# wmeddie/CycloneML

Hardware: AMD Instinct MI355X
Metric: rows/s per training iteration (higher is better)
Workload: dtype f64

## Files before the change

### cycloneml_amd/csrc/kmeans.hip

```cpp
#pragma clang fp contract(off)

#include <hip/hip_runtime.h>

#include <algorithm>
#include <cmath>
#include <cstdlib>
#include <mutex>
#include <utility>
#include <vector>

#include "common.hpp"
#include "kmeans_i8.hpp"
#include "kmeans_cos.hpp"
#include "kmeans_sparse.hpp"
#include "silhouette.hpp"

namespace {

constexpr int kWaves = 8;
constexpr int kAssignThreads = kWaves * 64;
constexpr int kSortTile = 4096;
constexpr int kChunkRows = 256;
constexpr int kMaxK = 8192;

constexpr int kNormRows = 256, kNormCols = 16, kNormStride = kNormCols + 1;
__global__ __launch_bounds__(kNormRows) void k_row_norms(const double* __restrict__ X, int64_t n,
                                                         int d, double* __restrict__ norms) {
  __shared__ double tile[2][kNormRows * kNormStride];
  const int t = threadIdx.x;
  const int64_t row0 = (int64_t)blockIdx.x * kNormRows;
  constexpr int PER = kNormRows * kNormCols / kNormRows;
  double v[PER];
  auto load = [&](int c0) {
#pragma unroll
    for (int i = 0; i < PER; ++i) {
      const int e = t + kNormRows * i, r = e / kNormCols, c = c0 + e % kNormCols;
      const int64_t gr = row0 + r;
      v[i] = (gr < n && c < d) ? __builtin_nontemporal_load(&X[gr * d + c]) : 0.0;
    }
  };
  auto store = [&](double* b) {
#pragma unroll
    for (int i = 0; i < PER; ++i) {
      const int e = t + kNormRows * i;
      b[(e / kNormCols) * kNormStride + e % kNormCols] = v[i];
    }
  };
  double s = 0.0;
  load(0);
  store(tile[0]);
  int buf = 0;
  for (int c0 = 0; c0 < d; c0 += kNormCols) {
    if (c0 + kNormCols < d) load(c0 + kNormCols);
    __syncthreads();
    const double* row = tile[buf] + t * kNormStride;
    const int lim = min(kNormCols, d - c0);
    for (int c = 0; c < lim; ++c) s = dadd(s, dmul(row[c], row[c]));
    if (c0 + kNormCols < d) store(tile[buf ^ 1]);
    buf ^= 1;
  }
  const int64_t gr = row0 + t;
  if (gr < n) norms[gr] = __builtin_sqrt(s);
}

__global__ void k_center_transpose(const double* __restrict__ C, int k, int d, int d4, int kpad,
                                   double* __restrict__ Ct) {
  int64_t idx = (int64_t)blockIdx.x * blockDim.x + threadIdx.x;
  int64_t total = (int64_t)d4 * kpad;
  if (idx >= total) return;
  int j = (int)(idx / kpad), i = (int)(idx % kpad);
  Ct[idx] = (i < k && j < d) ? C[(int64_t)i * d + j] : 0.0;
}

constexpr unsigned long long kInfBits = 0x7FF0000000000000ull;
constexpr int kStT = 32;
constexpr int kStC = 32;

__global__ void k_fill_u64(unsigned long long* __restrict__ p, int n, unsigned long long v) {
  const int i = blockIdx.x * blockDim.x + threadIdx.x;
  if (i < n) p[i] = v;
}
__global__ void k_center_transpose_fill(const double* __restrict__ C, int k, int d, int d4,
                                        int kpad, double* __restrict__ Ct,
                                        unsigned long long* __restrict__ p, unsigned long long v) {
  const int64_t idx = (int64_t)blockIdx.x * blockDim.x + threadIdx.x;
  if (idx < k) p[idx] = v;
  const int64_t total = (int64_t)d4 * kpad;
  if (idx >= total) return;
  const int j = (int)(idx / kpad), i = (int)(idx % kpad);
  Ct[idx] = (i < k && j < d) ? C[(int64_t)i * d + j] : 0.0;
}
__global__ void k_zero2(unsigned int* __restrict__ a, unsigned int* __restrict__ b) {
  if (threadIdx.x == 0) *a = 0u;
  if (threadIdx.x == 1 && b) *b = 0u;
}

__global__ __launch_bounds__(256) void k_stats_pairs(const double* __restrict__ C, int k, int d,
                                                     int tps, double* __restrict__ packed,
                                                     unsigned long long* __restrict__ dmin) {
  __shared__ double Ci[kStT][kStC + 1], Cj[kStT][kStC + 1];
  __shared__ unsigned long long rmin[kStT], cmin[kStT];
  int t = blockIdx.x, bi = 0;
  while (t >= tps - bi) {
    t -= tps - bi;
    ++bi;
  }
  const int bj = bi + t;
  const int tx = threadIdx.x & 15, ty = threadIdx.x >> 4;
  if (threadIdx.x < kStT) rmin[threadIdx.x] = cmin[threadIdx.x] = kInfBits;
  double s00 = 0.0, s01 = 0.0, s10 = 0.0, s11 = 0.0;
  for (int c0 = 0; c0 < d; c0 += kStC) {
    __syncthreads();
    for (int e = threadIdx.x; e < kStT * kStC; e += 256) {
      const int r = e >> 5, cc = e & 31, col = c0 + cc;
      const int gi = bi * kStT + r, gj = bj * kStT + r;
      Ci[r][cc] = (gi < k && col < d) ? C[(int64_t)gi * d + col] : 0.0;
      Cj[r][cc] = (gj < k && col < d) ? C[(int64_t)gj * d + col] : 0.0;
    }
    __syncthreads();
    const int lim = min(kStC, d - c0);
    for (int cc = 0; cc < lim; ++cc) {
      const double a0 = Ci[ty][cc], a1 = Ci[ty + 16][cc];
      const double b0 = Cj[tx][cc], b1 = Cj[tx + 16][cc];
      double q = dsub(a0, b0);
      s00 = dadd(s00, dmul(q, q));
      q = dsub(a0, b1);
      s01 = dadd(s01, dmul(q, q));
      q = dsub(a1, b0);
      s10 = dadd(s10, dmul(q, q));
      q = dsub(a1, b1);
      s11 = dadd(s11, dmul(q, q));
    }
  }
  const double sv[2][2] = {{s00, s01}, {s10, s11}};
#pragma unroll
  for (int a = 0; a < 2; ++a) {
#pragma unroll
    for (int b = 0; b < 2; ++b) {
      const int i = bi * kStT + ty + 16 * a, j = bj * kStT + tx + 16 * b;
      if (i < k && j < k && j > i) {
        const double dist = __builtin_sqrt(sv[a][b]);
        const double v = dmul(dmul(0.25, dist), dist);
        packed[iut(i, j)] = v;
        const unsigned long long bits = (unsigned long long)__double_as_longlong(v);
        atomicMin(&rmin[ty + 16 * a], bits);
        atomicMin(&cmin[tx + 16 * b], bits);
      }
    }
  }
  __syncthreads();
  if (threadIdx.x < kStT) {
    const int i = bi * kStT + threadIdx.x, j = bj * kStT + threadIdx.x;
    if (i < k && rmin[threadIdx.x] != kInfBits) atomicMin(&dmin[i], rmin[threadIdx.x]);
    if (j < k && cmin[threadIdx.x] != kInfBits) atomicMin(&dmin[j], cmin[threadIdx.x]);
  }
}

__global__ void k_stats_diag(int k, double* __restrict__ packed,
                             const unsigned long long* __restrict__ dmin) {
  const int i = blockIdx.x * blockDim.x + threadIdx.x;
  if (i >= k) return;
  if (k == 1) {
    packed[0] = __builtin_nan("");
    return;
  }
  packed[iut(i, i)] = __longlong_as_double((long long)dmin[i]);
}

struct Slot {
  float L1, U1, L2;
  int I1;
};

__device__ __forceinline__ float ulp_down(float f) {
  int b = __float_as_int(f);
  if (f == 0.0f) return -__int_as_float(1);
  return __int_as_float(f > 0.0f ? b - 1 : b + 1);
}
__device__ __forceinline__ float f_down(double x) {
  float f = (float)x;
  return ((double)f > x) ? ulp_down(f) : f;
}
__device__ __forceinline__ float f_up(double x) {
  float f = (float)x;
  return ((double)f < x) ? -ulp_down(-f) : f;
}

__device__ __forceinline__ void slot_merge(Slot& a, float oL1, float oU1, float oL2, int oI1) {
  float hi = fmaxf(a.L1, oL1);
  float l2 = fminf(hi, fminf(a.L2, oL2));
  if (oL1 < a.L1 || (oL1 == a.L1 && oI1 >= 0 && (a.I1 < 0 || oI1 < a.I1))) {
    a.L1 = oL1;
    a.U1 = oU1;
    a.I1 = oI1;
  }
  a.L2 = l2;
}

template <int BM>
__global__ __launch_bounds__(kAssignThreads, 1) void k_kmeans_assign(
    const double* __restrict__ X, const double* __restrict__ xnorm, int64_t n, int d, int d4,
    int ldsStride, const double* __restrict__ Ct, const double* __restrict__ C,
    const double* __restrict__ cnorm, int k, int kpad, double marginFac,
    int32_t* __restrict__ assign, double* __restrict__ cost, int32_t* __restrict__ slowList,
    unsigned int* __restrict__ slowCount, const int32_t* __restrict__ rowList,
    const unsigned int* __restrict__ rowCount) {
  constexpr int T = BM / 16;
  extern __shared__ __attribute__((aligned(16))) double smem[];
  double* Xs = smem;
  double* xnS = Xs + BM * ldsStride;
  double* mrg = xnS + BM;

  const int tid = threadIdx.x, lane = tid & 63, wave = tid >> 6;
  const int64_t nsrc = rowList ? (int64_t)*rowCount : n;
  for (int64_t blk = blockIdx.x; blk * BM < nsrc; blk += gridDim.x) {
#define CYC_GROW1(i) (rowList ? (int64_t)rowList[row0 + (i)] : row0 + (i))
  const int64_t row0 = blk * BM;
  const int rows = (int)min<int64_t>(BM, nsrc - row0);

  {
    const int total = rows * d;
    for (int e = tid; e < total; e += kAssignThreads) {
      int r = e / d, c = e - r * d;
      Xs[r * ldsStride + c] = X[CYC_GROW1(r) * d + c];
    }
    for (int e = tid; e < BM * d4; e += kAssignThreads) {
      int r = e / d4, c = e - r * d4;
      if (r >= rows || c >= d) Xs[r * ldsStride + c] = 0.0;
    }
    if (tid < BM) xnS[tid] = (tid < rows) ? xnorm[CYC_GROW1(tid)] : 0.0;
  }
  __syncthreads();

  float sL1[T * 4], sU1[T * 4], sL2[T * 4];
  int sI1[T * 4];
#pragma unroll
  for (int q = 0; q < T * 4; ++q) {
    sL1[q] = sU1[q] = sL2[q] = __builtin_inff();
    sI1[q] = -1;
  }
  unsigned poison = 0;
  const double* arow = Xs + (lane & 15) * ldsStride + (lane >> 4);
  cyc_double4 acc[T];

#define CYC_EPILOGUE(NB, CN)                                                   \
  do {                                                                         \
    const int c_ = (NB) + (lane & 15);                                         \
    if (c_ < k) {                                                              \
      const double cn_ = (CN);                                                 \
      const double cn2_ = cn_ * cn_;                                           \
      _Pragma("unroll") for (int t = 0; t < T; ++t) {                          \
        _Pragma("unroll") for (int r = 0; r < 4; ++r) {                        \
          const int q = 4 * t + r;                                             \
          const double xn = xnS[t * 16 + (lane >> 4) + 4 * r];                 \
          const double approx = (xn * xn + cn2_) - 2.0 * acc[t][r];            \
          const double sm = xn + cn_;                                          \
          const double M = (sm * sm) * marginFac;                              \
          const double L = approx - M, U = approx + M;                         \
          if (!(L == L) || !(U == U)) poison |= 1u << q;                       \
          if (L < sL1[q]) {                                                    \
            sL2[q] = sL1[q];                                                   \
            sL1[q] = f_down(L);                                                \
            sU1[q] = f_up(U);                                                  \
            sI1[q] = c_;                                                       \
          } else if (L < sL2[q]) {                                             \
            sL2[q] = f_down(L);                                                \
          }                                                                    \
        }                                                                      \
      }                                                                        \
    }                                                                          \
  } while (0)

  const int nslabs = (kpad - wave * 16 + kWaves * 16 - 1) / (kWaves * 16);
  if ((d4 & 15) == 0) {
    const int G = d4 / 16;
    const int total = nslabs * G;
    double cn = 0.0;
    double b0[4], b1[4];
#define CYC_LOADB(B, I)                                                             \
  do {                                                                              \
    const int nb_ = wave * 16 + ((I) / G) * (kWaves * 16);                          \
    const double* bc_ = Ct + (int64_t)(((I) % G) * 16 + (lane >> 4)) * kpad + nb_ + \
                        (lane & 15);                                                \
    _Pragma("unroll") for (int s = 0; s < 4; ++s) B[s] = bc_[(int64_t)(s * 4) * kpad]; \
  } while (0)
#define CYC_COMPUTE(B, I)                                                           \
  do {                                                                              \
    const int g_ = (I) % G;                                                         \
    const int nb_ = wave * 16 + ((I) / G) * (kWaves * 16);                          \
    if (g_ == 0) {                                                                  \
      _Pragma("unroll") for (int t = 0; t < T; ++t) acc[t] = cyc_double4{0.0, 0.0, 0.0, 0.0}; \
      const int c0_ = nb_ + (lane & 15);                                            \
      cn = c0_ < k ? cnorm[c0_] : 0.0;                                              \
    }                                                                               \
    _Pragma("unroll") for (int s = 0; s < 4; ++s) {                                 \
      _Pragma("unroll") for (int t = 0; t < T; ++t) {                               \
        const double a_ = arow[t * 16 * ldsStride + g_ * 16 + s * 4];               \
        acc[t] = __builtin_amdgcn_mfma_f64_16x16x4f64(a_, B[s], acc[t], 0, 0, 0);   \
      }                                                                             \
    }                                                                               \
    if (g_ == G - 1) CYC_EPILOGUE(nb_, cn);                                         \
  } while (0)
    if (total > 0) CYC_LOADB(b0, 0);
    for (int i = 0; i < total; i += 2) {
      if (i + 1 < total) CYC_LOADB(b1, i + 1);
      CYC_COMPUTE(b0, i);
      if (i + 2 < total) CYC_LOADB(b0, i + 2);
      if (i + 1 < total) CYC_COMPUTE(b1, i + 1);
    }
#undef CYC_LOADB
#undef CYC_COMPUTE
  } else {
    for (int nb = wave * 16; nb < kpad; nb += kWaves * 16) {
#pragma unroll
      for (int t = 0; t < T; ++t) acc[t] = cyc_double4{0.0, 0.0, 0.0, 0.0};
      const double* bcol = Ct + (int64_t)(lane >> 4) * kpad + nb + (lane & 15);
      for (int kb = 0; kb < d4; kb += 4) {
        const double b = bcol[(int64_t)kb * kpad];
#pragma unroll
// ... 604 lines not shown
  for (int i0 = first; !done && i0 < k; i0 += 64) {
    const int i = i0 + lane;
    const bool valid = i < k;
    double lb = __builtin_inf(), sii = 0.0, dd = 0.0;
    if (valid) {
      const double nd = dsub(cnorm[i], xn);
      lb = dmul(nd, nd);
      sii = ns ? 0.0 : stats[iut(i, i)];
      dd = dds[i];
    }
    int pos = 0;
    for (;;) {
      const bool visit = valid && lane >= pos && lb < best && (ns || stats[iut(i, bi)] < best);
      const bool brk = !ns && visit && dd < sii;
      const bool ev = visit && (brk || dd < best);
      const unsigned long long m = __ballot(ev);
      if (!m) break;
      const int f = __ffsll((long long)m) - 1;
      best = __shfl(dd, f);
      bi = i0 + f;
      if (__shfl((int)brk, f)) {
        done = true;
        break;
      }
      pos = f + 1;
    }
  }
  if (lane == 0) {
    assign[r] = bi;
    if (cost) cost[r] = best;
  }
}

constexpr int kExactChunk = 1024;
constexpr int kExactX = 1280;

__global__ __launch_bounds__(256) void k_assign_exact(
    const double* __restrict__ X, const double* __restrict__ xnorm, int d,
    const double* __restrict__ C, const double* __restrict__ Ct, int kpad,
    const double* __restrict__ cnorm, int k,
    const double* __restrict__ stats, const int32_t* __restrict__ slowList,
    const unsigned int* __restrict__ slowCount, int32_t* __restrict__ assign,
    double* __restrict__ cost, int exactNorm, unsigned int skipUpTo) {
  __shared__ double xs[kExactX];
  __shared__ double dds[kExactChunk];
  __shared__ int doneS;
  __shared__ double xnS;
  const unsigned cnt = *slowCount;
  if (cnt <= skipUpTo) return;
  const int tid = threadIdx.x, lane = tid & 63;
  const bool ns = stats == nullptr;
  for (unsigned idx = blockIdx.x; idx < cnt; idx += gridDim.x) {
    const int64_t r = slowList[idx];
    const double* x = X + r * d;
    __syncthreads();
    const bool xl = d <= kExactX;
    if (xl)
      for (int j = tid; j < d; j += 256) xs[j] = x[j];
    const double* xv = xl ? xs : x;
    if (exactNorm) {
      __syncthreads();
      if (tid == 0) xnS = seq_norm2(xv, d);
      __syncthreads();
    }
    const double xn = exactNorm ? xnS : xnorm[r];
    double best = __builtin_inf();
    int bi = 0;
    bool done = false;
    for (int c0 = 0; c0 < k; c0 += kExactChunk) {
      __syncthreads();
      double acc[kExactChunk / 256];
#pragma unroll
      for (int u = 0; u < kExactChunk / 256; ++u) acc[u] = 0.0;
      for (int j0 = 0; j0 < d; j0 += 16) {
        double cv[16][kExactChunk / 256];
#pragma unroll
        for (int jj = 0; jj < 16; ++jj) {
          const double* row = Ct + (int64_t)(j0 + jj) * kpad + c0 + tid;
#pragma unroll
          for (int u = 0; u < kExactChunk / 256; ++u)
            cv[jj][u] = (j0 + jj < d && c0 + tid + 256 * u < k) ? row[256 * u] : 0.0;
        }
#pragma unroll
        for (int jj = 0; jj < 16; ++jj) {
          if (j0 + jj < d) {
            const double xj = xv[j0 + jj];
#pragma unroll
            for (int u = 0; u < kExactChunk / 256; ++u) {
              const double sc = dsub(cv[jj][u], xj);
              acc[u] = dadd(acc[u], dmul(sc, sc));
            }
          }
        }
      }
#pragma unroll
      for (int u = 0; u < kExactChunk / 256; ++u)
        if (c0 + tid + 256 * u < k) dds[tid + 256 * u] = acc[u];
      __syncthreads();
      if (tid < 64) {
        int first = c0;
        if (c0 == 0 && !ns) {
          best = dds[0];
          done = best < stats[0];
          first = 1;
        }
        const int end = min(k, c0 + kExactChunk);
        for (int i0 = first; !done && i0 < end; i0 += 64) {
          const int i = i0 + lane;
          const bool valid = i < end;
          double lb = __builtin_inf(), sii = 0.0, dd = 0.0;
          if (valid) {
            const double nd = dsub(cnorm[i], xn);
            lb = dmul(nd, nd);
            sii = ns ? 0.0 : stats[iut(i, i)];
            dd = dds[i - c0];
          }
          int pos = 0;
          for (;;) {
            const bool visit = valid && lane >= pos && lb < best && (ns || stats[iut(i, bi)] < best);
            const bool brk = !ns && visit && dd < sii;
            const bool ev = visit && (brk || dd < best);
            const unsigned long long m = __ballot(ev);
            if (!m) break;
            const int f = __ffsll((long long)m) - 1;
            best = __shfl(dd, f);
            bi = i0 + f;
            if (__shfl((int)brk, f)) {
              done = true;
              break;
            }
            pos = f + 1;
          }
        }
        if (tid == 0) doneS = done;
      }
      __syncthreads();
      if (doneS) break;
    }
    if (tid == 0) {
      assign[r] = bi;
      if (cost) cost[r] = best;
    }
  }
}

__global__ void k_nostats_cost_fix(int64_t n, double* __restrict__ cost) {
  const int64_t r = (int64_t)blockIdx.x * blockDim.x + threadIdx.x;
  if (r < n && __builtin_isnan(cost[r])) cost[r] = __builtin_inf();
}

__global__ void k_require_norms(const double* __restrict__ C, int k, int d,
                                const double* __restrict__ xnorm, int64_t n,
                                unsigned long long* __restrict__ req) {
  const int64_t stride = (int64_t)gridDim.x * blockDim.x;
  const int64_t t0 = (int64_t)blockIdx.x * blockDim.x + threadIdx.x;
  const int64_t kd = (int64_t)k * d;
  for (int64_t i = t0; i < kd; i += stride)
    if (__builtin_isnan(C[i])) atomicMin(&req[0], (unsigned long long)(i / d));
  for (int64_t r = t0; r < n; r += stride)
    if (__builtin_isnan(xnorm[r])) atomicMin(&req[1], (unsigned long long)r);
  double* out = reinterpret_cast<double*>(req + 2);
  if (t0 < 2 && t0 < k) out[t0] = seq_norm2(C + t0 * d, d);
  if (t0 == 2) out[2] = n > 0 ? xnorm[0] : 0.0;
}

__global__ void k_hist(const int32_t* __restrict__ assign, int64_t n, int k,
                       int32_t* __restrict__ hist, const int* __restrict__ gate) {
  if (gate && !*gate) return;
  extern __shared__ int32_t cnt[];
  for (int c = threadIdx.x; c < k; c += blockDim.x) cnt[c] = 0;
  __syncthreads();
  const int64_t r0 = (int64_t)blockIdx.x * kSortTile;
  const int64_t r1 = min<int64_t>(n, r0 + kSortTile);
  for (int64_t r = r0 + threadIdx.x; r < r1; r += blockDim.x) atomicAdd(&cnt[assign[r]], 1);
  __syncthreads();
  for (int c = threadIdx.x; c < k; c += blockDim.x) hist[(int64_t)blockIdx.x * k + c] = cnt[c];
}

constexpr int kScanSegs = 64;

__global__ void k_scan_seg(const int32_t* __restrict__ hist, int tiles, int k, int segT,
                           int32_t* __restrict__ segsum, const int* __restrict__ gate) {
  if (gate && !*gate) return;
  const int c = blockIdx.x * 64 + threadIdx.x, s = blockIdx.y;
  if (c >= k) return;
  const int t0 = s * segT, t1 = min(tiles, t0 + segT);
  int sum = 0;
#pragma unroll 8
  for (int t = t0; t < t1; ++t) sum += hist[(int64_t)t * k + c];
  segsum[(int64_t)s * k + c] = sum;
}

__global__ void k_scan_segoff(int32_t* __restrict__ segsum, int segs, int k,
                              int64_t* __restrict__ total, const int* __restrict__ gate) {
  if (gate && !*gate) return;
  const int c = blockIdx.x * blockDim.x + threadIdx.x;
  if (c >= k) return;
  int64_t run = 0;
  for (int s = 0; s < segs; ++s) {
    const int32_t h = segsum[(int64_t)s * k + c];
    segsum[(int64_t)s * k + c] = (int32_t)run;
    run += h;
  }
  total[c] = run;
}

__global__ void k_scan_apply(int32_t* __restrict__ hist, int tiles, int k, int segT,
                             const int32_t* __restrict__ segoff, const int* __restrict__ gate) {
  if (gate && !*gate) return;
  const int c = blockIdx.x * 64 + threadIdx.x, s = blockIdx.y;
  if (c >= k) return;
  const int t0 = s * segT, t1 = min(tiles, t0 + segT);
  int32_t run = segoff[(int64_t)s * k + c];
  for (int t = t0; t < t1; ++t) {
    const int32_t h = hist[(int64_t)t * k + c];
    hist[(int64_t)t * k + c] = run;
    run += h;
  }
}

__global__ void k_scan_clusters(const int64_t* __restrict__ total, int k,
                                int64_t* __restrict__ cstart, int64_t* __restrict__ chunkStart,
                                const int* __restrict__ gate) {
  if (gate && !*gate) return;
  __shared__ int64_t s_rows[1024], s_chunks[1024];
  const int tid = threadIdx.x;
  const int per = (k + 1023) / 1024;
  int64_t rows = 0, chunks = 0;
  for (int q = 0; q < per; ++q) {
    int c = tid * per + q;
    if (c < k) {
      rows += total[c];
      chunks += (total[c] + kChunkRows - 1) / kChunkRows;
    }
  }
  s_rows[tid] = rows;
  s_chunks[tid] = chunks;
  __syncthreads();
  for (int off = 1; off < 1024; off <<= 1) {
    int64_t a = tid >= off ? s_rows[tid - off] : 0, b = tid >= off ? s_chunks[tid - off] : 0;
    __syncthreads();
    s_rows[tid] += a;
    s_chunks[tid] += b;
    __syncthreads();
  }
  int64_t rbase = tid ? s_rows[tid - 1] : 0, cbase = tid ? s_chunks[tid - 1] : 0;
  for (int q = 0; q < per; ++q) {
    int c = tid * per + q;
    if (c < k) {
      cstart[c] = rbase;
      chunkStart[c] = cbase;
      rbase += total[c];
      cbase += (total[c] + kChunkRows - 1) / kChunkRows;
    }
  }
  if (tid == 1023) {
    cstart[k] = s_rows[1023];
    chunkStart[k] = s_chunks[1023];
  }
}

__global__ void k_scatter(const int32_t* __restrict__ assign, int64_t n, int k,
                          const int32_t* __restrict__ tileOff, const int64_t* __restrict__ cstart,
                          int32_t* __restrict__ perm, int64_t tiles, const int* __restrict__ gate) {
  if (gate && !*gate) return;
  extern __shared__ int64_t pos[];
  const int64_t per = ((int64_t)gridDim.x + 7) / 8;
  const int64_t tile = (int64_t)(blockIdx.x & 7) * per + (blockIdx.x >> 3);
  if (tile >= tiles) return;
  const int lane = threadIdx.x;
  const int kb = 32 - __builtin_clz((unsigned)max(k - 1, 1));
  for (int c = lane; c < k; c += 64) pos[c] = cstart[c] + tileOff[tile * k + c];
  __syncthreads();
  const int64_t r0 = tile * kSortTile;
  const int64_t r1 = min<int64_t>(n, r0 + kSortTile);
  constexpr int PER = kSortTile / 64;
  int cv[PER];
#pragma unroll
  for (int i = 0; i < PER; ++i) {
    const int64_t r = r0 + i * 64 + lane;
    cv[i] = (r < r1) ? assign[r] : -1;
  }
#pragma unroll
  for (int i = 0; i < PER; ++i) {
    const int64_t r = r0 + i * 64 + lane;
    const int c = cv[i];
    unsigned long long m = __ballot(c >= 0);
    for (int b = 0; b < kb; ++b) {
      const bool bit = (c >> b) & 1;
      const unsigned long long bal = __ballot(bit);
      m &= bit ? bal : ~bal;
    }
    const int prior = __popcll(m & ((1ull << lane) - 1));
    const int last = 63 - __clzll(m);
    int64_t p = (c >= 0) ? pos[c] + prior : 0;
    __builtin_amdgcn_wave_barrier();
    if (c >= 0) {
      perm[p] = (int32_t)r;
      if (last == lane) pos[c] = p + 1;
    }
    __builtin_amdgcn_wave_barrier();
  }
}

template <int NJ>
__global__ __launch_bounds__(256) void k_chunk_sums(
    const double* __restrict__ X, int d, const double* __restrict__ w,
    const double* __restrict__ C, const int32_t* __restrict__ perm,
    const int64_t* __restrict__ cstart, const int64_t* __restrict__ chunkStart, int k,
    double* __restrict__ part, double* __restrict__ pw, double* __restrict__ pc,
    double* __restrict__ costOut) {
  constexpr int G = 16;
  __shared__ double sq[G * (NJ * 256 + 1)];
  __shared__ double rcost[G];
  const int64_t ch = blockIdx.x;
  if (ch >= chunkStart[k]) return;
// ... 914 lines not shown
  const int cands[3] = {64, 32, 16};
  const int maxbm = 64;
  for (int bm : cands) {
    if (bm > maxbm) continue;
    int s = d4 + ((2 - d4 % 32) + 32) % 32;
    size_t bytes = ((size_t)bm * s + bm + (size_t)kWaves * bm * 4) * sizeof(double);
    if (bytes <= 160 * 1024) {
      stride = s;
      lds = bytes;
      return bm;
    }
  }
  return 0;
}

template <int BM>
int launch_assign(cyc_kmeans_plan p, const double* X, const double* xnorm, int64_t n,
                  const double* C, const double* cnorm, int32_t* assign, double* cost,
                  hipStream_t st, const int32_t* rowList = nullptr,
                  const unsigned int* rowCount = nullptr) {
  static bool attr_set = false;
  if (!attr_set) {
    CYC_HIP(hipFuncSetAttribute((const void*)k_kmeans_assign<BM>,
                                hipFuncAttributeMaxDynamicSharedMemorySize, 160 * 1024));
    CYC_HIP(hipFuncSetAttribute(reinterpret_cast<const void*>(&k_kmeans_assign2<BM>),
                                hipFuncAttributeMaxDynamicSharedMemorySize, 160 * 1024));
    attr_set = true;
  }
  const double marginFac = (double)(p->d + 16) * 0x1p-46;
  const int64_t blocks = rowList ? std::min<int64_t>((n + BM - 1) / BM, 1024) : (n + BM - 1) / BM;
  cyc::KernelTimer timer(rowList ? "k_kmeans_assign_fp64" : "k_kmeans_assign", st);
#define CYC_A2()                                                                              \
  hipLaunchKernelGGL(HIP_KERNEL_NAME(k_kmeans_assign2<BM>), dim3((unsigned)blocks), dim3(kAssignThreads), \
                     p->assignLds2, st, X, xnorm, n, p->d, p->d4, p->ldsStride2,               \
                     (const double*)p->ct.ptr, C, cnorm, p->k, p->kpad, marginFac, assign, cost, \
                     (int32_t*)p->slowList.ptr, (unsigned int*)p->slowCount.ptr, rowList, rowCount)
  if (p->variant == 2 || p->variant == 3) CYC_A2();
  else
  hipLaunchKernelGGL(k_kmeans_assign<BM>, dim3((unsigned)blocks), dim3(kAssignThreads),
                     p->assignLds, st, X, xnorm, n, p->d, p->d4, p->ldsStride,
                     (const double*)p->ct.ptr, C, cnorm, p->k, p->kpad, marginFac, assign, cost,
                     (int32_t*)p->slowList.ptr, (unsigned int*)p->slowCount.ptr, rowList,
                     rowCount);
  CYC_LAUNCH_CHECK("k_kmeans_assign");
  return CYC_OK;
}

int do_stats(cyc_kmeans_plan p, const double* C, hipStream_t st) {
  const int k = p->k, d = p->d;
  const int tps = (k + kStT - 1) / kStT;
  unsigned long long* dmin = (unsigned long long*)p->dmin.ptr;
  if (p->dense_ok) {
    const int64_t total = std::max<int64_t>((int64_t)p->d4 * p->kpad, k);
    hipLaunchKernelGGL(k_center_transpose_fill, dim3((unsigned)((total + 255) / 256)), dim3(256),
                       0, st, C, k, d, p->d4, p->kpad, (double*)p->ct.ptr, dmin, kInfBits);
    CYC_LAUNCH_CHECK("k_center_transpose_fill");
  } else {
    hipLaunchKernelGGL(k_fill_u64, dim3((k + 255) / 256), dim3(256), 0, st, dmin, k, kInfBits);
    CYC_LAUNCH_CHECK("k_fill_u64");
  }
  hipLaunchKernelGGL(k_stats_pairs, dim3((unsigned)(tps * (tps + 1) / 2)), dim3(256), 0, st, C, k,
                     d, tps, (double*)p->stats.ptr, dmin);
  CYC_LAUNCH_CHECK("k_stats_pairs");
  hipLaunchKernelGGL(k_stats_diag, dim3((k + 255) / 256), dim3(256), 0, st, k,
                     (double*)p->stats.ptr, (const unsigned long long*)dmin);
  CYC_LAUNCH_CHECK("k_stats_diag");
  return CYC_OK;
}

template <int TB>
int launch_assign3(cyc_kmeans_plan p, const double* X, const double* xnorm, int64_t n,
                   const double* C, const double* cnorm, int32_t* assign, double* cost,
                   hipStream_t st) {
  static bool attr_set = false;
  if (!attr_set) {
    CYC_HIP(hipFuncSetAttribute(reinterpret_cast<const void*>(&k_kmeans_assign3<TB>),
                                hipFuncAttributeMaxDynamicSharedMemorySize, 160 * 1024));
    attr_set = true;
  }
  cyc::KernelTimer timer("k_kmeans_assign", st);
  hipLaunchKernelGGL(HIP_KERNEL_NAME(k_kmeans_assign3<TB>), dim3((unsigned)((n + kS3BM - 1) / kS3BM)),
                     dim3(kS3Threads), p->lds3, st, X, xnorm, n, p->d, p->ks3,
                     (const uint4*)p->cb3.ptr, (const float*)p->cq3.ptr, p->ktp3,
                     (const int*)p->ok3.ptr, C, cnorm, p->omE3, p->tauL3, p->facU3, p->tauU3,
                     assign, cost, (int32_t*)p->list3.ptr, (unsigned int*)p->list3Count.ptr);
  CYC_LAUNCH_CHECK("k_kmeans_assign3");
  return CYC_OK;
}

int cand_args(cyc_kmeans_plan p, int64_t n, const double* X, const double* xnorm,
              const double* C, const double* cnorm, bool unit, cyc::km8::CandArgs& ca,
              bool& use) {
  use = cyc::km8::uses32(p->d);
  if (!use) return CYC_OK;
  int rc;
  if ((rc = p->candRows.reserve(sizeof(int32_t) * (size_t)n)) ||
      (rc = p->cands.reserve(sizeof(int32_t) * (size_t)n * cyc::km8::kCandMax)) ||
      (rc = p->candCount.reserve(64)))
    return rc;
  ca = cyc::km8::CandArgs{X, xnorm, C, cnorm, p->k, unit, unit ? 0x1p-19 : 0x1p-30,
                          (int32_t*)p->candRows.ptr, (int32_t*)p->cands.ptr,
                          (unsigned int*)p->candCount.ptr};
  const char* e3 = std::getenv("CYC_KMEANS_CANDS3");
  p->cands3 = !(e3 && e3[0] == '0');
  if (p->cands3) {
    if ((rc = p->candRows2.reserve(sizeof(int32_t) * (size_t)n)) ||
        (rc = p->cands2.reserve(sizeof(int32_t) * (size_t)n * cyc::km8::kCandMax)) ||
        (rc = p->candCount2.reserve(64)))
      return rc;
    ca.candRows2 = (int32_t*)p->candRows2.ptr;
    ca.cands2 = (int32_t*)p->cands2.ptr;
    ca.candCount2 = (unsigned int*)p->candCount2.ptr;
  }
  return CYC_OK;
}

int refine_args(cyc_kmeans_plan p, int64_t n, bool useCa, cyc::km8::RefineArgs& ra, bool& use) {
  const int kstride = cyc::km8::tiles32(p->k) * 32;
  use = useCa && p->k > 96 && kstride <= 4096 && std::getenv("CYC_KMEANS_NO_REFINE") == nullptr;
  p->lastRefined = use;
  if (!use) return CYC_OK;
  int rc;
  if ((rc = p->cand1Rows.reserve(sizeof(int32_t) * (size_t)n)) ||
      (rc = p->cand1.reserve(sizeof(int32_t) * (size_t)n * cyc::km8::kCand1)) ||
      (rc = p->cand1Count.reserve(64)) ||
      (rc = p->fullList.reserve(sizeof(int32_t) * (size_t)n)) ||
      (rc = p->fullCount.reserve(64)))
    return rc;
  ra = cyc::km8::RefineArgs{kstride, (int32_t*)p->cand1Rows.ptr, (int32_t*)p->cand1.ptr,
                            (unsigned int*)p->cand1Count.ptr, (int32_t*)p->fullList.ptr,
                            (unsigned int*)p->fullCount.ptr};
  return CYC_OK;
}

bool bounds_on(cyc_kmeans_plan p, cyc_kmeans_rows rows) {
  static const bool envOff = [] {
    const char* e = std::getenv("CYC_KMEANS_BOUNDS");
    return e && e[0] == '0';
  }();
  return rows && rows->usable && !rows->cosine && rows->bEnabled && !envOff &&
         !cyc::strict_parity() &&
         p->measure == CYC_DISTANCE_EUCLIDEAN && cyc::km8::uses32(p->d) && p->k > 96 &&
         cyc::km8::tiles32(p->k) * 32 <= 4096 && std::getenv("CYC_KMEANS_NO_REFINE") == nullptr;
}

bool nbrOff() {
  static const bool off = [] {
    const char* e = std::getenv("CYC_KMEANS_NBR");
    return e && e[0] == '0';
  }();
  return off || cyc::strict_parity();
}

int bounds_prepare(cyc_kmeans_plan p, cyc_kmeans_rows rows, const double* C,
                   const double* xnorm, int64_t n, hipStream_t st, cyc::km8::Bounds& bd) {
  namespace k8 = cyc::km8;
  const int k = p->k, d = p->d;
  int rc;
  if ((rc = rows->bnd.reserve(sizeof(float2) * (size_t)n)) ||
      (rc = rows->bAssign.reserve(sizeof(int32_t) * (size_t)n)) ||
      (rc = rows->bCp.reserve(sizeof(double) * (size_t)k * d)) ||
      (rc = rows->bDelta.reserve(sizeof(double) * (size_t)k)) ||
      (rc = rows->bCcs.reserve(sizeof(double) * (size_t)k)) ||
      (rc = rows->bPrm.reserve(sizeof(k8::DriftParams))) ||
      (rc = rows->bTmp.reserve(sizeof(int32_t) * (size_t)n)) ||
      (rc = rows->bCount.reserve(sizeof(unsigned int) * (size_t)(k8::bounds_blocks(n) + 1))) ||
      (rc = rows->bTmp2.reserve(sizeof(int32_t) * (size_t)n)) ||
      (rc = rows->bCount2.reserve(sizeof(unsigned int) * (size_t)(k8::bounds_blocks(n) + 1))) ||
      (rc = rows->bList.reserve(sizeof(int32_t) * (size_t)n)) ||
      (rc = rows->bListCount.reserve(64)) ||
      (rc = rows->bLnc.reserve(sizeof(float) * (size_t)n)) ||
      (rc = rows->bSets.reserve(sizeof(int32_t) * (size_t)n * k8::kCandMax)) ||
      (rc = rows->bState.reserve((size_t)n)) ||
      (rc = rows->bRc.reserve(sizeof(int32_t) * (size_t)n)) ||
      (rc = rows->bRcCount.reserve(64)) ||
      (rc = rows->bNbr.reserve(sizeof(int32_t) * (size_t)k * k8::kCandMax)) ||
      (rc = rows->bNbrR.reserve(sizeof(float) * (size_t)k)))
    return rc;
  if (!rows->bCum.ptr) {
    if ((rc = rows->bCum.reserve(64)) || (rc = rows->bRcCum.reserve(64))) return rc;
    CYC_HIP(hipMemsetAsync(rows->bCum.ptr, 0, 8, st));
    CYC_HIP(hipMemsetAsync(rows->bRcCum.ptr, 0, 8, st));
  }
  const bool carry = rows->bValid && rows->bk == k;
  rows->bValid = false;
  if ((rc = k8::centers_drift(C, (double*)rows->bCp.ptr, k, d, (double*)rows->bDelta.ptr,
                              (double*)rows->bCcs.ptr, (k8::DriftParams*)rows->bPrm.ptr, st)))
    return rc;
  bd = k8::Bounds{(float2*)rows->bnd.ptr, nullptr, nullptr};
  bd.lnc = (float*)rows->bLnc.ptr;
  bd.sets = (int32_t*)rows->bSets.ptr;
  bd.state = (unsigned char*)rows->bState.ptr;
  bd.dp = (const k8::DriftParams*)rows->bPrm.ptr;
  bd.tmp = (int32_t*)rows->bTmp.ptr;
  bd.bcount = (unsigned int*)rows->bCount.ptr;
  bd.list = (int32_t*)rows->bList.ptr;
  bd.listCount = (unsigned int*)rows->bListCount.ptr;
  bd.cum = (unsigned long long*)rows->bCum.ptr;
  bd.n = n;
  if (carry) {
    const bool two = k8::recheck_two_phase();
    if ((rc = k8::bounds_filter((const int32_t*)rows->bAssign.ptr, (float2*)rows->bnd.ptr,
                                bd.lnc, bd.state, xnorm, n, k, (const double*)rows->bDelta.ptr,
                                bd.dp, bd.tmp, bd.bcount, (int32_t*)rows->bRc.ptr,
                                (unsigned int*)rows->bRcCount.ptr,
                                (unsigned long long*)rows->bRcCum.ptr,
                                nbrOff() ? nullptr : (const double*)p->stats.ptr,
                                (int32_t*)rows->bNbr.ptr, (float*)rows->bNbrR.ptr, st,
                                two ? (int32_t*)rows->bTmp2.ptr : nullptr,
                                two ? (unsigned int*)rows->bCount2.ptr : nullptr,
                                two ? bd.list : nullptr, two ? bd.listCount : nullptr,
                                two ? bd.cum : nullptr)))
      return rc;
    bd.collected = two;
    if (!nbrOff()) {
      bd.nbr = (const int32_t*)rows->bNbr.ptr;
      bd.nbrR = (const float*)rows->bNbrR.ptr;
    }
    static const int dumpCall = [] {
      const char* e = std::getenv("CYC_KMEANS_DUMP_CALL");
      return e ? std::atoi(e) : 10;
    }();
    if (cyc::dump_dir() && rows->bCalls == dumpCall) {
      bd.dump = 1;
      cyc::dump_dev("state_filter", rows->bState.ptr, (size_t)n, st);
      cyc::dump_dev("bnd", rows->bnd.ptr, sizeof(float2) * (size_t)n, st);
      cyc::dump_dev("lnc", rows->bLnc.ptr, sizeof(float) * (size_t)n, st);
      cyc::dump_dev("assign", rows->bAssign.ptr, sizeof(int32_t) * (size_t)n, st);
      cyc::dump_dev("nbrR", rows->bNbrR.ptr, sizeof(float) * (size_t)k, st);
      cyc::dump_dev("nbr", rows->bNbr.ptr, sizeof(int32_t) * (size_t)k * k8::kCandMax, st);
      cyc::dump_dev("delta", rows->bDelta.ptr, sizeof(double) * (size_t)k, st);
      cyc::dump_dev("prm", rows->bPrm.ptr, sizeof(k8::DriftParams), st);
    }
    bd.rcRows = (const int32_t*)rows->bRc.ptr;
    bd.rcCount = (const unsigned int*)rows->bRcCount.ptr;
    bd.rowsIn = bd.list;
    bd.rowsInCount = bd.listCount;
  } else {
    CYC_HIP(hipMemsetAsync(bd.lnc, 0xff, sizeof(float) * (size_t)n, st));
    rows->bFullRows += n;
  }
  return CYC_OK;
}

int stage_args(cyc_kmeans_plan p, int64_t n, bool useCa, cyc::km8::AppendStage& sg, bool& use) {
  use = useCa && std::getenv("CYC_KMEANS_NO_STAGE") == nullptr;
  if (!use) return CYC_OK;
  namespace k8 = cyc::km8;
  const unsigned cap = k8::shard_cap(n);
  const size_t ent = (size_t)cap * k8::kShards;
  const size_t cbytes = sizeof(unsigned int) * k8::kSets * k8::kShards * k8::kShardStride;
  int rc;
  if ((rc = p->stgRowsA.reserve(sizeof(int32_t) * ent)) ||
      (rc = p->stgRowsB.reserve(sizeof(int32_t) * ent)) ||
      (rc = p->stgCandRows.reserve(sizeof(int32_t) * ent)) ||
      (rc = p->stgCands.reserve(sizeof(int32_t) * ent * k8::kCand1)) ||
      (rc = p->stgCounts.reserve(cbytes)))
    return rc;
  sg = k8::AppendStage{(int32_t*)p->stgRowsA.ptr, (int32_t*)p->stgRowsB.ptr,
                       (int32_t*)p->stgCandRows.ptr, (int32_t*)p->stgCands.ptr,
                       (unsigned int*)p->stgCounts.ptr, cap};
  return CYC_OK;
}

int launch_exact(cyc_kmeans_plan p, const double* X, const double* xnorm, int64_t n,
                 const double* C, const double* cnorm, const double* statsArg, int32_t* assign,
                 double* cost, bool approxNorm, int64_t known, hipStream_t st) {
  cyc::KernelTimer timer("k_kmeans_exact", st);
  const int k = p->k, kpad = p->kpad;
  const unsigned* cnt = (const unsigned*)p->slowCount.ptr;
  static const bool splitOff = [] {
    const char* e = std::getenv("CYC_KMEANS_EXACT_SPLIT");
    return e && e[0] == '0';
  }();
  const bool split = !splitOff && p->d <= 1280 && (known < 0 || known <= kExactCap);
  if (split) {
    int rc;
    if ((rc = p->exactDist.reserve(sizeof(double) * (size_t)kExactCap * kpad))) return rc;
    const unsigned rowsMax = (unsigned)std::min<int64_t>(known < 0 ? n : known, kExactCap);
    hipLaunchKernelGGL(k_exact_dist, dim3((unsigned)((k + 255) / 256), rowsMax), dim3(256), 0, st,
                       X, p->d, (const double*)p->ct.ptr, kpad, k, (const int32_t*)p->slowList.ptr,
                       cnt, (double*)p->exactDist.ptr);
    CYC_LAUNCH_CHECK("k_exact_dist");
    hipLaunchKernelGGL(k_exact_replay, dim3(rowsMax), dim3(64), 0, st, X, xnorm, p->d, kpad, cnorm,
                       k, statsArg, (const int32_t*)p->slowList.ptr, cnt,
                       (const double*)p->exactDist.ptr, assign, cost, approxNorm ? 1 : 0);
    CYC_LAUNCH_CHECK("k_exact_replay");
    if (known >= 0) return CYC_OK;
  }
  const unsigned grid = known >= 0 ? (unsigned)std::min<int64_t>(known, 4096)
                                   : (unsigned)std::min<int64_t>((n + 3) / 4, 2048);
  hipLaunchKernelGGL(k_assign_exact, dim3(grid), dim3(256), 0, st, X, xnorm, p->d, C,
                     (const double*)p->ct.ptr, kpad, cnorm, k, statsArg,
                     (const int32_t*)p->slowList.ptr, cnt, assign, cost, approxNorm ? 1 : 0,
                     split ? (unsigned)kExactCap : 0u);
  CYC_LAUNCH_CHECK("k_assign_exact");
  return CYC_OK;
}

int do_assign(cyc_kmeans_plan p, const double* X, const double* xnorm, cyc_kmeans_rows rows,
              int64_t n, const double* C, const double* cnorm, int32_t* assign, double* cost,
              int64_t* n_exact_out, hipStream_t st, bool nostats = false,
              const cyc::km8::Bounds* bd = nullptr, bool approxNorm = false) {
  const double* statsArg = nostats ? nullptr : (const double*)p->stats.ptr;
  const bool i8 = rows && rows->usable;
  hipLaunchKernelGGL(k_zero2, dim3(1), dim3(64), 0, st, (unsigned int*)p->slowCount.ptr,
                     i8 ? (unsigned int*)p->list3Count.ptr : nullptr);
  CYC_LAUNCH_CHECK("k_zero2");
  int rc = CYC_OK;
  const int32_t* rowList = nullptr;
  const unsigned int* rowCount = nullptr;
  if (i8) {
    if ((rc = cyc::km8::centers_prepare(C, cnorm, p->k, p->d, p->ktp8, p->cb8.ptr,
                                        (float*)p->cq8.ptr, (double*)p->g8.ptr,
                                        (cyc::km8::CenterParams*)p->prm8.ptr,
                                        (double*)p->scr8.ptr, st)))
      return rc;
    cyc::km8::CandArgs ca;
    bool useCa = false;
    if ((rc = cand_args(p, n, X, nullptr, C, cnorm, false, ca, useCa))) return rc;
    cyc::km8::RefineArgs ra;
    bool useRa = false;
    if ((rc = refine_args(p, n, useCa, ra, useRa))) return rc;
    cyc::km8::AppendStage sg;
    bool useSg = false;
    if ((rc = stage_args(p, n, useCa, sg, useSg))) return rc;
    if ((rc = cyc::km8::screen(rows->img.ptr, (const int2*)rows->meta.ptr, xnorm, n, p->d,
                               p->cb8.ptr, (const float*)p->cq8.ptr, (const double*)p->g8.ptr,
                               cnorm, (const cyc::km8::CenterParams*)p->prm8.ptr, p->ktp8,
                               assign, (int32_t*)p->list3.ptr, (unsigned int*)p->list3Count.ptr,
                               (int32_t*)p->slowList.ptr, (unsigned int*)p->list8Count.ptr, st,
                               useCa ? &ca : nullptr, useRa ? &ra : nullptr,
                               useSg ? &sg : nullptr, bd)))
      return rc;
    rowList = (const int32_t*)p->list3.ptr;
    rowCount = (const unsigned int*)p->list3Count.ptr;
  } else if (p->variant == 3) {
    CYC_HIP(hipMemsetAsync(p->list3Count.ptr, 0, sizeof(unsigned int), st));
    CYC_HIP(hipMemsetAsync(p->ok3.ptr, 1, sizeof(int), st));
    const int64_t tot = (int64_t)p->ktp3 * p->ks3 * 64;
    hipLaunchKernelGGL(k_center_split, dim3((unsigned)((tot + 255) / 256)), dim3(256), 0, st, C,
                       cnorm, p->k, p->d, p->ks3, p->ktp3, p->omE3, (uint4*)p->cb3.ptr,
                       (float*)p->cq3.ptr, (int*)p->ok3.ptr);
    CYC_LAUNCH_CHECK("k_center_split");
    rc = launch_assign3<2>(p, X, xnorm, n, C, cnorm, assign, cost, st);
    if (rc) return rc;
    rowList = (const int32_t*)p->list3.ptr;
    rowCount = (const unsigned int*)p->list3Count.ptr;
  }
  static const bool list16 = [] {
    const char* e = std::getenv("CYC_KMEANS_LIST_BM");
    return !(e && e[0] == '0');
  }();
  if (rowList && list16 && p->bm >= 16) {
    rc = launch_assign<16>(p, X, xnorm, n, C, cnorm, assign, cost, st, rowList, rowCount);
  } else switch (p->bm) {
    case 64: rc = launch_assign<64>(p, X, xnorm, n, C, cnorm, assign, cost, st, rowList, rowCount); break;
    case 32: rc = launch_assign<32>(p, X, xnorm, n, C, cnorm, assign, cost, st, rowList, rowCount); break;
    default: rc = launch_assign<16>(p, X, xnorm, n, C, cnorm, assign, cost, st, rowList, rowCount); break;
  }
  if (rc) return rc;
  unsigned int h_slow = 0, h_tier2 = 0, h_limb3 = 0, h_cand = 0, h_cand2 = 0;
  if (n_exact_out) {
    const bool twoPass = rows && rows->usable && cyc::km8::uses32(p->d);
    CYC_HIP(hipMemcpyAsync(&h_slow, p->slowCount.ptr, sizeof(unsigned), hipMemcpyDeviceToHost, st));
    if (rowCount)
      CYC_HIP(hipMemcpyAsync(&h_tier2, rowCount, sizeof(unsigned), hipMemcpyDeviceToHost, st));
    if (twoPass) {
      CYC_HIP(hipMemcpyAsync(&h_limb3, p->list8Count.ptr, sizeof(unsigned), hipMemcpyDeviceToHost, st));
      CYC_HIP(hipMemcpyAsync(&h_cand, p->candCount.ptr, sizeof(unsigned), hipMemcpyDeviceToHost, st));
      if (p->cands3)
        CYC_HIP(hipMemcpyAsync(&h_cand2, p->candCount2.ptr, sizeof(unsigned), hipMemcpyDeviceToHost, st));
    }
    CYC_HIP(hipStreamSynchronize(st));
    *n_exact_out = h_slow;
    p->lastTier2 = rowCount ? (int64_t)h_tier2 : n;
    p->lastExact = h_slow;
    p->lastLimb3 = twoPass ? (int64_t)h_limb3 : -1;
    p->lastCands = twoPass ? (int64_t)h_cand : -1;
    p->lastCands2 = twoPass && p->cands3 ? (int64_t)h_cand2 : -1;
    if (h_slow)
      return launch_exact(p, X, xnorm, n, C, cnorm, statsArg, assign, cost, approxNorm,
                          (int64_t)h_slow, st);
    return CYC_OK;
  }
  return launch_exact(p, X, xnorm, n, C, cnorm, statsArg, assign, cost, approxNorm, -1, st);
}

int require_enqueue(cyc_kmeans_plan p, const double* C, const double* xnorm, int64_t n,
                    hipStream_t st) {
  int rc;
  if ((rc = p->req.reserve(5 * sizeof(unsigned long long)))) return rc;
  if (!p->reqHost) CYC_HIP(hipHostMalloc((void**)&p->reqHost, 5 * sizeof(unsigned long long)));
  if (!p->reqEv) CYC_HIP(hipEventCreateWithFlags(&p->reqEv, hipEventDisableTiming));
  CYC_HIP(hipMemsetAsync(p->req.ptr, 0xff, 2 * sizeof(unsigned long long), st));
  const int64_t work = std::max<int64_t>(n, (int64_t)p->k * p->d);
  const unsigned grid = (unsigned)std::max<int64_t>(1, std::min<int64_t>((work + 255) / 256, 2048));
  hipLaunchKernelGGL(k_require_norms, dim3(grid), dim3(256), 0, st, C, p->k, p->d, xnorm, n,
                     (unsigned long long*)p->req.ptr);
  CYC_LAUNCH_CHECK("k_require_norms");
  CYC_HIP(hipMemcpyAsync(p->reqHost, p->req.ptr, 5 * sizeof(unsigned long long),
                         hipMemcpyDeviceToHost, st));
  CYC_HIP(hipEventRecord(p->reqEv, st));
  return CYC_OK;
}

int require_check(cyc_kmeans_plan p, int64_t n, const double* Xrow0 = nullptr) {
  CYC_HIP(hipEventSynchronize(p->reqEv));
  const unsigned long long cbad = p->reqHost[0], rbad = p->reqHost[1];
  double* v = reinterpret_cast<double*>(p->reqHost + 2);
  if (Xrow0 && n > 0 && cbad == 0 && !(p->k >= 2)) {
    std::vector<double> x0((size_t)p->d);
    CYC_HIP(hipMemcpy(x0.data(), Xrow0, sizeof(double) * (size_t)p->d, hipMemcpyDeviceToHost));
    double sq = 0.0;
    for (int j = 0; j < p->d; ++j) sq = sq + x0[j] * x0[j];
    v[2] = std::sqrt(sq);
  }
  const double nan = __builtin_nan("");
  auto fail = [](double n1, double n2) {
    cyc::set_error("requirement failed: Both norms should be greater or equal to 0.0, found "
                   "norm1=" + cyc::java_double(n1) + ", norm2=" + cyc::java_double(n2));
    return CYC_ERR_INVALID_ARG;
  };
  if (p->k >= 2 && cbad < (unsigned long long)p->k) return cbad == 0 ? fail(nan, v[1]) : fail(v[0], nan);
  if (n > 0 && cbad == 0) return fail(nan, v[2]);
  if (rbad < (unsigned long long)n) return fail(v[0], nan);
  return CYC_OK;
}

int ensure_rows(cyc_kmeans_plan p, int64_t n) {
  if (n <= p->max_rows && p->slowList.ptr) return CYC_OK;
  int rc;
  if ((rc = p->slowList.reserve(sizeof(int32_t) * (size_t)std::max<int64_t>(n, 1)))) return rc;
  if ((rc = p->list3.reserve(sizeof(int32_t) * (size_t)std::max<int64_t>(n, 1)))) return rc;
  p->max_rows = std::max(p->max_rows, n);
  return CYC_OK;
}

bool is_cos(cyc_kmeans_plan p) { return p->measure == CYC_DISTANCE_COSINE; }

int cos_enqueue(cyc_kmeans_plan p, const double* cnorm, bool checkCenters, const double* xnorm,
                int64_t n, hipStream_t st) {
  int rc;
  if ((rc = p->req.reserve(5 * sizeof(unsigned long long)))) return rc;
  if (!p->reqHost) CYC_HIP(hipHostMalloc((void**)&p->reqHost, 5 * sizeof(unsigned long long)));
  if (!p->reqEv) CYC_HIP(hipEventCreateWithFlags(&p->reqEv, hipEventDisableTiming));
  if ((rc = cyc::kmcos::assert_norms(cnorm, p->k, checkCenters, xnorm, n,
                                     (unsigned long long*)p->req.ptr, st)))
    return rc;
  CYC_HIP(hipMemcpyAsync(p->reqHost, p->req.ptr, sizeof(unsigned long long),
                         hipMemcpyDeviceToHost, st));
  CYC_HIP(hipEventRecord(p->reqEv, st));
  return CYC_OK;
}

int cos_check(cyc_kmeans_plan p) {
  CYC_HIP(hipEventSynchronize(p->reqEv));
  if (p->reqHost[0]) {
    cyc::set_error("assertion failed: Cosine distance is not defined for zero-length vectors.");
    return CYC_ERR_ASSERTION;
  }
  return CYC_OK;
}

int cos_transpose(cyc_kmeans_plan p, const double* C, hipStream_t st) {
  const int64_t total = (int64_t)p->d4 * p->kpad;
  hipLaunchKernelGGL(k_center_transpose, dim3((unsigned)((total + 255) / 256)), dim3(256), 0, st,
                     C, p->k, p->d, p->d4, p->kpad, (double*)p->ct.ptr);
  CYC_LAUNCH_CHECK("k_center_transpose");
  return CYC_OK;
}

int cos_stats(cyc_kmeans_plan p, const double* C, const double* cnorm, hipStream_t st) {
  return cyc::kmcos::stats(C, cnorm, p->k, p->d, (double*)p->stats.ptr,
                           (unsigned long long*)p->dmin.ptr, st);
}

int cos_assign(cyc_kmeans_plan p, const double* X, const double* xnorm, cyc_kmeans_rows rows,
               int64_t n, const double* C, const double* cnorm, int32_t* assign, double* cost,
               int64_t* n_exact_out, hipStream_t st, bool nostats) {
  int rc;
  if ((rc = cos_transpose(p, C, st))) return rc;
  int32_t* list = (int32_t*)p->list3.ptr;
  unsigned int* count = (unsigned int*)p->list3Count.ptr;
  const bool screen = rows && rows->usable && p->ktp8 > 0;
  if (screen) {
    if ((rc = p->cosV.reserve(sizeof(double) * (size_t)p->k * p->d)) ||
        (rc = p->cosVn.reserve(sizeof(double) * (size_t)p->k)))
      return rc;
    double* V = (double*)p->cosV.ptr;
    double* Vn = (double*)p->cosVn.ptr;
    if ((rc = cyc::kmcos::centers_unit(C, cnorm, p->k, p->d, V, Vn, st))) return rc;
    CYC_HIP(hipMemsetAsync(count, 0, sizeof(unsigned int), st));
    cyc::km8::CandArgs ca;
    bool useCa = false;
    if ((rc = cand_args(p, n, X, xnorm, V, Vn, true, ca, useCa))) return rc;
    cyc::km8::AppendStage sg;
    bool useSg = false;
    if ((rc = stage_args(p, n, useCa, sg, useSg))) return rc;
    if ((rc = cyc::km8::centers_prepare(V, Vn, p->k, p->d, p->ktp8, p->cb8.ptr,
                                        (float*)p->cq8.ptr, (double*)p->g8.ptr,
                                        (cyc::km8::CenterParams*)p->prm8.ptr,
                                        (double*)p->scr8.ptr, st)) ||
        (rc = cyc::km8::screen(rows->img.ptr, (const int2*)rows->meta.ptr,
                               (const double*)rows->unorm.ptr, n, p->d, p->cb8.ptr,
                               (const float*)p->cq8.ptr, (const double*)p->g8.ptr, Vn,
                               (const cyc::km8::CenterParams*)p->prm8.ptr, p->ktp8, assign, list,
                               count, (int32_t*)p->slowList.ptr,
                               (unsigned int*)p->list8Count.ptr, st, useCa ? &ca : nullptr,
                               nullptr, useSg ? &sg : nullptr)))
      return rc;
  } else if ((rc = cyc::kmcos::list_all(list, count, n, st))) {
    return rc;
  }
  int64_t maxRows = n;
  if (n_exact_out) {
    unsigned int h = 0, h3 = 0, hc = 0, hc2 = 0;
    const bool twoPass = screen && cyc::km8::uses32(p->d);
    CYC_HIP(hipMemcpyAsync(&h, count, sizeof(unsigned), hipMemcpyDeviceToHost, st));
    if (twoPass) {
      CYC_HIP(hipMemcpyAsync(&h3, p->list8Count.ptr, sizeof(unsigned), hipMemcpyDeviceToHost, st));
      CYC_HIP(hipMemcpyAsync(&hc, p->candCount.ptr, sizeof(unsigned), hipMemcpyDeviceToHost, st));
      if (p->cands3)
        CYC_HIP(hipMemcpyAsync(&hc2, p->candCount2.ptr, sizeof(unsigned), hipMemcpyDeviceToHost, st));
    }
    CYC_HIP(hipStreamSynchronize(st));
    *n_exact_out = h;
    p->lastTier2 = h;
    p->lastExact = h;
    p->lastLimb3 = twoPass ? (int64_t)h3 : -1;
    p->lastCands = twoPass ? (int64_t)hc : -1;
    p->lastCands2 = twoPass && p->cands3 ? (int64_t)hc2 : -1;
    maxRows = h;
  }
  if (maxRows == 0) return CYC_OK;
  return cyc::kmcos::assign_exact(X, xnorm, p->d, C, (const double*)p->ct.ptr, p->kpad, cnorm,
                                  p->k, nostats ? nullptr : (const double*)p->stats.ptr, list,
                                  count, maxRows, assign, cost, st);
}

}

namespace {

int sort_clusters(cyc_kmeans_plan p, const int32_t* assign, int64_t n, int d, hipStream_t st,
                  int64_t& maxChunks, const int* gate = nullptr) {
  const int k = p->k;
  int rc;
  const int tiles = (int)((n + kSortTile - 1) / kSortTile);
  maxChunks = (n + kChunkRows - 1) / kChunkRows + k;
  if ((rc = p->hist.reserve(sizeof(int32_t) * (size_t)tiles * k)) ||
      (rc = p->total.reserve(sizeof(int64_t) * (size_t)k)) ||
      (rc = p->cstart.reserve(sizeof(int64_t) * (size_t)(k + 1))) ||
      (rc = p->chunkStart.reserve(sizeof(int64_t) * (size_t)(k + 1))) ||
      (rc = p->perm.reserve(sizeof(int32_t) * (size_t)n)) ||
      (rc = p->part.reserve(sizeof(double) * (size_t)maxChunks * d)) ||
      (rc = p->pw.reserve(sizeof(double) * (size_t)maxChunks)) ||
// ... 171 lines not shown
  CYC_REQUIRE(d > 0, "Number of features must be positive");
  CYC_REQUIRE(k >= 1, "Number of clusters must be positive but got " + std::to_string(k));
  int ndev = 0;
  if (hipGetDeviceCount(&ndev) != hipSuccess || ndev == 0) {
    cyc::set_error("no HIP device visible");
    return CYC_ERR_NO_DEVICE;
  }
  if (k > kMaxK) {
    cyc::set_error("k > 8192 is not supported by the device counting sort");
    return CYC_ERR_UNSUPPORTED;
  }
  auto* p = new cyc_kmeans_plan_s();
  p->d = d;
  p->k = k;
  p->d4 = (int)cyc::round_up(d, 4);
  p->kpad = (int)cyc::round_up(k, 16);
  p->bm = pick_bm(p->d4, p->ldsStride, p->assignLds);
  p->ldsStride2 = p->d4 + 1;
  p->assignLds2 = p->assignLds + sizeof(double) * ((size_t)p->kpad + p->bm) -
                  sizeof(double) * (size_t)p->bm * (p->ldsStride - p->ldsStride2);
  p->variant = ((p->d4 % 32) == 0 && p->assignLds2 <= 160 * 1024) ? 2 : 1;
  p->ks3 = (int)((d + 31) / 32);
  p->lds3 = (size_t)2 * kS3BM * (p->ks3 * 4 + 1) * 16 + (size_t)kS3Waves * kS3BM * 12 +
            (size_t)kS3BM * 8;
  const bool fits3 = p->variant == 2 && p->lds3 <= 160 * 1024;
  if (fits3) p->variant = 3;
  if (const char* v = std::getenv("CYC_KMEANS_ASSIGN")) {
    const int want = std::atoi(v);
    if (want == 1 || (p->d4 % 32 == 0 && p->assignLds2 <= 160 * 1024 && want >= 2 && want <= 3 &&
                      (want != 3 || fits3)))
      p->variant = want;
  }
  {
    p->ktp3 = (int)cyc::round_up((k + 15) / 16, kS3Waves * p->tb3);
    const double d32 = 32.0 * p->ks3;
    const double eps = 3.1 * 0x1p-16 + 2.0 * 1.03 * (3.0 * d32 + 64.0) * 0x1p-23 + 0x1p-20;
    const double tau = 0x1p-58;
    p->omE3 = 1.0 - eps;
    p->tauL3 = 2.0 * tau;
    p->facU3 = (2.0 * eps + 0x1p-20) * (1.0 + 0x1p-20);
    p->tauU3 = 4.0 * tau;
  }
  p->dense_ok = p->bm != 0;
  int rc;
  if (p->variant == 3 &&
      ((rc = p->cb3.reserve((size_t)p->ktp3 * p->ks3 * 2 * 64 * 16)) ||
       (rc = p->cq3.reserve(sizeof(float) * (size_t)p->ktp3 * 16)) ||
       (rc = p->ok3.reserve(64)))) {
    delete p;
    return rc;
  }
  if ((rc = p->list3Count.reserve(64))) {
    delete p;
    return rc;
  }
  if (d <= cyc::km8::kMaxD) {
    const int ks8 = cyc::km8::ksteps(d);
    p->ktp8 = (int)cyc::round_up((k + 15) / 16, cyc::km8::kWaves);
    if ((rc = p->cb8.reserve((size_t)p->ktp8 * ks8 * 3 * 64 * 16 * 2)) ||
        (rc = p->cq8.reserve(sizeof(float) * (size_t)p->ktp8 * 48)) ||
        (rc = p->g8.reserve(sizeof(double) * (size_t)p->ktp8 * 48)) ||
        (rc = p->list8Count.reserve(64)) ||
        (rc = p->prm8.reserve(sizeof(cyc::km8::CenterParams))) ||
        (rc = p->scr8.reserve(sizeof(double) * 2 * (size_t)k))) {
      delete p;
      return rc;
    }
  }
  if ((p->dense_ok && (rc = p->ct.reserve(sizeof(double) * (size_t)p->d4 * p->kpad))) ||
      (rc = p->stats.reserve(sizeof(double) * ((size_t)k * (k + 1) / 2))) ||
      (rc = p->dmin.reserve(sizeof(unsigned long long) * (size_t)k)) ||
      (rc = p->slowCount.reserve(64)) || (rc = ensure_rows(p, std::max<int64_t>(max_rows, 1)))) {
    delete p;
    return rc;
  }
  *plan = p;
  return CYC_OK;
}

int cyc_kmeans_last_tiers(cyc_kmeans_plan p, int64_t* fp64_screen_rows, int64_t* exact_rows) {
  CYC_REQUIRE(p != nullptr && fp64_screen_rows && exact_rows, "arguments must not be null");
  std::lock_guard<std::mutex> g(p->mu);
  *fp64_screen_rows = p->lastTier2;
  *exact_rows = p->lastExact;
  return CYC_OK;
}

int cyc_kmeans_last_screen(cyc_kmeans_plan p, int64_t* three_limb_rows) {
  CYC_REQUIRE(p != nullptr && three_limb_rows, "arguments must not be null");
  std::lock_guard<std::mutex> g(p->mu);
  *three_limb_rows = p->lastLimb3;
  return CYC_OK;
}

int cyc_kmeans_last_candidates(cyc_kmeans_plan p, int64_t* candidate_rows) {
  CYC_REQUIRE(p != nullptr && candidate_rows, "arguments must not be null");
  std::lock_guard<std::mutex> g(p->mu);
  *candidate_rows = p->lastCands;
  return CYC_OK;
}

int cyc_kmeans_last_candidates3(cyc_kmeans_plan p, int64_t* fp64_rows) {
  CYC_REQUIRE(p != nullptr && fp64_rows, "arguments must not be null");
  std::lock_guard<std::mutex> g(p->mu);
  *fp64_rows = p->lastCands2;
  return CYC_OK;
}

int cyc_kmeans_last_refine(cyc_kmeans_plan p, int64_t* listed_rows, int64_t* full_rows,
                           int64_t* union_centers) {
  CYC_REQUIRE(p != nullptr && listed_rows && full_rows && union_centers,
              "arguments must not be null");
  std::lock_guard<std::mutex> g(p->mu);
  *listed_rows = *full_rows = *union_centers = -1;
  if (!p->lastRefined) return CYC_OK;
  unsigned int h[3] = {0, 0, 0};
  CYC_HIP(hipMemcpy(h, p->cand1Count.ptr, sizeof(unsigned int), hipMemcpyDeviceToHost));
  CYC_HIP(hipMemcpy(h + 1, p->fullCount.ptr, 2 * sizeof(unsigned int), hipMemcpyDeviceToHost));
  *listed_rows = h[0];
  *full_rows = h[1];
  *union_centers = h[2];
  return CYC_OK;
}

int cyc_kmeans_plan_destroy(cyc_kmeans_plan plan) {
  delete plan;
  return CYC_OK;
}

int cyc_kmeans_plan_set_distance_measure(cyc_kmeans_plan p, int32_t measure) {
  CYC_REQUIRE(p != nullptr, "plan must not be null");
  CYC_REQUIRE(measure == CYC_DISTANCE_EUCLIDEAN || measure == CYC_DISTANCE_COSINE,
              "distanceMeasure must be one of: euclidean, cosine. " + std::to_string(measure) +
                  " provided.");
  std::lock_guard<std::mutex> g(p->mu);
  p->measure = measure;
  return CYC_OK;
}

int cyc_kmeans_stats_dev(cyc_kmeans_plan p, const double* C, double* stats_out, void* stream) {
  CYC_REQUIRE(p != nullptr && C != nullptr, "plan and centers must not be null");
  std::lock_guard<std::mutex> g(p->mu);
  hipStream_t st = cyc::as_stream(stream);
  int rc;
  if (is_cos(p)) {
    if ((rc = p->cosCn.reserve(sizeof(double) * (size_t)p->k))) return rc;
    const double* cn = (const double*)p->cosCn.ptr;
    hipLaunchKernelGGL(k_row_norms, dim3((unsigned)((p->k + kNormRows - 1) / kNormRows)),
                       dim3(kNormRows), 0, st, C, (int64_t)p->k, p->d, (double*)p->cosCn.ptr);
    CYC_LAUNCH_CHECK("k_row_norms");
    if ((rc = cos_enqueue(p, cn, p->k >= 2, nullptr, 0, st))) return rc;
    if (p->dense_ok && (rc = cos_transpose(p, C, st))) return rc;
    if ((rc = cos_stats(p, C, cn, st))) return rc;
  } else {
    if ((rc = require_enqueue(p, C, nullptr, 0, st))) return rc;
    if ((rc = do_stats(p, C, st))) return rc;
  }
  if (stats_out)
    CYC_HIP(hipMemcpyAsync(stats_out, p->stats.ptr, sizeof(double) * ((size_t)p->k * (p->k + 1) / 2),
                           hipMemcpyDeviceToDevice, st));
  return is_cos(p) ? cos_check(p) : require_check(p, 0);
}

int cyc_kmeans_rows_create(cyc_kmeans_plan p, const double* X, int64_t n, void* stream,
                           cyc_kmeans_rows* out) {
  CYC_REQUIRE(p != nullptr && out != nullptr, "plan and out must not be null");
  CYC_REQUIRE(n >= 0, "n >= 0");
  CYC_REQUIRE(X != nullptr || n == 0, "X must not be null");
  auto* r = new cyc_kmeans_rows_s();
  r->X = X;
  r->n = n;
  r->d = p->d;
  r->usable = p->d <= cyc::km8::kMaxD && p->ktp8 > 0;
  r->cosine = is_cos(p);
  if (r->usable && n > 0) {
    int rc;
    hipStream_t st = cyc::as_stream(stream);
    if ((rc = r->img.reserve((size_t)n * cyc::km8::image_row_bytes(p->d))) ||
        (rc = r->meta.reserve(sizeof(int2) * (size_t)n))) {
      delete r;
      return rc;
    }
    if (r->cosine) {
      cyc::DeviceBuffer xn;
      if ((rc = r->unorm.reserve(sizeof(double) * (size_t)n)) ||
          (rc = xn.reserve(sizeof(double) * (size_t)n))) {
        delete r;
        return rc;
      }
      hipLaunchKernelGGL(k_row_norms, dim3((unsigned)((n + kNormRows - 1) / kNormRows)),
                         dim3(kNormRows), 0, st, X, n, p->d, (double*)xn.ptr);
      CYC_LAUNCH_CHECK("k_row_norms");
      rc = cyc::km8::rows_quantize(X, n, p->d, r->img.ptr, (int2*)r->meta.ptr, st,
                                   (const double*)xn.ptr, (double*)r->unorm.ptr);
      if (!rc && hipStreamSynchronize(st) != hipSuccess) rc = CYC_ERR_HIP;
    } else {
      if ((rc = r->unorm.reserve(sizeof(double) * (size_t)n))) {
        delete r;
        return rc;
      }
      rc = cyc::km8::rows_quantize(X, n, p->d, r->img.ptr, (int2*)r->meta.ptr, st, nullptr,
                                   (double*)r->unorm.ptr);
    }
    if (rc) {
      delete r;
      return rc;
    }
  }
  *out = r;
  return CYC_OK;
}

int cyc_kmeans_rows_destroy(cyc_kmeans_rows rows) {
  delete rows;
  return CYC_OK;
}

int64_t cyc_kmeans_rows_bytes(cyc_kmeans_rows rows) {
  return rows ? (int64_t)(rows->img.bytes + rows->meta.bytes) : 0;
}

int cyc_kmeans_rows_set_bounds(cyc_kmeans_rows rows, int32_t enable) {
  CYC_REQUIRE(rows != nullptr, "rows must not be null");
  rows->bEnabled = enable != 0;
  rows->bValid = false;
  return CYC_OK;
}

int cyc_kmeans_rows_set_incremental(cyc_kmeans_rows rows, int32_t enable) {
  CYC_REQUIRE(rows != nullptr, "rows must not be null");
  rows->iEnabled = enable != 0;
  rows->iValid = false;
  return CYC_OK;
}

int cyc_kmeans_rows_incremental_info(cyc_kmeans_rows rows, int64_t* incremental_calls,
                                     int64_t* moved_rows) {
  CYC_REQUIRE(rows != nullptr && incremental_calls != nullptr && moved_rows != nullptr,
              "arguments must not be null");
  unsigned long long cum[2] = {0, 0};
  if (rows->iCum.ptr) {
    CYC_HIP(hipDeviceSynchronize());
    CYC_HIP(hipMemcpy(cum, rows->iCum.ptr, sizeof(cum), hipMemcpyDeviceToHost));
  }
  *incremental_calls = (int64_t)cum[1];
  *moved_rows = (int64_t)cum[0];
  return CYC_OK;
}

int cyc_kmeans_rows_bounds_rechecked(cyc_kmeans_rows rows, int64_t* rechecked_rows) {
  CYC_REQUIRE(rows != nullptr && rechecked_rows != nullptr, "arguments must not be null");
  unsigned long long cum = 0;
  if (rows->bRcCum.ptr) {
    CYC_HIP(hipDeviceSynchronize());
    CYC_HIP(hipMemcpy(&cum, rows->bRcCum.ptr, sizeof(cum), hipMemcpyDeviceToHost));
  }
  *rechecked_rows = (int64_t)cum;
  return CYC_OK;
}

int cyc_kmeans_rows_bounds_info(cyc_kmeans_rows rows, int64_t* calls, int64_t* screened_rows) {
  CYC_REQUIRE(rows != nullptr && calls != nullptr && screened_rows != nullptr,
              "arguments must not be null");
  unsigned long long cum = 0;
  if (rows->bCum.ptr) {
    CYC_HIP(hipDeviceSynchronize());
    CYC_HIP(hipMemcpy(&cum, rows->bCum.ptr, sizeof(cum), hipMemcpyDeviceToHost));
  }
  *calls = rows->bCalls;
  *screened_rows = rows->bFullRows + (int64_t)cum;
  return CYC_OK;
}

namespace {
int check_rows(cyc_kmeans_plan p, cyc_kmeans_rows rows, const double* X, int64_t n) {
  CYC_REQUIRE(rows == nullptr || (rows->X == X && rows->n == n && rows->d == p->d),
              "the row image was built for other rows (cyc_kmeans_rows_create)");
  CYC_REQUIRE(rows == nullptr || rows->cosine == is_cos(p),
              "the row image was built for another distance measure");
  return CYC_OK;
}
}

int cyc_kmeans_assign_dev(cyc_kmeans_plan p, const double* X, const double* xnorm,
                          cyc_kmeans_rows rows, int64_t n, const double* C, const double* cnorm,
                          int32_t* assign, double* cost, int64_t* n_exact_out, void* stream) {
  CYC_REQUIRE(p != nullptr, "plan must not be null");
  CYC_REQUIRE(n >= 0, "n >= 0");
  CYC_REQUIRE(assign != nullptr && cost != nullptr, "assign and cost must not be null");
  if (n_exact_out) *n_exact_out = 0;
  if (n == 0) return CYC_OK;
  if (int rc = check_rows(p, rows, X, n)) return rc;
  if (!p->dense_ok) {
    cyc::set_error("d > 1240 is not supported by the LDS-resident assign kernel (dense rows)");
    return CYC_ERR_UNSUPPORTED;
  }
  std::lock_guard<std::mutex> g(p->mu);
  hipStream_t st = cyc::as_stream(stream);
  int rc = ensure_rows(p, n);
  if (rc) return rc;
  if (is_cos(p)) {
    if ((rc = cos_enqueue(p, cnorm, true, xnorm, n, st)) ||
        (rc = cos_assign(p, X, xnorm, rows, n, C, cnorm, assign, nullptr, n_exact_out, st, false)) ||
        (rc = cyc::kmcos::row_cost(X, n, p->d, C, cnorm, xnorm, assign, cost, st)))
      return rc;
    return cos_check(p);
  }
  if ((rc = require_enqueue(p, C, xnorm, n, st))) return rc;
  if ((rc = do_assign(p, X, xnorm, rows, n, C, cnorm, assign, nullptr, n_exact_out, st))) return rc;
  hipLaunchKernelGGL(k_row_cost, dim3((unsigned)((n + kNormRows - 1) / kNormRows)),
                     dim3(kNormRows), 0, st, X, n, p->d, C,
                     (const int32_t*)assign, cost);
  CYC_LAUNCH_CHECK("k_row_cost");
  return require_check(p, n);
}

int cyc_kmeans_point_cost_dev(cyc_kmeans_plan p, const double* X, const double* xnorm,
                              cyc_kmeans_rows rows, int64_t n, const double* C,
                              const double* cnorm, int32_t* assign, double* cost, void* stream) {
  CYC_REQUIRE(p != nullptr, "plan must not be null");
  CYC_REQUIRE(n >= 0, "n >= 0");
  CYC_REQUIRE(assign != nullptr && cost != nullptr, "assign and cost must not be null");
  if (n == 0) return CYC_OK;
  if (int rc = check_rows(p, rows, X, n)) return rc;
  if (!p->dense_ok) {
    cyc::set_error("d > 1240 is not supported by the LDS-resident assign kernel (dense rows)");
    return CYC_ERR_UNSUPPORTED;
  }
  std::lock_guard<std::mutex> g(p->mu);
  hipStream_t st = cyc::as_stream(stream);
  int rc = ensure_rows(p, n);
  if (rc) return rc;
  if (is_cos(p)) {
    if ((rc = cos_enqueue(p, cnorm, true, xnorm, n, st)) ||
        (rc = cos_assign(p, X, xnorm, rows, n, C, cnorm, assign, nullptr, nullptr, st, true)) ||
        (rc = cyc::kmcos::row_cost(X, n, p->d, C, cnorm, xnorm, assign, cost, st)))
      return rc;
    hipLaunchKernelGGL(k_nostats_cost_fix, dim3((unsigned)((n + 255) / 256)), dim3(256), 0, st, n,
                       cost);
    CYC_LAUNCH_CHECK("k_nostats_cost_fix");
    return cos_check(p);
  }
  const int64_t total = (int64_t)p->d4 * p->kpad;
  hipLaunchKernelGGL(k_center_transpose, dim3((unsigned)((total + 255) / 256)), dim3(256), 0, st,
                     C, p->k, p->d, p->d4, p->kpad, (double*)p->ct.ptr);
  CYC_LAUNCH_CHECK("k_center_transpose");
  if ((rc = do_assign(p, X, xnorm, rows, n, C, cnorm, assign, nullptr, nullptr, st, true)))
    return rc;
  hipLaunchKernelGGL(k_row_cost, dim3((unsigned)((n + kNormRows - 1) / kNormRows)),
                     dim3(kNormRows), 0, st, X, n, p->d, C,
                     (const int32_t*)assign, cost);
  CYC_LAUNCH_CHECK("k_row_cost");
  hipLaunchKernelGGL(k_nostats_cost_fix, dim3((unsigned)((n + 255) / 256)), dim3(256), 0, st, n,
                     cost);
  CYC_LAUNCH_CHECK("k_nostats_cost_fix");
  return CYC_OK;
}

int cyc_kmeans_accumulate_dev(cyc_kmeans_plan p, const double* X, const double* xnorm,
                              cyc_kmeans_rows rows, const double* weights, int64_t n,
                              const double* C, const double* cnorm, double* sums, double* wsum,
                              double* cost_sum, int32_t* assign, double* cost, void* stream) {
  CYC_REQUIRE(p != nullptr, "plan must not be null");
  CYC_REQUIRE(n >= 0, "n >= 0");
  CYC_REQUIRE(sums && wsum && cost_sum, "sums, wsum and cost_sum must not be null");
  if (n == 0) return CYC_OK;
  if (int rc = check_rows(p, rows, X, n)) return rc;
  if (!p->dense_ok) {
    cyc::set_error("d > 1240 is not supported by the LDS-resident assign kernel (dense rows)");
    return CYC_ERR_UNSUPPORTED;
  }
  const bool approxNorm = xnorm == nullptr;
  CYC_REQUIRE(!approxNorm || (rows && rows->usable && !rows->cosine && rows->unorm.ptr),
              "xnorm may be null only with a Euclidean row image (cyc_kmeans_rows_create)");
  if (approxNorm) xnorm = (const double*)rows->unorm.ptr;
  std::lock_guard<std::mutex> g(p->mu);
  hipStream_t st = cyc::as_stream(stream);
  const int k = p->k, d = p->d;
  int rc = ensure_rows(p, n);
  if (rc) return rc;
  const bool useBnd = bounds_on(p, rows);
  int32_t* const userAssign = assign;
  if (useBnd) {
    assign = (int32_t*)nullptr;
  } else if (!assign) {
    if ((rc = p->assignTmp.reserve(sizeof(int32_t) * (size_t)n))) return rc;
    assign = (int32_t*)p->assignTmp.ptr;
  }
  const bool cosm = is_cos(p);
  if (cosm) {
    if ((rc = cos_enqueue(p, cnorm, true, xnorm, n, st)) || (rc = cos_stats(p, C, cnorm, st)) ||
        (rc = cos_assign(p, X, xnorm, rows, n, C, cnorm, assign, nullptr, nullptr, st, false)))
      return rc;
  } else {
    if ((rc = require_enqueue(p, C, xnorm, n, st))) return rc;
    if ((rc = do_stats(p, C, st))) return rc;
    cyc::km8::Bounds bd{};
    if (useBnd) {
      if ((rc = bounds_prepare(p, rows, C, xnorm, n, st, bd))) return rc;
      assign = (int32_t*)rows->bAssign.ptr;
    }
    if ((rc = do_assign(p, X, xnorm, rows, n, C, cnorm, assign, nullptr, nullptr, st, false,
                        useBnd ? &bd : nullptr, approxNorm)))
      return rc;
    if (useBnd) {
      rows->bValid = true;
      rows->bk = k;
      ++rows->bCalls;
      if (userAssign)
        CYC_HIP(hipMemcpyAsync(userAssign, assign, sizeof(int32_t) * (size_t)n,
                               hipMemcpyDeviceToDevice, st));
    }
  }
  const int nj = (d + 255) / 256;
  const bool useInc = useBnd && inc_on(rows) && !cost && !weights && nj <= 4;
  if (rows && !useInc) rows->iValid = false;
  if (useInc) {
    if ((rc = inc_accumulate(p, rows, X, xnorm, assign, n, C, sums, wsum, cost_sum, st)))
      return rc;
    rc = require_check(p, n, approxNorm ? X : nullptr);
    rows->iValid = rc == CYC_OK;
    rows->ik = k;
    return rc;
  }
  if (cosm) {
    if (!cost) {
      if ((rc = p->costTmp.reserve(sizeof(double) * (size_t)n))) return rc;
      cost = (double*)p->costTmp.ptr;
    }
    if ((rc = cyc::kmcos::row_cost(X, n, d, C, cnorm, xnorm, assign, cost, st))) return rc;
  } else if (nj > 4) {
    if (!cost) {
      if ((rc = p->costTmp.reserve(sizeof(double) * (size_t)n))) return rc;
      cost = (double*)p->costTmp.ptr;
    }
    hipLaunchKernelGGL(k_row_cost, dim3((unsigned)((n + kNormRows - 1) / kNormRows)),
                     dim3(kNormRows), 0, st, X, n, d, C,
                       (const int32_t*)assign, cost);
    CYC_LAUNCH_CHECK("k_row_cost");
  }

  int64_t maxChunks = 0;
  if ((rc = sort_clusters(p, assign, n, d, st, maxChunks))) return rc;
  if (cosm) {
    if ((rc = cyc::kmcos::chunk_sums(X, d, weights, xnorm, cost, (const int32_t*)p->perm.ptr,
                                     (const int64_t*)p->cstart.ptr,
                                     (const int64_t*)p->chunkStart.ptr, k, maxChunks,
                                     (double*)p->part.ptr, (double*)p->pw.ptr,
                                     (double*)p->pc.ptr, st)))
      return rc;
  } else {
    cyc::KernelTimer timer("k_chunk_sums", st);
    const dim3 grid((unsigned)maxChunks);
#define CYC_CS(NJ)                                                                              \
  hipLaunchKernelGGL(HIP_KERNEL_NAME(k_chunk_sums<NJ>), grid, dim3(256), 0, st, X, d, weights, C, \
                     (const int32_t*)p->perm.ptr, (const int64_t*)p->cstart.ptr,               \
                     (const int64_t*)p->chunkStart.ptr, k, (double*)p->part.ptr,               \
                     (double*)p->pw.ptr, (double*)p->pc.ptr, cost)
#define CYC_CSF(NJ)                                                                              \
  hipLaunchKernelGGL(HIP_KERNEL_NAME(k_chunk_sums_fast<NJ>), grid, dim3(256), 0, st, X, d, weights, \
                     C, (const int32_t*)p->perm.ptr, (const int64_t*)p->cstart.ptr,             \
                     (const int64_t*)p->chunkStart.ptr, k, (double*)p->part.ptr,                \
                     (double*)p->pw.ptr, (double*)p->pc.ptr, (const double*)nullptr,             \
                     (double*)nullptr, (const int*)nullptr)
    if (!cost && nj == 1) CYC_CSF(1);
    else if (!cost && nj == 2) CYC_CSF(2);
    else if (!cost && nj <= 4) CYC_CSF(4);
    else if (nj == 1) CYC_CS(1);
    else if (nj == 2) CYC_CS(2);
    else if (nj <= 4) CYC_CS(4);
    else
      hipLaunchKernelGGL(k_chunk_sums_nocost, grid, dim3(256), 0, st, X, d, weights,
                         (const double*)cost, (const int32_t*)p->perm.ptr,
                         (const int64_t*)p->cstart.ptr, (const int64_t*)p->chunkStart.ptr, k,
                         (double*)p->part.ptr, (double*)p->pw.ptr, (double*)p->pc.ptr);
#undef CYC_CS
#undef CYC_CSF
    CYC_LAUNCH_CHECK("k_chunk_sums");
  }
  hipLaunchKernelGGL(k_reduce_clusters, dim3(k), dim3(256), 0, st, (const double*)p->part.ptr,
                     (const double*)p->pw.ptr, (const double*)p->pc.ptr,
                     (const int64_t*)p->chunkStart.ptr, d, sums, wsum, (double*)p->ccost.ptr,
                     (const double*)nullptr, (double*)nullptr, (double*)nullptr, (double*)nullptr,
                     (const int*)nullptr);
  CYC_LAUNCH_CHECK("k_reduce_clusters");
  hipLaunchKernelGGL(k_cost_total, dim3(1), dim3(256), 0, st, (const double*)p->ccost.ptr, k,
                     cost_sum, (const int*)nullptr);
  CYC_LAUNCH_CHECK("k_cost_total");
  return cosm ? cos_check(p) : require_check(p, n, approxNorm ? X : nullptr);
}

int cyc_kmeans_update_dev(cyc_kmeans_plan p, double* C, double* cnorm, const double* sums,
                          const double* wsum, double epsilon, int32_t* converged_out,
                          void* stream) {
  CYC_REQUIRE(p != nullptr, "plan must not be null");
  CYC_REQUIRE(epsilon >= 0, "epsilon must be nonnegative");
  std::lock_guard<std::mutex> g(p->mu);
  hipStream_t st = cyc::as_stream(stream);
  if (converged_out) CYC_HIP(hipMemsetD32Async((hipDeviceptr_t)converged_out, 1, 1, st));
  if (is_cos(p))
    return cyc::kmcos::update(C, cnorm, sums, wsum, p->k, p->d, epsilon, converged_out, st);
  hipLaunchKernelGGL(k_update_centers, dim3((unsigned)p->k), dim3(64),
                     p->d <= kUpdLds ? sizeof(double) * 2 * (size_t)p->d : 0, st, C, cnorm, sums, wsum, p->k, p->d,
                     epsilon * epsilon, converged_out);
  CYC_LAUNCH_CHECK("k_update_centers");
  return CYC_OK;
}


namespace {

int sil_check(cyc_kmeans_plan p, const int32_t* pred, const double* w, int64_t n,
              hipStream_t st) {
  int rc;
  if ((rc = p->silFlags.reserve(16))) return rc;
  unsigned int* bad = (unsigned int*)p->silFlags.ptr;
  unsigned long long* badW = (unsigned long long*)((char*)p->silFlags.ptr + 8);
  CYC_HIP(hipMemsetAsync(bad, 0, 8, st));
  CYC_HIP(hipMemsetAsync(badW, 0xff, 8, st));
  if ((rc = cyc::silh::check_pred(pred, w, n, p->k, bad, badW, st))) return rc;
  unsigned long long h[2] = {0, 0};
  CYC_HIP(hipMemcpyAsync(h, p->silFlags.ptr, 16, hipMemcpyDeviceToHost, st));
  CYC_HIP(hipStreamSynchronize(st));
  if ((unsigned int)h[0] != 0u) {
    cyc::set_error("requirement failed: predictions must lie in [0, k) for k = " +
                   std::to_string(p->k));
    return CYC_ERR_INVALID_ARG;
  }
  if (h[1] != ~0ull) {
    double v = 0.0;
    CYC_HIP(hipMemcpy(&v, w + h[1], sizeof(double), hipMemcpyDeviceToHost));
    cyc::set_error("requirement failed: illegal weight value: " + cyc::java_double(v) +
                   ". weight must be >= 0.0.");
    return CYC_ERR_INVALID_ARG;
  }
  return CYC_OK;
}

int sil_norms(cyc_kmeans_plan p, const double* X, const double* xnorm, int64_t n, hipStream_t st,
              const double*& out) {
  if (xnorm) {
    out = xnorm;
    return CYC_OK;
  }
  int rc;
  if ((rc = p->silNorms.reserve(sizeof(double) * (size_t)n))) return rc;
  if ((rc = cyc_row_norms_dev(X, n, p->d, (double*)p->silNorms.ptr, st))) return rc;
  out = (const double*)p->silNorms.ptr;
  return CYC_OK;
}

}

int cyc_kmeans_silhouette_stats_dev(cyc_kmeans_plan p, const double* X, const double* xnorm,
                                    int64_t n, const int32_t* pred, const double* weights,
                                    double* stats, void* stream) {
// ... 168 lines not shown
```

### cycloneml_amd/csrc/kmeans_i8.hip

```cpp
#include "kmeans_i8.hpp"

#include <climits>
#include <type_traits>
#include <cstdlib>

#include "common.hpp"

#ifndef CYC_PROBE_MODE
#define CYC_PROBE_MODE 0
#endif

namespace cyc {
namespace km8 {
namespace {

typedef int v4i __attribute__((ext_vector_type(4)));
typedef unsigned v4u __attribute__((ext_vector_type(4)));
typedef double v2d __attribute__((ext_vector_type(2)));

#ifndef CYC_QUANT_COAL
#define CYC_QUANT_COAL 1
#endif

__device__ __forceinline__ float ulp_dn(float f) {
// ... 145 lines not shown
  for (; row < n; row += nw) {
    v2d nxt[2];
    load(row + nw, nxt);
    const double sc = scale ? scale[row] : 1.0;
    double v[4] = {cur[0].x, cur[0].y, cur[1].x, cur[1].y};
    double m = 0.0, s1 = 0.0, s2 = 0.0;
    bool fin = true;
#pragma unroll
    for (int q = 0; q < 4; ++q) {
      if (scale) v[q] = v[q] / sc;
      fin = fin && __builtin_isfinite(v[q]);
      m = __builtin_fmax(m, __builtin_fabs(v[q]));
      s1 += __builtin_fabs(v[q]);
      s2 += v[q] * v[q];
    }
    m = wave_max(m);
    s1 = wave_sum(s1);
    if (unorm) {
      s2 = wave_sum(s2);
      if (lane == 0) unorm[row] = __builtin_sqrt(s2);
    }
    const bool allFin = __all(fin);
    const int e = choose_exp(m);
    const bool bad = !allFin || e > kMaxExp;
    if (j0 < D) {
      int a[4], b[4], c[4];
#pragma unroll
      for (int q = 0; q < 4; ++q) {
        if (bad) a[q] = b[q] = c[q] = 0;
        else quant3(v[q], e, a[q], b[q], c[q]);
      }
      unsigned char* db = reinterpret_cast<unsigned char*>(img + row * (int64_t)(3 * D / 4));
      *reinterpret_cast<unsigned*>(db + j0) = pack4(a);
      *reinterpret_cast<unsigned*>(db + D + j0) = pack4(b);
      *reinterpret_cast<unsigned*>(db + 2 * D + j0) = pack4(c);
    }
    if (lane == 0) {
      const double n1 = bad ? 0.0 : s1 * (1.0 + 0x1p-40) + (double)d * __builtin_ldexp(1.0, e - 22);
      meta[row] = make_int2(bad ? INT_MIN : e, __float_as_int(fup(n1)));
    }
    cur[0] = nxt[0];
    cur[1] = nxt[1];
  }
}

__global__ __launch_bounds__(256) void k_rows_quantize(const double* __restrict__ X, int64_t n,
                                                       int d, int D, unsigned* __restrict__ img,
                                                       int2* __restrict__ meta,
                                                       const double* __restrict__ scale,
                                                       double* __restrict__ unorm, int vec) {
  const int lane = threadIdx.x & 63;
  const int64_t nw = ((int64_t)gridDim.x * blockDim.x) >> 6;
  for (int64_t row = ((int64_t)blockIdx.x * blockDim.x + threadIdx.x) >> 6; row < n; row += nw) {
    const double* x = X + row * d;
    double v[8];
    double m = 0.0, s1 = 0.0, s2 = 0.0;
    bool fin = true;
    const double sc = scale ? scale[row] : 1.0;
#if CYC_QUANT_COAL
#pragma unroll
    for (int h = 0; h < 4; ++h) {
      const int j = h * 128 + 2 * lane;
      v2d w = {0.0, 0.0};
      if (vec) {
        if (j < d) w = __builtin_nontemporal_load(reinterpret_cast<const v2d*>(x + j));
      } else {
        if (j < d) w.x = x[j];
        if (j + 1 < d) w.y = x[j + 1];
      }
#pragma unroll
      for (int q = 0; q < 2; ++q) {
        double t = q ? w.y : w.x;
        if (scale) t = t / sc;
        v[2 * h + q] = t;
        fin = fin && __builtin_isfinite(t);
        m = __builtin_fmax(m, __builtin_fabs(t));
        s1 += __builtin_fabs(t);
        s2 += t * t;
      }
    }
#else
#pragma unroll
    for (int p = 0; p < 2; ++p) {
#pragma unroll
      for (int q = 0; q < 4; ++q) {
        const int j = p * 256 + 4 * lane + q;
        double t = j < d ? x[j] : 0.0;
        if (scale) t = t / sc;
        v[4 * p + q] = t;
        fin = fin && __builtin_isfinite(t);
        m = __builtin_fmax(m, __builtin_fabs(t));
        s1 += __builtin_fabs(t);
        s2 += t * t;
      }
    }
#endif
    m = wave_max(m);
    s1 = wave_sum(s1);
    if (unorm) {
      s2 = wave_sum(s2);
      if (lane == 0) unorm[row] = __builtin_sqrt(s2);
    }
    const bool allFin = __all(fin);
    const int e = choose_exp(m);
    const bool bad = !allFin || e > kMaxExp;
#if CYC_QUANT_COAL
    unsigned char* db = reinterpret_cast<unsigned char*>(img + row * (int64_t)(3 * D / 4));
#pragma unroll
    for (int h = 0; h < 4; ++h) {
      const int j0 = h * 128 + 2 * lane;
      if (j0 < D) {
        int a[2], b[2], c[2];
#pragma unroll
        for (int q = 0; q < 2; ++q) {
          if (bad) {
            a[q] = b[q] = c[q] = 0;
          } else {
            quant3(v[2 * h + q], e, a[q], b[q], c[q]);
          }
        }
        *reinterpret_cast<unsigned short*>(db + j0) = (unsigned short)((a[0] & 0xff) | ((a[1] & 0xff) << 8));
        *reinterpret_cast<unsigned short*>(db + D + j0) = (unsigned short)((b[0] & 0xff) | ((b[1] & 0xff) << 8));
        *reinterpret_cast<unsigned short*>(db + 2 * D + j0) = (unsigned short)((c[0] & 0xff) | ((c[1] & 0xff) << 8));
      }
    }
#else
    unsigned* dst = img + row * (int64_t)(3 * D / 4);
#pragma unroll
    for (int p = 0; p < 2; ++p) {
      const int j0 = p * 256 + 4 * lane;
      if (j0 < D) {
        int a[4], b[4], c[4];
#pragma unroll
        for (int q = 0; q < 4; ++q) {
          if (bad) {
            a[q] = b[q] = c[q] = 0;
          } else {
            quant3(v[4 * p + q], e, a[q], b[q], c[q]);
          }
        }
        dst[j0 / 4] = pack4(a);
        dst[(D + j0) / 4] = pack4(b);
        dst[(2 * D + j0) / 4] = pack4(c);
      }
    }
#endif
    if (lane == 0) {
      const double n1 = bad ? 0.0 : s1 * (1.0 + 0x1p-40) + (double)d * __builtin_ldexp(1.0, e - 22);
      meta[row] = make_int2(bad ? INT_MIN : e, __float_as_int(fup(n1)));
    }
  }
}

__global__ __launch_bounds__(256) void k_centers_scan(const double* __restrict__ C, int k, int d,
                                                      double* __restrict__ cmax,
                                                      double* __restrict__ cn1) {
  const int lane = threadIdx.x & 63;
  const int c = (blockIdx.x * blockDim.x + threadIdx.x) >> 6;
  if (c >= k) return;
  double m = 0.0, s1 = 0.0;
  bool fin = true;
  for (int j = lane; j < d; j += 64) {
    const double t = C[(int64_t)c * d + j];
    fin = fin && __builtin_isfinite(t);
    m = __builtin_fmax(m, __builtin_fabs(t));
    s1 += __builtin_fabs(t);
  }
  m = wave_max(m);
  s1 = wave_sum(s1);
  const bool allFin = __all(fin);
  if (lane == 0) {
    cmax[c] = allFin ? m : __builtin_inf();
    cn1[c] = s1 * (1.0 + 0x1p-40);
  }
}

__global__ __launch_bounds__(256) void k_centers_params(int k, const double* __restrict__ cmax,
                                                        const double* __restrict__ cn1,
                                                        CenterParams* __restrict__ prm) {
  __shared__ double sm[256], sn[256];
  double m = 0.0, nmax = 0.0;
  for (int c = threadIdx.x; c < k; c += 256) {
    m = __builtin_fmax(m, cmax[c]);
    nmax = __builtin_fmax(nmax, cn1[c]);
    if (!(cmax[c] <= 0x1p60)) m = __builtin_inf();
  }
  sm[threadIdx.x] = m;
  sn[threadIdx.x] = nmax;
  __syncthreads();
  for (int off = 128; off > 0; off >>= 1) {
    if (threadIdx.x < off) {
      sm[threadIdx.x] = __builtin_fmax(sm[threadIdx.x], sm[threadIdx.x + off]);
      sn[threadIdx.x] = __builtin_fmax(sn[threadIdx.x], sn[threadIdx.x + off]);
    }
    __syncthreads();
  }
  if (threadIdx.x == 0) {
    const double gm = sm[0];
    const int ec = choose_exp(__builtin_isfinite(gm) ? gm : 0.0);
    CenterParams p;
    p.ok = (__builtin_isfinite(gm) && ec <= kMaxExp) ? 1 : 0;
    p.ec = ec;
    const double Ac = __builtin_ldexp(1.0, ec - 22);
    const double mu = sn[0] / Ac;
    p.mu = (mu > 0.0 && __builtin_isfinite(mu)) ? mu : 1.0;
    p.k = k;
    *prm = p;
  }
}

__global__ __launch_bounds__(256) void k_centers_pack(
    const double* __restrict__ C, const double* __restrict__ cnorm, int k, int d, int KS, int ktp,
    const double* __restrict__ cn1, const CenterParams* __restrict__ prm, uint4* __restrict__ Cb,
    float* __restrict__ cq, double* __restrict__ g) {
  const CenterParams p = *prm;
  const int64_t idx = (int64_t)blockIdx.x * blockDim.x + threadIdx.x;
  const int64_t total = (int64_t)ktp * KS * 64;
  if (idx < total) {
    const int lane = (int)(idx & 63);
    const int64_t t = idx >> 6;
    const int ks = (int)(t % KS), ct = (int)(t / KS);
    const int c = ct * 16 + (lane & 15), j0 = ks * 64 + 16 * (lane >> 4);
    int a[16], b[16], cc[16];
#pragma unroll
    for (int e = 0; e < 16; ++e) {
      const int j = j0 + e;
      const double v = (p.ok && c < k && j < d) ? C[(int64_t)c * d + j] : 0.0;
      quant3(v, p.ec, a[e], b[e], cc[e]);
    }
    uint4 pa, pb, pc;
    pa.x = pack4(a); pa.y = pack4(a + 4); pa.z = pack4(a + 8); pa.w = pack4(a + 12);
    pb.x = pack4(b); pb.y = pack4(b + 4); pb.z = pack4(b + 8); pb.w = pack4(b + 12);
    pc.x = pack4(cc); pc.y = pack4(cc + 4); pc.z = pack4(cc + 8); pc.w = pack4(cc + 12);
    uint4* dst = Cb + (t * 3) * 64 + lane;
    dst[0] = pa;
    dst[64] = pb;
    dst[128] = pc;
  }
  if (idx < (int64_t)ktp * 16) {
    const int c = (int)idx;
    if (c < k && p.ok) {
      const double gc = err_term(p.ec, cn1[c], p.mu, d);
      const double cn = cnorm[c];
      g[c] = gc;
      cq[c] = fdown((cn * cn) * (1.0 - kEpsF) - 2.0 * gc);
    } else {
      g[c] = 0.0;
      cq[c] = __builtin_inff();
    }
  }
}

__device__ __forceinline__ v4i as_v4i(uint4 u) { return __builtin_bit_cast(v4i, u); }

template <int KS>
__global__ __launch_bounds__(256, KS <= 4 ? 3 : 2) void k_screen(
    const uint4* __restrict__ Xq, const int2* __restrict__ meta, const double* __restrict__ xnorm,
    int64_t n, int d, const uint4* __restrict__ Cb, const float* __restrict__ cq,
    const double* __restrict__ g, const double* __restrict__ cnorm,
    const CenterParams* __restrict__ prm, int ktp, int32_t* __restrict__ assign,
    int32_t* __restrict__ list, unsigned int* __restrict__ listCount) {
  constexpr int BM = kBM, W = kWaves, CH = 12 * KS, STR = CH + 2;
  extern __shared__ __attribute__((aligned(16))) uint4 smem8[];
  uint4* As = smem8;
  int* exS = (int*)(As + BM * STR);
  float* mL1 = (float*)As;
  float* mL2 = mL1 + W * BM;
  int* mI1 = (int*)(mL2 + W * BM);

  const int tid = threadIdx.x, lane = tid & 63;
  const int wave = __builtin_amdgcn_readfirstlane(tid >> 6);
  const int64_t row0 = (int64_t)blockIdx.x * BM;
  const int rows = (int)min<int64_t>(BM, n - row0);
  const CenterParams P = *prm;
  if (!P.ok) {
    if (tid < rows) list[atomicAdd(listCount, 1u)] = (int32_t)(row0 + tid);
    return;
  }
  {
    constexpr int PER = BM * CH / 256;
    const uint4* src = Xq + row0 * CH;
    const int lim = rows * CH;
    v4u st[PER];
#pragma unroll
    for (int i = 0; i < PER; ++i)
      st[i] = __builtin_nontemporal_load((const v4u*)(src + min(tid + 256 * i, lim - 1)));
#pragma unroll
    for (int i = 0; i < PER; ++i) {
      const int e = tid + 256 * i, r = e / CH, ch = e - r * CH;
      As[r * STR + ch] = e < lim ? make_uint4(st[i].x, st[i].y, st[i].z, st[i].w)
                                 : make_uint4(0u, 0u, 0u, 0u);
    }
    if (tid < BM) exS[tid] = tid < rows ? meta[row0 + tid].x : INT_MIN;
  }
  __syncthreads();

  float F1[16];
#pragma unroll
  for (int ta = 0; ta < 4; ++ta) {
#pragma unroll
    for (int r = 0; r < 4; ++r) {
      const int ex = exS[ta * 16 + 4 * (lane >> 4) + r];
      F1[4 * ta + r] = ex == INT_MIN ? 0.0f : __builtin_ldexpf(1.0f, ex + P.ec - 20);
    }
  }
  float sL1[16], sL2[16];
  int sI1[16];
#pragma unroll
  for (int q = 0; q < 16; ++q) {
    sL1[q] = sL2[q] = __builtin_inff();
    sI1[q] = -1;
  }
  const uint4* ap = As + (lane & 15) * STR + (lane >> 4);
  const int nT = ktp / W;
  const uint4* cb = Cb + (size_t)wave * KS * 192 + lane;
  const size_t tstride = (size_t)W * KS * 192;
  v4i B0[3], B1[3], A0[3], A1[3];
#define CYC_LDB(DST, P)                                  \
  do {                                                   \
    DST[0] = as_v4i((P)[0]);                             \
    DST[1] = as_v4i((P)[64]);                            \
    DST[2] = as_v4i((P)[128]);                           \
  } while (0)
#define CYC_LDA(DST, KS_, TA_)                           \
  do {                                                   \
    const uint4* a_ = ap + (TA_) * 16 * STR + (KS_) * 4; \
    DST[0] = as_v4i(a_[0]);                              \
    DST[1] = as_v4i(a_[4 * KS]);                         \
    DST[2] = as_v4i(a_[8 * KS]);                         \
  } while (0)
#define CYC_MM(ACC, A, B)                                                    \
  do {                                                                       \
    ACC[0] = __builtin_amdgcn_mfma_i32_16x16x64_i8(A[0], B[0], ACC[0], 0, 0, 0); \
    ACC[1] = __builtin_amdgcn_mfma_i32_16x16x64_i8(A[0], B[1], ACC[1], 0, 0, 0); \
    ACC[1] = __builtin_amdgcn_mfma_i32_16x16x64_i8(A[1], B[0], ACC[1], 0, 0, 0); \
    ACC[2] = __builtin_amdgcn_mfma_i32_16x16x64_i8(A[0], B[2], ACC[2], 0, 0, 0); \
    ACC[2] = __builtin_amdgcn_mfma_i32_16x16x64_i8(A[1], B[1], ACC[2], 0, 0, 0); \
    ACC[2] = __builtin_amdgcn_mfma_i32_16x16x64_i8(A[2], B[0], ACC[2], 0, 0, 0); \
  } while (0)
#define CYC_TA(KS_, TA_, AC, AN, BC)                                          \
  do {                                                                        \
    if ((TA_) < 3) CYC_LDA(AN, KS_, (TA_) + 1);                               \
    else CYC_LDA(AN, ((KS_) + 1 < KS ? (KS_) + 1 : 0), 0);                    \
    CYC_MM(acc[TA_], AC, BC);                                                 \
    __builtin_amdgcn_sched_group_barrier(0x100, 3, 0);                        \
    __builtin_amdgcn_sched_group_barrier(0x008, 6, 0);                        \
  } while (0)
#define CYC_KSTEP(KS_, BC, BN)                                                \
  do {                                                                        \
    CYC_LDB(BN, ((KS_) + 1 < KS ? cb + ((KS_) + 1) * 192 : cbn));             \
    __builtin_amdgcn_sched_group_barrier(0x020, 3, 0);                        \
    CYC_TA(KS_, 0, A0, A1, BC);                                               \
    CYC_TA(KS_, 1, A1, A0, BC);                                               \
    CYC_TA(KS_, 2, A0, A1, BC);                                               \
    CYC_TA(KS_, 3, A1, A0, BC);                                               \
  } while (0)
  CYC_LDB(B0, cb);
  CYC_LDA(A0, 0, 0);

  __builtin_amdgcn_s_setreg(0x801, 2);
  for (int t = 0; t < nT; ++t) {
    const float cqv = cq[(t * W + wave) * 16 + (lane & 15)];
    const uint4* cbn = cb + (t + 1 < nT ? tstride : 0);
    v4i acc[4][3];
#pragma unroll
    for (int ta = 0; ta < 4; ++ta)
#pragma unroll
      for (int s = 0; s < 3; ++s) acc[ta][s] = v4i{0, 0, 0, 0};
#pragma unroll
    for (int kp = 0; kp < KS; kp += 2) {
      CYC_KSTEP(kp, B0, B1);
      CYC_KSTEP(kp + 1, B1, B0);
    }
#undef CYC_KSTEP
#undef CYC_TA
#undef CYC_MM
#undef CYC_LDA
#undef CYC_LDB
    cb = cbn;
    const int c = (t * W + wave) * 16 + (lane & 15);
#pragma unroll
    for (int ta = 0; ta < 4; ++ta) {
#pragma unroll
      for (int r = 0; r < 4; ++r) {
        const int q = 4 * ta + r;
        const int T = acc[ta][0][r] * 128 + acc[ta][1][r];
        const float V = __builtin_fmaf((float)acc[ta][2][r], 0x1p-7f, (float)T);
        const float L = __builtin_fmaf(-F1[q], V, cqv);
        const bool lt = L < sL1[q];
        sL2[q] = __builtin_amdgcn_fmed3f(sL1[q], sL2[q], L);
        sI1[q] = lt ? c : sI1[q];
        sL1[q] = __builtin_fminf(sL1[q], L);
      }
    }
  }
  __builtin_amdgcn_s_setreg(0x801, 0);

#pragma unroll
  for (int q = 0; q < 16; ++q) {
#pragma unroll
    for (int m = 1; m < 16; m <<= 1) {
      const float oL1 = __shfl_xor(sL1[q], m), oL2 = __shfl_xor(sL2[q], m);
      const int oI1 = __shfl_xor(sI1[q], m);
      sL2[q] = __builtin_fminf(__builtin_fmaxf(sL1[q], oL1), __builtin_fminf(sL2[q], oL2));
      const bool take = oL1 < sL1[q] || (oL1 == sL1[q] && oI1 >= 0 && (sI1[q] < 0 || oI1 < sI1[q]));
      sI1[q] = take ? oI1 : sI1[q];
      sL1[q] = take ? oL1 : sL1[q];
    }
  }
  __syncthreads();
  if ((lane & 15) == 0) {
#pragma unroll
    for (int ta = 0; ta < 4; ++ta) {
#pragma unroll
      for (int r = 0; r < 4; ++r) {
        const int q = 4 * ta + r, row = ta * 16 + 4 * (lane >> 4) + r;
        mL1[wave * BM + row] = sL1[q];
        mL2[wave * BM + row] = sL2[q];
        mI1[wave * BM + row] = sI1[q];
      }
    }
  }
  __syncthreads();
  if (tid < rows) {
    const int row = tid;
    const int ex = exS[row];
    float L1 = __builtin_inff(), L2 = __builtin_inff();
    int I1 = -1;
#pragma unroll
    for (int w = 0; w < W; ++w) {
      const float oL1 = mL1[w * BM + row], oL2 = mL2[w * BM + row];
      const int oI1 = mI1[w * BM + row];
      L2 = __builtin_fminf(__builtin_fmaxf(L1, oL1), __builtin_fminf(L2, oL2));
      if (oL1 < L1 || (oL1 == L1 && oI1 >= 0 && (I1 < 0 || oI1 < I1))) {
        L1 = oL1;
        I1 = oI1;
      }
    }
    bool decided = false;
    if (ex != INT_MIN && I1 >= 0 && __builtin_isfinite(L1)) {
      const double xn = xnorm[row0 + row], cn = cnorm[I1];
      const double xx = xn * xn, cc = cn * cn;
      const double n1 = (double)__int_as_float(meta[row0 + row].y);
      const double fx = err_term(ex, n1, P.mu, d);
      const double l1 = (double)L1;
      const double M = (4.0 * (fx + g[I1]) + 2.0 * kEpsF * (xx + cc) +
                        0x1p-20 * (__builtin_fabs(l1) + cc + 2.0 * g[I1]) +
                        0x1p-24 * (2.0 * (xx + cc) + __builtin_fabs(l1) +
                                   __builtin_fmin(__builtin_fabs((double)L2), 0x1p120)) +
                        0x1p-90) *
                       (1.0 + 0x1p-30);
      decided = !__builtin_isfinite(L2) || ((double)L2 - l1) > M;
    }
    if (decided) {
      assign[row0 + row] = I1;
    } else {
      list[atomicAdd(listCount, 1u)] = (int32_t)(row0 + row);
    }
  }
}


__device__ __forceinline__ double err_term2(int e, double n1, double mu, int d);
__device__ __forceinline__ double err_term1(int e, double n1, double mu);
__global__ __launch_bounds__(256) void k_centers_pack32(
    const double* __restrict__ C, const double* __restrict__ cnorm, int k, int d, int S, int ktp,
    const double* __restrict__ cn1, const CenterParams* __restrict__ prm, uint4* __restrict__ Cb,
    float* __restrict__ cq, double* __restrict__ g, float* __restrict__ cq2,
    double* __restrict__ g2, float* __restrict__ cq1, double* __restrict__ g1) {
  const CenterParams p = *prm;
  const int64_t idx = (int64_t)blockIdx.x * blockDim.x + threadIdx.x;
  const int64_t total = (int64_t)ktp * S * 64;
  if (idx < total) {
    const int lane = (int)(idx & 63);
    const int64_t t = idx >> 6;
    const int s = (int)(t % S), ct = (int)(t / S);
    const int c = ct * 32 + (lane & 31), j0 = s * 32 + 16 * (lane >> 5);
    int a[16], b[16], cc[16];
#pragma unroll
    for (int e = 0; e < 16; ++e) {
      const int j = j0 + e;
      const double v = (p.ok && c < k && j < d) ? C[(int64_t)c * d + j] : 0.0;
      quant3(v, p.ec, a[e], b[e], cc[e]);
    }
    uint4 pa, pb, pc;
    pa.x = pack4(a); pa.y = pack4(a + 4); pa.z = pack4(a + 8); pa.w = pack4(a + 12);
    pb.x = pack4(b); pb.y = pack4(b + 4); pb.z = pack4(b + 8); pb.w = pack4(b + 12);
    pc.x = pack4(cc); pc.y = pack4(cc + 4); pc.z = pack4(cc + 8); pc.w = pack4(cc + 12);
    uint4* dst = Cb + (t * 3) * 64 + lane;
    dst[0] = pa;
    dst[64] = pb;
    dst[128] = pc;
    uint4* cr = Cb + (int64_t)ktp * S * 3 * 64 + (int64_t)c * (6 * S) + 2 * s + (lane >> 5);
    cr[0] = pa;
    cr[2 * S] = pb;
    cr[4 * S] = pc;
  }
  if (idx < (int64_t)ktp * 32) {
    const int c = (int)idx;
    if (c < k && p.ok) {
      const double gc = err_term(p.ec, cn1[c], p.mu, d);
      const double gc2 = err_term2(p.ec, cn1[c], p.mu * 0x1p-7, d);
      const double gc1 = err_term1(p.ec, cn1[c], p.mu * 0x1p-14);
      const double cn = cnorm[c];
      g[c] = gc;
      cq[c] = fdown((cn * cn) * (1.0 - kEpsF) - 2.0 * gc);
      g2[c] = gc2;
      cq2[c] = fdown((cn * cn) * (1.0 - kEpsF) - 2.0 * gc2);
      g1[c] = gc1;
      cq1[c] = fdown((cn * cn) * (1.0 - kEpsF) - 2.0 * gc1);
    } else {
      g[c] = g2[c] = g1[c] = 0.0;
      cq[c] = __builtin_inff();
      cq2[c] = cq1[c] = 0x1.fffffep127f;
    }
  }
}

typedef int v16i __attribute__((ext_vector_type(16)));

__device__ __forceinline__ double err_term1(int e, double n1, double mu) {
  const double A = __builtin_ldexp(1.0078125, e - 8);
  return (0.5 * mu * A * A + 0.5 * n1 * n1 / mu) * (1.0 + 0x1p-40);
}

__device__ __forceinline__ double err_term2(int e, double n1, double mu, int d) {
  const double A = __builtin_ldexp(1.0078125, e - 15);
  const double kd = 0.502 * (double)d * 0x1p14;
  return (0.5 * mu * A * A + 0.5 * n1 * n1 / mu + kd * A * A) * (1.0 + 0x1p-40);
}

__device__ __forceinline__ double bnd_ub_sq(double xx, double cc, double l1, double fx, double gw,
                                            double enc) {
  return (xx + l1 + enc + 2.0 * fx + 4.0 * gw + 2.0 * kEpsF * (xx + cc) +
          0x1p-20 * (xx + __builtin_fabs(l1) + cc + 2.0 * gw) + 0x1p-90) *
         (1.0 + 0x1p-30);
}
__device__ __forceinline__ double bnd_lb_sq(double xx, double l, double fx, double enc,
                                            double extra) {
  return xx + l - enc - 2.0 * fx - 2.0 * kEpsF * xx -
         0x1p-20 * (xx + __builtin_fabs(l) + 2.0 * fx + enc) - extra;
}
__device__ __forceinline__ float bnd_dist_up(double s2) {
  return fup(__builtin_sqrt(s2) * (1.0 + 0x1p-50));
}
__device__ __forceinline__ float bnd_dist_dn(double s2) {
  return s2 > 0.0 ? fdown(__builtin_sqrt(s2) * (1.0 - 0x1p-50)) : -1.0f;
}
__device__ __forceinline__ void rows_max32(int (&v)[16], int lane, int* out) {
#pragma unroll
  for (int lev = 0; lev < 4; ++lev) {
    const int half = 8 >> lev, m = 16 >> lev;
    const bool hi = (lane & m) != 0;
#pragma unroll
    for (int i = 0; i < half; ++i) {
      const int o = __shfl_xor(hi ? v[i] : v[i + half], m);
      v[i] = max(hi ? v[i + half] : v[i], o);
    }
  }
  v[0] = max(v[0], __shfl_xor(v[0], 1));
  if ((lane & 1) == 0) {
    const int q = (lane >> 1) & 15;
    out[(q & 3) + 8 * (q >> 2) + 4 * (lane >> 5)] = v[0];
  }
}

constexpr int kShMax = 2;

template <int S, int W, int LIMBS, bool LIST>
__global__ __launch_bounds__(64 * W, W == 8 ? 2 : (LIMBS < 3 ? 12 : 8) / W) void k_screen32(
    const uint4* __restrict__ Xq, const int2* __restrict__ meta, const double* __restrict__ xnorm,
    int64_t n, int d, const uint4* __restrict__ Cb, const float* __restrict__ cq,
    const double* __restrict__ g, const double* __restrict__ cnorm,
    const CenterParams* __restrict__ prm, int ktp, const int32_t* __restrict__ rowsIn,
    const unsigned int* __restrict__ rowsInCount, int32_t* __restrict__ assign,
    int32_t* __restrict__ list, unsigned int* __restrict__ listCount,
    int32_t* __restrict__ candRows, int32_t* __restrict__ cands,
    unsigned int* __restrict__ candCount, unsigned int scap, float2* __restrict__ bnd) {
  constexpr int D = 32 * S, CH = 3 * D / 16;
  constexpr bool PAIR = LIMBS == 1;
  constexpr int FR = PAIR ? 2 * S : LIMBS * S;
  constexpr int TB = FR * 1024 + 256;
  constexpr int G = FR / W;
  static_assert(FR % W == 0, "fragments split evenly over the waves");
  __shared__ __attribute__((aligned(16))) char lds[3 * TB];
  const int lane = threadIdx.x & 63, r = lane & 31, h = lane >> 5;
  const int wave = __builtin_amdgcn_readfirstlane(threadIdx.x >> 6);
  const CenterParams P = *prm;
  const double mu = LIMBS == 3 ? P.mu : LIMBS == 2 ? P.mu * 0x1p-7 : P.mu * 0x1p-14;
  constexpr int SH = LIMBS == 1 ? 13 : 20;
  constexpr int CMAX = LIMBS == 1 ? kCand1 : kCandMax;
  const int64_t total = LIST ? (int64_t)*rowsInCount : n;
  auto group = [&](int64_t grp) {
  const int64_t pos0 = (grp * W + wave) * 32;
  const int rows = (int)max<int64_t>(0, min<int64_t>(32, total - pos0));
  const unsigned shard = (unsigned)((grp * W + wave) % kShards);
  int32_t* const listS = scap ? list + (size_t)shard * scap : list;
  unsigned int* const listCountS = scap ? listCount + shard * kShardStride : listCount;
  int32_t* const candRowsS = scap && candRows ? candRows + (size_t)shard * scap : candRows;
  int32_t* const candsS = scap && cands ? cands + (size_t)shard * scap * CMAX : cands;
  unsigned int* const candCountS =
      scap && candCount ? candCount + shard * kShardStride : candCount;
  auto rowAt = [&](int i) -> int64_t {
    if constexpr (LIST) return rowsIn[pos0 + i];
    else return pos0 + i;
  };
  if (!P.ok) {
    if (lane < rows) {
      listS[atomicAdd(listCountS, 1u)] = (int32_t)rowAt(lane);
      if (LIMBS == 1 && bnd) bnd[rowAt(lane)] = make_float2(-1.0f, -1.0f);
    }
    return;
  }
  const int nsteps = PAIR ? ktp / 2 : ktp;
  auto issue = [&](int t, int slot) {
    if constexpr (PAIR && (CYC_PROBE_MODE & 2)) return;
    const int tt = t < nsteps ? t : nsteps - 1;
    char* dst = lds + slot * TB;
#pragma unroll
    for (int j = 0; j < FR / W; ++j) {
      const int f = wave + W * j;
      const int tile = PAIR ? 2 * tt + f / S : tt;
      const int piece = PAIR ? (f % S) * 3 : (f / LIMBS) * 3 + f % LIMBS;
      const char* src = (const char*)Cb + (size_t)tile * (3 * S) * 1024 + lane * 16;
      __builtin_amdgcn_global_load_lds((const void*)(src + piece * 1024),
                                       (__attribute__((address_space(3))) void*)(dst + f * 1024),
                                       16, 0, 0);
    }
    if (wave == 0)
      __builtin_amdgcn_global_load_lds(
          (const void*)(cq + (PAIR ? (size_t)tt * 64 + lane : (size_t)tt * 32 + r)),
          (__attribute__((address_space(3))) void*)(dst + FR * 1024), 4, 0, 0);
  };
  issue(0, 0);
  issue(1, 1);
  v4i A[S][LIMBS];
  const bool rowOk = r < rows;
  const int64_t myRow = rowOk ? rowAt(r) : 0;
  {
    const bool ok = rowOk;
    const uint4* src = Xq + ((PAIR && (CYC_PROBE_MODE & 8)) ? 0 : myRow) * CH + h;
#pragma unroll
    for (int s = 0; s < S; ++s)
#pragma unroll
      for (int L = 0; L < LIMBS; ++L) {
        const v4u* a = (const v4u*)(src + L * (D / 16) + 2 * s);
        const v4u t = PAIR ? *a : __builtin_nontemporal_load(a);
        A[s][L] = ok ? __builtin_bit_cast(v4i, t) : v4i{0, 0, 0, 0};
      }
  }
  const int exr = rowOk ? meta[myRow].x : INT_MIN;
  float F1[16];
  int sh[16];
  int exmin = 0;
  if constexpr (LIMBS == 3) {
    const float f = exr == INT_MIN ? 0.0f : __builtin_ldexpf(1.0f, exr + P.ec - 20);
#pragma unroll
    for (int reg = 0; reg < 16; ++reg) F1[reg] = __shfl(f, (reg & 3) + 8 * (reg >> 2) + 4 * h);
  } else {
    int e = exr == INT_MIN ? INT_MAX : exr;
#pragma unroll
    for (int m = 1; m < 32; m <<= 1) e = min(e, __shfl_xor(e, m));
    exmin = __builtin_amdgcn_readfirstlane(e == INT_MAX ? 0 : e);
    const int s0 = exr == INT_MIN ? 31 : min(exr - exmin, 31);
#pragma unroll
    for (int reg = 0; reg < 16; ++reg) sh[reg] = __shfl(s0, (reg & 3) + 8 * (reg >> 2) + 4 * h);
  }
  const float qscale = __builtin_ldexpf(1.0f, max(-160, min(160, SH - P.ec - exmin)));
  constexpr float QCLAMP = LIMBS == 1 ? 0x1p25f : 0x1p30f;
// ... 1218 lines not shown
        if (decided) {
          const double L = (double)lnc0, tau = 0x1p-29 * (xx + dp->cmax2) + 0x1p-48 * (L * L + ub2);
          decided = lnc0 >= 0.0f && !dp->bad && L * L - ub2 > tau;
        }
        if (decided) {
          const float ub = bnd_dist_up(ub2);
          const float lb = __builtin_isfinite(l2)
                               ? bnd_dist_dn(bnd_lb_sq(xx, l2, fx, 0.0, 0x1p-20 * (double)cqMax))
                               : __builtin_inff();
          bnd[row] = ub < 0x1p120f ? make_float2(ub, __builtin_fminf(lb, lnc0))
                                   : make_float2(-1.0f, -1.0f);
          if (nbrMode && ub < 0x1p120f) {
            lncA[row] = lnc0;
#pragma unroll
            for (int i = 0; i < kCandMax; ++i)
              sets[(size_t)row * kCandMax + i] = nbr[(size_t)a0 * kCandMax + i];
          }
        }
      }
      if (decided) assign[row] = I1;
      state[row] = decided ? 0 : 1;
      if (failList && !decided) rank = atomicAdd(&sFail, 1u);
    }
    if (failList) {
      __syncthreads();
      if (t == 0 && sFail) {
        sFailBase = atomicAdd(failCount, sFail);
        atomicAdd(failCum, (unsigned long long)sFail);
      }
      __syncthreads();
      if (rank != ~0u) failList[sFailBase + rank] = row;
    }
    __syncthreads();
  }
}

template <int S>
int launch_cands3(const CandArgs& ca, const void* img, const int2* meta, const double* xnorm,
                  int64_t n, int d, const void* Cb, const float* cq, const double* g,
                  const double* cnorm, const CenterParams* prm, int ktp, int32_t* assign,
                  int32_t* outRows, int32_t* outCands, unsigned int* outCount, hipStream_t st,
                  unsigned int scap, const Bounds* bd = nullptr) {
  KernelTimer timer("k_kmeans_cands3", st);
  const unsigned grid = (unsigned)std::max<int64_t>(1, std::min<int64_t>((n + 127) / 128, 4096));
  const uint4* Cr = (const uint4*)Cb + (size_t)ktp * S * 3 * 64;
  hipLaunchKernelGGL(HIP_KERNEL_NAME(k_screen_cands3<S, 16>), dim3(grid), dim3(256), 0, st,
                     (const uint4*)img, meta, xnorm, d, Cr, cq, g, cnorm, prm,
                     (const int32_t*)ca.candRows, (const int32_t*)ca.cands,
                     (const unsigned int*)ca.candCount, assign, outRows, outCands, outCount, scap,
                     bd ? bd->ub_lb : nullptr, bd ? bd->lnc : nullptr, bd ? bd->sets : nullptr,
                     nullptr, nullptr, nullptr, nullptr);
  CYC_LAUNCH_CHECK("k_screen_cands3");
  return CYC_OK;
}

int launch_cands(const CandArgs& ca, int64_t n, int d, int32_t* assign, int32_t* list,
                 unsigned int* listCount, hipStream_t st, unsigned int scap = 0) {
  KernelTimer timer("k_kmeans_cands", st);
  const unsigned grid = (unsigned)std::max<int64_t>(1, std::min<int64_t>((n + 127) / 128, 4096));
  hipLaunchKernelGGL(k_screen_cands, dim3(grid), dim3(256), 0, st, ca.X, ca.xnorm, d, ca.C,
                     ca.cnorm, ca.k, ca.unit, ca.margin, (const int32_t*)ca.candRows, (const int32_t*)ca.cands,
                     (const unsigned int*)ca.candCount, assign, list, listCount, scap);
  CYC_LAUNCH_CHECK("k_screen_cands");
  return CYC_OK;
}

struct CompactJob {
  unsigned int* counts;
  const int32_t* src;
  int32_t* dst;
  int width;
  const int32_t* src2;
  int32_t* dst2;
  int width2;
  unsigned int* dstCount;
};
constexpr int kMaxCompactJobs = 4;
struct CompactJobs {
  CompactJob j[kMaxCompactJobs];
};
__device__ __forceinline__ void shard_compact(const CompactJob& J, unsigned int cap) {
  __shared__ unsigned sb[2];
  const int j = blockIdx.y;
  unsigned int* counts = J.counts;
  if (threadIdx.x < 64) {
    const int l = threadIdx.x;
    const unsigned c = counts[l * kShardStride];
    unsigned incl = c;
#pragma unroll
    for (int m = 1; m < kShards; m <<= 1) {
      const unsigned o = __shfl_up(incl, m);
      if (l >= m) incl += o;
    }
    if (l == j) {
      sb[0] = incl - c;
      sb[1] = c;
    }
  }
  const unsigned old = *J.dstCount;
  __syncthreads();
  if (J.dst) {
    const size_t base = (size_t)old + sb[0], c = sb[1];
    const size_t t0 = (size_t)blockIdx.x * blockDim.x + threadIdx.x;
    const size_t stride = (size_t)gridDim.x * blockDim.x;
    const int32_t* s1 = J.src + (size_t)j * cap * J.width;
    int32_t* d1 = J.dst + base * J.width;
    for (size_t i = t0; i < c * J.width; i += stride) d1[i] = s1[i];
    if (J.src2) {
      const int32_t* s2 = J.src2 + (size_t)j * cap * J.width2;
      int32_t* d2 = J.dst2 + base * J.width2;
      for (size_t i = t0; i < c * J.width2; i += stride) d2[i] = s2[i];
    }
  }
  __syncthreads();
  if (threadIdx.x == 0) {
    const unsigned blocks = gridDim.x * gridDim.y;
    if (atomicAdd(&counts[3], 1u) == blocks - 1) {
      unsigned tot = 0;
      for (int l = 0; l < kShards; ++l) {
        tot += counts[l * kShardStride];
        counts[l * kShardStride] = 0u;
      }
      *J.dstCount = old + tot;
      counts[3] = 0u;
    }
  }
}
__global__ __launch_bounds__(256) void k_shard_compact(CompactJobs jobs, unsigned int cap) {
  shard_compact(jobs.j[blockIdx.z], cap);
}

int compact_jobs(const CompactJob* jobs, int nj, unsigned int cap, hipStream_t st) {
  if (nj <= 0) return CYC_OK;
  KernelTimer timer("k_kmeans_compact", st);
  CompactJobs J{};
  bool anyDst = false;
  for (int i = 0; i < nj; ++i) {
    J.j[i] = jobs[i];
    anyDst = anyDst || jobs[i].dst;
  }
  hipLaunchKernelGGL(k_shard_compact, anyDst ? dim3(2, kShards, nj) : dim3(1, 1, nj), dim3(256), 0,
                     st, J, cap);
  CYC_LAUNCH_CHECK("k_shard_compact");
  return CYC_OK;
}

int compact(unsigned int* counts, unsigned int cap, const int32_t* src, int32_t* dst, int width,
            const int32_t* src2, int32_t* dst2, int width2, unsigned int* dstCount,
            hipStream_t st) {
  const CompactJob j{counts, src, dst, width, src2, dst2, width2, dstCount};
  return compact_jobs(&j, 1, cap, st);
}

struct ZeroArgs {
  unsigned int* p[8];
  int w[8];
  int n;
};
__global__ __launch_bounds__(256) void k_zero_counters(ZeroArgs z) {
  unsigned int* q = z.p[blockIdx.x];
  for (int i = threadIdx.x; i < z.w[blockIdx.x]; i += 256) q[i] = 0u;
}

template <int S, int W>
int screen32(const void* img, const int2* meta, const double* xnorm, int64_t n, int d,
             const void* Cb, const float* cq, const double* g, const double* cnorm,
             const CenterParams* prm, int ktp, int32_t* assign, int32_t* list,
             unsigned int* listCount, int32_t* list2, unsigned int* list2Count,
             const CandArgs* ca, hipStream_t st, const RefineArgs* ra = nullptr,
             const AppendStage* stg = nullptr, const Bounds* bd = nullptr) {
  const AppendStage* sg = ca ? stg : nullptr;
  const unsigned scap = sg ? sg->cap : 0u;
  {
    ZeroArgs z{};
    auto add = [&](unsigned int* q, int words) {
      if (q) {
        z.p[z.n] = q;
        z.w[z.n++] = words;
      }
    };
    add(list2Count, 1);
    if (ca) {
      add(ca->candCount, 1);
      add(ca->candCount2, 1);
    }
    if (ra && ca) {
      add(ra->cand1Count, 1);
      add(ra->fullCount, 2);
    }
    add(sg ? sg->counts : nullptr, kSets * kShards * kShardStride);
    if (z.n) {
      hipLaunchKernelGGL(k_zero_counters, dim3(z.n), dim3(256), 0, st, z);
      CYC_LAUNCH_CHECK("k_zero_counters");
    }
  }
  auto A = [&](int32_t* staged, int32_t* direct) { return sg ? staged : direct; };
  auto N = [&](int set, unsigned int* direct) { return sg ? sg->set(set) : direct; };
  int rc;
  auto compact2 = [&]() -> int {
    if (!sg) return CYC_OK;
    const CompactJob jb[2] = {
        {sg->set(kSetRowsA), sg->rowsA, list2, 1, nullptr, nullptr, 0, list2Count},
        {sg->set(kSetCand), sg->candRows, ca->candRows, 1, sg->cands, ca->cands, kCandMax,
         ca->candCount}};
    return compact_jobs(jb, 2, scap, st);
  };
  if (ra && ca) {
    if (bd && bd->rcRows) {
      {
        KernelTimer timer("k_kmeans_recheck", st);
        static const bool onePhase = [] {
          const char* e = std::getenv("CYC_KMEANS_RECHECK");
          return e && e[0] == '1';
        }();
        if (onePhase) {
          const unsigned grid = (unsigned)std::max<int64_t>(1, std::min<int64_t>((n + 127) / 128, 4096));
          hipLaunchKernelGGL(HIP_KERNEL_NAME(k_screen_cands3<S, 16, true>), dim3(grid), dim3(256), 0,
                             st, (const uint4*)img, meta, xnorm, d,
                             (const uint4*)Cb + (size_t)ktp * S * 3 * 64, cq, g, cnorm, prm,
                             bd->rcRows, (const int32_t*)bd->sets, bd->rcCount, assign, nullptr,
                             nullptr, nullptr, 0u, bd->ub_lb, bd->lnc, bd->sets, bd->state, bd->dp,
                             bd->nbr, bd->nbrR);
          CYC_LAUNCH_CHECK("k_screen_cands3 (re-check)");
        } else {
          const unsigned grid = (unsigned)std::max<int64_t>(
              1, std::min<int64_t>((n + kRcBatch - 1) / kRcBatch, 2048));
          hipLaunchKernelGGL(HIP_KERNEL_NAME(k_recheck<S>), dim3(grid), dim3(kRcBatch), 0, st,
                             (const uint4*)img, meta, xnorm, d,
                             (const uint4*)Cb + (size_t)ktp * S * 3 * 64, cq, g, cnorm, prm,
                             bd->rcRows, bd->rcCount, assign, bd->ub_lb, bd->lnc, bd->sets,
                             bd->state, bd->dp, bd->nbr, bd->nbrR,
                             bd->collected ? bd->list : nullptr,
                             bd->collected ? bd->listCount : nullptr,
                             bd->collected ? bd->cum : nullptr);
          CYC_LAUNCH_CHECK("k_recheck");
        }
      }
      if (bd->dump) dump_dev("state_rc", bd->state, (size_t)bd->n, st);
      if (!(bd->collected && recheck_two_phase()) && (rc = bounds_collect(*bd, st))) return rc;
    }
    if (bd && bd->rowsIn)
      rc = launch_screen32<S, W, 1, true>(
          img, meta, xnorm, n, d, Cb, cq + (size_t)ktp * 64, g + (size_t)ktp * 64, cnorm, prm,
          ktp, bd->rowsIn, bd->rowsInCount, assign, A(sg ? sg->rowsA : nullptr, ra->fullList),
          N(kSetRowsA, ra->fullCount), st, A(sg ? sg->candRows : nullptr, ra->cand1Rows),
          A(sg ? sg->cands : nullptr, ra->cand1), N(kSetCand, ra->cand1Count), scap, bd->ub_lb);
    else
      rc = launch_screen32<S, W, 1, false>(
          img, meta, xnorm, n, d, Cb, cq + (size_t)ktp * 64, g + (size_t)ktp * 64, cnorm, prm,
          ktp, nullptr, nullptr, assign, A(sg ? sg->rowsA : nullptr, ra->fullList),
          N(kSetRowsA, ra->fullCount), st, A(sg ? sg->candRows : nullptr, ra->cand1Rows),
          A(sg ? sg->cands : nullptr, ra->cand1), N(kSetCand, ra->cand1Count), scap,
          bd ? bd->ub_lb : nullptr);
    if (rc) return rc;
    if (sg) {
      const CompactJob jb[2] = {
          {sg->set(kSetRowsA), sg->rowsA, ra->fullList, 1, nullptr, nullptr, 0, ra->fullCount},
          {sg->set(kSetCand), sg->candRows, ra->cand1Rows, 1, sg->cands, ra->cand1, kCand1,
           ra->cand1Count}};
      if ((rc = compact_jobs(jb, 2, scap, st))) return rc;
    }
    {
      KernelTimer timer("k_kmeans_refine2", st);
      hipLaunchKernelGGL(HIP_KERNEL_NAME(k_screen32r<S>), dim3((unsigned)((n + 127) / 128)),
                         dim3(256), 0, st, (const uint4*)img, meta, xnorm, n, d, (const uint4*)Cb,
                         cq + (size_t)ktp * 32, g + (size_t)ktp * 32, cnorm, prm, ra->kstride,
                         (const int32_t*)ra->cand1Rows, (const unsigned int*)ra->cand1Count,
                         (const int32_t*)ra->cand1, assign, A(sg ? sg->rowsA : nullptr, list2),
                         N(kSetRowsA, list2Count), A(sg ? sg->candRows : nullptr, ca->candRows),
                         A(sg ? sg->cands : nullptr, ca->cands), N(kSetCand, ca->candCount),
                         A(sg ? sg->rowsB : nullptr, ra->fullList), N(kSetRowsB, ra->fullCount),
                         N(kSetStat, ra->fullCount + 1), scap, bd ? bd->ub_lb : nullptr);
      CYC_LAUNCH_CHECK("k_screen32r");
    }
    if (sg) {
      const CompactJob jb[4] = {
          {sg->set(kSetRowsA), sg->rowsA, list2, 1, nullptr, nullptr, 0, list2Count},
          {sg->set(kSetCand), sg->candRows, ca->candRows, 1, sg->cands, ca->cands, kCandMax,
           ca->candCount},
          {sg->set(kSetRowsB), sg->rowsB, ra->fullList, 1, nullptr, nullptr, 0, ra->fullCount},
          {sg->set(kSetStat), nullptr, nullptr, 0, nullptr, nullptr, 0, ra->fullCount + 1}};
      if ((rc = compact_jobs(jb, 4, scap, st))) return rc;
    }
    rc = launch_screen32<S, W, 2, true>(
        img, meta, xnorm, n, d, Cb, cq + (size_t)ktp * 32, g + (size_t)ktp * 32, cnorm, prm, ktp,
        ra->fullList, ra->fullCount, assign, A(sg ? sg->rowsA : nullptr, list2),
        N(kSetRowsA, list2Count), st, A(sg ? sg->candRows : nullptr, ca->candRows),
        A(sg ? sg->cands : nullptr, ca->cands), N(kSetCand, ca->candCount), scap);
  } else {
    rc = launch_screen32<S, W, 2, false>(
        img, meta, xnorm, n, d, Cb, cq + (size_t)ktp * 32, g + (size_t)ktp * 32, cnorm, prm, ktp,
        nullptr, nullptr, assign, A(sg ? sg->rowsA : nullptr, list2), N(kSetRowsA, list2Count),
        st, ca ? A(sg ? sg->candRows : nullptr, ca->candRows) : nullptr,
        ca ? A(sg ? sg->cands : nullptr, ca->cands) : nullptr,
        ca ? N(kSetCand, ca->candCount) : nullptr, scap);
  }
  if (rc || (rc = compact2())) return rc;
  if (!ca)
    return launch_screen32<S, W, 3, true>(img, meta, xnorm, n, d, Cb, cq, g, cnorm, prm, ktp,
                                          list2, list2Count, assign, list, listCount, st);
  CandArgs caF = *ca;
  if (ca->candRows2) {
    if ((rc = launch_cands3<S>(*ca, img, meta, xnorm, n, d, Cb, cq, g, cnorm, prm, ktp, assign,
                               A(sg ? sg->candRows : nullptr, ca->candRows2),
                               A(sg ? sg->cands : nullptr, ca->cands2),
                               N(kSetCand, ca->candCount2), st, scap, bd)))
      return rc;
    if (sg && (rc = compact(sg->set(kSetCand), scap, sg->candRows, ca->candRows2, 1, sg->cands,
                            ca->cands2, kCandMax, ca->candCount2, st)))
      return rc;
    caF.candRows = ca->candRows2;
    caF.cands = ca->cands2;
    caF.candCount = ca->candCount2;
  }
  static const bool sideStream = [] {
    const char* e = std::getenv("CYC_KMEANS_SIDE");
    return e && e[0] == '1';
  }();
  if (!sideStream) {
    if ((rc = launch_screen32<S, W, 3, true>(img, meta, xnorm, n, d, Cb, cq, g, cnorm, prm, ktp,
                                             list2, list2Count, assign,
                                             A(sg ? sg->rowsA : nullptr, list),
                                             N(kSetRowsA, listCount), st, nullptr, nullptr,
                                             nullptr, scap)) ||
        (rc = launch_cands(caF, n, d, assign, A(sg ? sg->rowsB : nullptr, list),
                           N(kSetRowsB, listCount), st, scap)))
      return rc;
  } else {
  constexpr int kMaxDev = 64;
  thread_local hipStream_t sides[kMaxDev] = {};
  thread_local hipEvent_t forks[kMaxDev] = {}, joins[kMaxDev] = {};
  int dev = 0;
  CYC_HIP(hipGetDevice(&dev));
  if (dev < 0 || dev >= kMaxDev) {
    cyc::set_error("device index out of range");
    return CYC_ERR_INVALID_ARG;
  }
  if (!sides[dev]) {
    CYC_HIP(hipStreamCreateWithFlags(&sides[dev], hipStreamNonBlocking));
    CYC_HIP(hipEventCreateWithFlags(&forks[dev], hipEventDisableTiming));
    CYC_HIP(hipEventCreateWithFlags(&joins[dev], hipEventDisableTiming));
  }
  hipStream_t side = sides[dev];
  hipEvent_t fork = forks[dev], join = joins[dev];
  CYC_HIP(hipEventRecord(fork, st));
  CYC_HIP(hipStreamWaitEvent(side, fork, 0));
  if ((rc = launch_screen32<S, W, 3, true>(img, meta, xnorm, n, d, Cb, cq, g, cnorm, prm, ktp,
                                           list2, list2Count, assign,
                                           A(sg ? sg->rowsA : nullptr, list),
                                           N(kSetRowsA, listCount), side, nullptr, nullptr,
                                           nullptr, scap)))
    return rc;
  rc = launch_cands(caF, n, d, assign, A(sg ? sg->rowsB : nullptr, list), N(kSetRowsB, listCount),
                    st, scap);
  CYC_HIP(hipEventRecord(join, side));
  CYC_HIP(hipStreamWaitEvent(st, join, 0));
  if (rc) return rc;
  }
  if (sg && ((rc = compact(sg->set(kSetRowsA), scap, sg->rowsA, list, 1, nullptr, nullptr, 0,
                           listCount, st)) ||
             (rc = compact(sg->set(kSetRowsB), scap, sg->rowsB, list, 1, nullptr, nullptr, 0,
                           listCount, st))))
    return rc;
  return CYC_OK;
}


__global__ __launch_bounds__(256) void k_center_drift(const double* __restrict__ C,
                                                      double* __restrict__ Cp, int k, int d,
                                                      double* __restrict__ delta,
                                                      double* __restrict__ ccs) {
  const int lane = threadIdx.x & 63;
  const int c = (blockIdx.x * blockDim.x + threadIdx.x) >> 6;
  if (c >= k) return;
  double s = 0.0, q = 0.0;
  for (int j = lane; j < d; j += 64) {
    const double v = C[(int64_t)c * d + j], o = Cp[(int64_t)c * d + j];
    const double t = v - o;
    s += t * t;
    q += v * v;
    Cp[(int64_t)c * d + j] = v;
  }
  s = wave_sum(s);
  q = wave_sum(q);
  if (lane == 0) {
    delta[c] = __builtin_sqrt(s) * (1.0 + 0x1p-40) + 0x1p-500;
    ccs[c] = q * (1.0 + 0x1p-40);
  }
}

__global__ __launch_bounds__(1024) void k_drift_top(const double* __restrict__ delta,
                                                    const double* __restrict__ ccs, int k,
                                                    DriftParams* __restrict__ prm) {
  __shared__ double s1[1024], s2[1024], sc[1024];
  __shared__ int si[1024];
  const int t = threadIdx.x;
  double d1 = 0.0, d2 = 0.0, cm = 0.0;
  int i1 = -1;
  bool bad = false;
  for (int c = t; c < k; c += 1024) {
    const double v = delta[c], q = ccs[c];
    bad = bad || !(v <= 0x1p1000) || !(q <= 0x1p1000);
    if (v > d1 || i1 < 0) {
      d2 = i1 < 0 ? 0.0 : d1;
      d1 = v;
      i1 = c;
    } else if (v > d2) {
      d2 = v;
    }
    cm = __builtin_fmax(cm, q);
  }
  s1[t] = d1;
  s2[t] = d2;
  si[t] = i1;
  sc[t] = cm;
  bad = __syncthreads_or(bad);
  for (int off = 512; off > 0; off >>= 1) {
    if (t < off && si[t + off] >= 0) {
      const double a1 = s1[t], a2 = s2[t], b1 = s1[t + off], b2 = s2[t + off];
      const bool aEmpty = si[t] < 0;
      if (aEmpty || b1 > a1) {
        s1[t] = b1;
        si[t] = si[t + off];
        s2[t] = aEmpty ? b2 : __builtin_fmax(a1, b2);
      } else {
        s2[t] = __builtin_fmax(a2, b1);
      }
      sc[t] = __builtin_fmax(sc[t], sc[t + off]);
    }
    __syncthreads();
  }
  if (t == 0) {
    DriftParams p;
    p.d1 = s1[0];
    p.d2 = s2[0];
    p.i1 = si[0];
    p.cmax2 = sc[0];
    p.bad = bad ? 1 : 0;
    *prm = p;
  }
}

constexpr int kBndIT = kBndRows / 256;
__device__ __forceinline__ void bnd_block_list(const unsigned long long (&masks)[kBndIT],
                                               unsigned* wc, int64_t base, int32_t* tmp,
                                               unsigned int* bcount,
                                               const unsigned long long* flips = nullptr) {
  const int tid = threadIdx.x, lane = tid & 63, wave = tid >> 6;
  __syncthreads();
  const unsigned long long below = (1ull << lane) - 1ull;
#pragma unroll
  for (int it = 0; it < kBndIT; ++it) {
    unsigned before = 0;
    for (int j = 0; j < it * 4 + wave; ++j) before += wc[j];
    if ((masks[it] >> lane) & 1ull)
      tmp[base + before + (unsigned)__builtin_popcountll(masks[it] & below)] =
          (flips && ((flips[it] >> lane) & 1ull)) ? ~(int32_t)(base + it * 256 + tid)
                                                  : (int32_t)(base + it * 256 + tid);
  }
  if (tid == 0) {
    unsigned total = 0;
    for (int j = 0; j < kBndIT * 4; ++j) total += wc[j];
    bcount[blockIdx.x] = total;
  }
}

__global__ __launch_bounds__(64) void k_center_nbrs(const double* __restrict__ stats, int k,
                                                    int32_t* __restrict__ nbr,
                                                    float* __restrict__ nbrR) {
  const int a = blockIdx.x, lane = threadIdx.x;
  constexpr int T = kCandMax;
  double v[T];
  int ix[T];
#pragma unroll
  for (int i = 0; i < T; ++i) {
    v[i] = INFINITY;
    ix[i] = -1;
  }
  for (int j = lane; j < k; j += 64) {
    if (j == a) continue;
    const int64_t pi = a <= j ? (int64_t)j * (j + 1) / 2 + a : (int64_t)a * (a + 1) / 2 + j;
    double x = stats[pi];
    if (!(x >= 0.0)) x = INFINITY;
    if (x < v[T - 1]) {
      double cv = x;
      int ci = j;
#pragma unroll
      for (int i = 0; i < T; ++i) {
        const bool sw = cv < v[i];
        const double tv = v[i];
        const int ti = ix[i];
        v[i] = sw ? cv : v[i];
        ix[i] = sw ? ci : ix[i];
        cv = sw ? tv : cv;
        ci = sw ? ti : ci;
      }
    }
  }
  if (lane == 0) nbr[(int64_t)a * kCandMax] = a;
  for (int t = 0; t < T; ++t) {
    double bv = v[0];
    int bl = lane;
    for (int m = 32; m > 0; m >>= 1) {
      const double ov = __shfl_xor(bv, m);
      const int ol = __shfl_xor(bl, m);
      if (ov < bv || (ov == bv && ol < bl)) {
        bv = ov;
        bl = ol;
      }
    }
    const int bi = __shfl(ix[0], bl);
    if (lane == bl) {
#pragma unroll
      for (int i = 0; i < T - 1; ++i) {
        v[i] = v[i + 1];
        ix[i] = ix[i + 1];
      }
      v[T - 1] = INFINITY;
      ix[T - 1] = -1;
    }
    if (lane == 0) {
      if (t < T - 1) {
        nbr[(int64_t)a * kCandMax + 1 + t] = bv < INFINITY ? bi : -1;
      } else {
        nbrR[a] = bv < INFINITY ? fdown(__builtin_sqrt(4.0 * bv) * (1.0 - 0x1p-40))
                                : __builtin_inff();
      }
    }
  }
}

__global__ __launch_bounds__(256) void k_bounds_filter(const int32_t* __restrict__ assign,
                                                       float2* __restrict__ bnd,
                                                       float* __restrict__ lnc,
                                                       unsigned char* __restrict__ state,
                                                       const double* __restrict__ xnorm,
                                                       int64_t n, int k,
                                                       const double* __restrict__ delta,
                                                       const DriftParams* __restrict__ prm,
                                                       int32_t* __restrict__ tmp,
                                                       unsigned int* __restrict__ bcount,
                                                       const float* __restrict__ nbrR,
                                                       int32_t* __restrict__ tmp2,
                                                       unsigned int* __restrict__ bcount2) {
  __shared__ unsigned wc[kBndIT * 4], wc2[kBndIT * 4];
  unsigned long long masks2[kBndIT];
  const DriftParams P = *prm;
  unsigned long long flips[kBndIT];
  const int tid = threadIdx.x, lane = tid & 63, wave = tid >> 6;
  const int64_t base = (int64_t)blockIdx.x * kBndRows;
  unsigned long long masks[kBndIT];
#pragma unroll
  for (int it = 0; it < kBndIT; ++it) {
    const int64_t r = base + it * 256 + tid;
    int st = 1;
    if (r < n) {
      const int a = assign[r];
      const float2 b = bnd[r];
      const float ln = lnc[r];
      const bool okA = !P.bad && a >= 0 && a < k;
      if (okA && b.x >= 0.0f && b.y > 0.0f) {
        const double U = (double)b.x + delta[a];
        const double L = (double)b.y - (a == P.i1 ? P.d2 : P.d1);
        const double xr = U + __builtin_sqrt(P.cmax2);
        const double xx = xr * xr * (1.0 + 0x1p-50);
        const double U2 = U * U, L2 = L * L;
        const double tau = 0x1p-29 * (xx + P.cmax2) + 0x1p-48 * (L2 + U2) + 0x1p-1000;
        if (L > 0.0 && (L2 - U2) > tau) {
          st = 0;
          bnd[r] = make_float2(fup(U * (1.0 + 0x1p-50)), fdown(L * (1.0 - 0x1p-50)));
        }
      }
      const double Ln = ln >= 0.0f && okA ? ((double)ln - P.d1) * (1.0 - 0x1p-50) : -1.0;
      const double Um = okA && b.x >= 0.0f ? (double)b.x + delta[a] : 0.0;
      if (st == 1 && Ln > 0.0 && Ln > Um) st = 2;
      if (st == 1 && nbrR && okA) {
        const double R = (double)nbrR[a];
        if (R > 0.0 && R > 2.0 * Um && (b.x >= 0.0f || delta[a] < 0.125 * R)) st = 3;
      }
      if (st == 1 && Ln > 0.0) st = 2;
      if (ln >= 0.0f)
        lnc[r] = (st == 0 || st == 2) && Ln > 0.0 ? fdown(Ln) : -1.0f;
      state[r] = (unsigned char)st;
    }
    masks[it] = __builtin_amdgcn_ballot_w64(st >= 2);
    flips[it] = __builtin_amdgcn_ballot_w64(st == 3);
    masks2[it] = __builtin_amdgcn_ballot_w64(r < n && st == 1);
    if (lane == 0) {
      wc[it * 4 + wave] = (unsigned)__builtin_popcountll(masks[it]);
      wc2[it * 4 + wave] = (unsigned)__builtin_popcountll(masks2[it]);
    }
  }
  bnd_block_list(masks, wc, base, tmp, bcount, flips);
  if (tmp2) bnd_block_list(masks2, wc2, base, tmp2, bcount2);
}

__global__ __launch_bounds__(256) void k_bounds_collect(const unsigned char* __restrict__ state,
                                                        int64_t n, int32_t* __restrict__ tmp,
                                                        unsigned int* __restrict__ bcount) {
  __shared__ unsigned wc[kBndIT * 4];
  const int tid = threadIdx.x, lane = tid & 63, wave = tid >> 6;
  const int64_t base = (int64_t)blockIdx.x * kBndRows;
  unsigned long long masks[kBndIT];
#pragma unroll
  for (int it = 0; it < kBndIT; ++it) {
    const int64_t r = base + it * 256 + tid;
    masks[it] = __builtin_amdgcn_ballot_w64(r < n && state[r] == 1);
    if (lane == 0) wc[it * 4 + wave] = (unsigned)__builtin_popcountll(masks[it]);
  }
  bnd_block_list(masks, wc, base, tmp, bcount);
}

__global__ __launch_bounds__(1024) void k_bounds_scan(unsigned int* __restrict__ bcount, int64_t nb,
                                                      unsigned int* __restrict__ listCount,
                                                      unsigned long long* __restrict__ cum,
                                                      unsigned int* __restrict__ bcount2 = nullptr,
                                                      unsigned int* __restrict__ listCount2 = nullptr,
                                                      unsigned long long* __restrict__ cum2 = nullptr) {
  __shared__ unsigned part[1024];
  if (blockIdx.x == 1) {
    bcount = bcount2;
    listCount = listCount2;
    cum = cum2;
  }
  const int t = threadIdx.x;
  const int64_t per = (nb + 1023) / 1024;
  const int64_t a = min<int64_t>(nb, t * per), e = min<int64_t>(nb, a + per);
  unsigned s = 0;
  for (int64_t i = a; i < e; ++i) s += bcount[i];
  part[t] = s;
  __syncthreads();
  for (int off = 1; off < 1024; off <<= 1) {
    const unsigned v = t >= off ? part[t - off] : 0u;
    __syncthreads();
    part[t] += v;
    __syncthreads();
  }
  unsigned run = t ? part[t - 1] : 0u;
  for (int64_t i = a; i < e; ++i) {
    const unsigned c = bcount[i];
    bcount[i] = run;
    run += c;
  }
  if (t == 1023) {
    bcount[nb] = part[1023];
    *listCount = part[1023];
    if (cum) *cum += (unsigned long long)part[1023];
  }
}

__global__ __launch_bounds__(256) void k_bounds_scatter(const int32_t* __restrict__ tmp,
                                                        const unsigned int* __restrict__ off,
                                                        int32_t* __restrict__ list,
                                                        const int32_t* __restrict__ tmp2 = nullptr,
                                                        const unsigned int* __restrict__ off2 = nullptr,
                                                        int32_t* __restrict__ list2 = nullptr) {
  if (blockIdx.y == 1) {
    tmp = tmp2;
    off = off2;
    list = list2;
  }
  const int64_t b = blockIdx.x;
  const unsigned o = off[b], c = off[b + 1] - o;
  for (unsigned i = threadIdx.x; i < c; i += 256) list[o + i] = tmp[b * kBndRows + i];
}

template <int KS>
int launch_screen(const void* img, const int2* meta, const double* xnorm, int64_t n, int d,
                  const void* Cb, const float* cq, const double* g, const double* cnorm,
                  const CenterParams* prm, int ktp, int32_t* assign, int32_t* list,
                  unsigned int* listCount, hipStream_t st) {
  constexpr int STR = 12 * KS + 2;
  const size_t lds = (size_t)kBM * STR * 16 + (size_t)kBM * 4;
  static bool attr = false;
  if (!attr) {
    CYC_HIP(hipFuncSetAttribute(reinterpret_cast<const void*>(&k_screen<KS>),
                                hipFuncAttributeMaxDynamicSharedMemorySize, (int)lds));
    attr = true;
  }
  KernelTimer timer("k_kmeans_screen3", st);
  hipLaunchKernelGGL(HIP_KERNEL_NAME(k_screen<KS>), dim3((unsigned)((n + kBM - 1) / kBM)),
                     dim3(256), lds, st, (const uint4*)img, meta, xnorm, n, d, (const uint4*)Cb,
                     cq, g, cnorm, prm, ktp, assign, list, listCount);
  CYC_LAUNCH_CHECK("k_kmeans_screen_i8");
  return CYC_OK;
}

}

int rows_quantize(const double* X, int64_t n, int d, void* img, int2* meta, hipStream_t st,
                  const double* scale, double* unorm) {
  if (n <= 0) return CYC_OK;
  const int D = 64 * ksteps(d);
  const int64_t blocks = std::min<int64_t>((n + 3) / 4, 65536);
  const int vec = (d % 2 == 0) && (reinterpret_cast<uintptr_t>(X) % 16 == 0);
  static const bool pf = [] {
    const char* e = std::getenv("CYC_QUANT_PF");
    return !(e && e[0] == '0');
  }();
  const bool q4 = d % 4 == 0 && reinterpret_cast<uintptr_t>(X) % 32 == 0;
  if (q4 && pf && d <= 256)
    hipLaunchKernelGGL(k_rows_quantize_q4, dim3((unsigned)blocks), dim3(256), 0, st, X, n, d, D,
                       (unsigned*)img, meta, scale, unorm);
  else if (vec && pf && d <= 256)
    hipLaunchKernelGGL(HIP_KERNEL_NAME(k_rows_quantize_pf<2>), dim3((unsigned)blocks), dim3(256), 0,
                       st, X, n, d, D, (unsigned*)img, meta, scale, unorm);
  else if (vec && pf)
    hipLaunchKernelGGL(HIP_KERNEL_NAME(k_rows_quantize_pf<4>), dim3((unsigned)blocks), dim3(256), 0,
                       st, X, n, d, D, (unsigned*)img, meta, scale, unorm);
  else
    hipLaunchKernelGGL(k_rows_quantize, dim3((unsigned)blocks), dim3(256), 0, st, X, n, d, D,
                       (unsigned*)img, meta, scale, unorm, vec);
  CYC_LAUNCH_CHECK("k_rows_quantize");
  return CYC_OK;
}

int centers_prepare(const double* C, const double* cnorm, int k, int d, int ktp, void* Cb,
                    float* cq, double* g, CenterParams* prm, double* scratch, hipStream_t st) {
  const int KS = ksteps(d);
  double* cmax = scratch;
  double* cn1 = scratch + k;
  hipLaunchKernelGGL(k_centers_scan, dim3((unsigned)((k + 3) / 4)), dim3(256), 0, st, C, k, d,
                     cmax, cn1);
  CYC_LAUNCH_CHECK("k_centers_scan");
  hipLaunchKernelGGL(k_centers_params, dim3(1), dim3(256), 0, st, k, (const double*)cmax,
                     (const double*)cn1, prm);
  CYC_LAUNCH_CHECK("k_centers_params");
  if (uses32(d)) {
    const int ktp32 = tiles32(k), S = 2 * KS;
    const int64_t total = std::max<int64_t>((int64_t)ktp32 * S * 64, (int64_t)ktp32 * 32);
    hipLaunchKernelGGL(k_centers_pack32, dim3((unsigned)((total + 255) / 256)), dim3(256), 0, st,
                       C, cnorm, k, d, S, ktp32, (const double*)cn1, (const CenterParams*)prm,
                       (uint4*)Cb, cq, g, cq + (size_t)ktp * 16, g + (size_t)ktp * 16,
                       cq + (size_t)ktp * 32, g + (size_t)ktp * 32);
    CYC_LAUNCH_CHECK("k_centers_pack32");
    return CYC_OK;
  }
  const int64_t total = std::max<int64_t>((int64_t)ktp * KS * 64, (int64_t)ktp * 16);
  hipLaunchKernelGGL(k_centers_pack, dim3((unsigned)((total + 255) / 256)), dim3(256), 0, st, C,
                     cnorm, k, d, KS, ktp, (const double*)cn1, (const CenterParams*)prm,
                     (uint4*)Cb, cq, g);
  CYC_LAUNCH_CHECK("k_centers_pack");
  return CYC_OK;
}

int centers_drift(const double* C, double* Cp, int k, int d, double* delta, double* ccs,
                  DriftParams* prm, hipStream_t st) {
  hipLaunchKernelGGL(k_center_drift, dim3((unsigned)((k + 3) / 4)), dim3(256), 0, st, C, Cp, k, d,
                     delta, ccs);
  CYC_LAUNCH_CHECK("k_center_drift");
  hipLaunchKernelGGL(k_drift_top, dim3(1), dim3(1024), 0, st, (const double*)delta,
                     (const double*)ccs, k, prm);
  CYC_LAUNCH_CHECK("k_drift_top");
  return CYC_OK;
}

int bounds_filter(const int32_t* assign, float2* ub_lb, float* lnc, unsigned char* state,
                  const double* xnorm, int64_t n, int k, const double* delta,
                  const DriftParams* prm, int32_t* tmp, unsigned int* bcount, int32_t* rcList,
                  unsigned int* rcCount, unsigned long long* rcCum, const double* stats,
                  int32_t* nbr, float* nbrR, hipStream_t st, int32_t* tmp2,
                  unsigned int* bcount2, int32_t* list1, unsigned int* list1Count,
                  unsigned long long* cum1) {
  const int64_t nb = bounds_blocks(n);
  const bool two = tmp2 && bcount2 && list1 && list1Count;
  if (nb <= 0) return CYC_OK;
  KernelTimer timer("k_kmeans_bounds", st);
  if (stats) {
    hipLaunchKernelGGL(k_center_nbrs, dim3((unsigned)k), dim3(64), 0, st, stats, k, nbr, nbrR);
    CYC_LAUNCH_CHECK("k_center_nbrs");
  }
  hipLaunchKernelGGL(k_bounds_filter, dim3((unsigned)nb), dim3(256), 0, st, assign, ub_lb, lnc,
                     state, xnorm, n, k, delta, prm, tmp, bcount,
                     stats ? (const float*)nbrR : nullptr, two ? tmp2 : nullptr,
                     two ? bcount2 : nullptr);
  CYC_LAUNCH_CHECK("k_bounds_filter");
  hipLaunchKernelGGL(k_bounds_scan, dim3(two ? 2 : 1), dim3(1024), 0, st, bcount, nb, rcCount,
                     rcCum, two ? bcount2 : nullptr, two ? list1Count : nullptr,
                     two ? cum1 : nullptr);
  CYC_LAUNCH_CHECK("k_bounds_scan");
  hipLaunchKernelGGL(k_bounds_scatter, dim3((unsigned)nb, two ? 2 : 1), dim3(256), 0, st,
                     (const int32_t*)tmp, (const unsigned int*)bcount, rcList,
                     two ? (const int32_t*)tmp2 : nullptr,
                     two ? (const unsigned int*)bcount2 : nullptr, two ? list1 : nullptr);
  CYC_LAUNCH_CHECK("k_bounds_scatter");
  return CYC_OK;
}

bool recheck_two_phase() {
  static const bool two = [] {
    const char* e = std::getenv("CYC_KMEANS_RECHECK");
    return !(e && e[0] == '1');
  }();
  return two;
}

int bounds_collect(const Bounds& bd, hipStream_t st) {
  const int64_t nb = bounds_blocks(bd.n);
  if (nb <= 0) return CYC_OK;
  hipLaunchKernelGGL(k_bounds_collect, dim3((unsigned)nb), dim3(256), 0, st,
                     (const unsigned char*)bd.state, bd.n, bd.tmp, bd.bcount);
  CYC_LAUNCH_CHECK("k_bounds_collect");
  hipLaunchKernelGGL(k_bounds_scan, dim3(1), dim3(1024), 0, st, bd.bcount, nb, bd.listCount,
                     bd.cum);
  CYC_LAUNCH_CHECK("k_bounds_scan");
  hipLaunchKernelGGL(k_bounds_scatter, dim3((unsigned)nb), dim3(256), 0, st,
                     (const int32_t*)bd.tmp, (const unsigned int*)bd.bcount, bd.list);
  CYC_LAUNCH_CHECK("k_bounds_scatter");
  return CYC_OK;
}

int screen(const void* img, const int2* meta, const double* xnorm, int64_t n, int d,
           const void* Cb, const float* cq, const double* g, const double* cnorm,
           const CenterParams* prm, int ktp, int32_t* assign, int32_t* list,
           unsigned int* listCount, int32_t* list2, unsigned int* list2Count, hipStream_t st,
           const CandArgs* ca, const RefineArgs* ra, const AppendStage* stg,
           const Bounds* bd) {
  if (n <= 0) return CYC_OK;
  if (stg && stg->cap < shard_cap(n)) {
    set_error("append stage smaller than shard_cap(n)");
    return CYC_ERR_INVALID_ARG;
  }
  if (bd && !(ra && ca && uses32(d))) {
    set_error("carried bounds need the one-limb pass (d <= 256, refinement, candidate pass)");
    return CYC_ERR_INVALID_ARG;
  }
  if (uses32(d)) {
    const int k32 = ktp * 16 / 32;
    switch (ksteps(d)) {
      case 2: return screen32<4, 4>(img, meta, xnorm, n, d, Cb, cq, g, cnorm, prm, k32, assign, list, listCount, list2, list2Count, ca, st, ra, stg, bd);
      default: return screen32<8, 4>(img, meta, xnorm, n, d, Cb, cq, g, cnorm, prm, k32, assign, list, listCount, list2, list2Count, ca, st, ra, stg, bd);
    }
  }
  switch (ksteps(d)) {
#define CYC_S8(K) \
  case K: return launch_screen<K>(img, meta, xnorm, n, d, Cb, cq, g, cnorm, prm, ktp, assign, list, listCount, st);
    CYC_S8(2) CYC_S8(4) CYC_S8(6) CYC_S8(8)
#undef CYC_S8
    default:
      set_error("the i8 screen supports d <= 512");
      return CYC_ERR_UNSUPPORTED;
  }
}

}
}
```

### cycloneml_amd/csrc/kmeans_i8.hpp

```cpp
#pragma once

#include <hip/hip_runtime.h>

#include <cstdint>

namespace cyc {
namespace km8 {

constexpr int kMaxD = 512;
constexpr int kBM = 64;
constexpr int kWaves = 4;

struct CenterParams {
  int ec;
  int ok;
  double mu;
  int k;
};

inline int ksteps(int d) { return ((d + 127) / 128) * 2; }

inline bool uses32(int d) { return d <= 256; }
inline int tiles32(int k) { return 2 * ((k + 63) / 64); }

inline int64_t image_row_bytes(int d) { return 3 * 64 * (int64_t)ksteps(d); }

int rows_quantize(const double* X, int64_t n, int d, void* img, int2* meta, hipStream_t st,
                  const double* scale = nullptr, double* unorm = nullptr);

int centers_prepare(const double* C, const double* cnorm, int k, int d, int ktp, void* Cb,
                    float* cq, double* g, CenterParams* prm, double* scratch, hipStream_t st);

constexpr int kCandMax = 6;
constexpr int kCand1 = 8;
struct CandArgs {
  const double* X;
  const double* xnorm;
  const double* C;
  const double* cnorm;
  int k;
  bool unit;
  double margin;
  int32_t* candRows;
  int32_t* cands;
  unsigned int* candCount;
  int32_t* candRows2 = nullptr;
  int32_t* cands2 = nullptr;
  unsigned int* candCount2 = nullptr;
};

struct RefineArgs {
  int kstride;
  int32_t* cand1Rows;
  int32_t* cand1;
  unsigned int* cand1Count;
  int32_t* fullList;
  unsigned int* fullCount;
};

constexpr int kShards = 64;
constexpr int kShardStride = 64;
enum { kSetRowsA = 0, kSetRowsB = 1, kSetCand = 2, kSetStat = 3, kSets = 4 };
struct AppendStage {
  int32_t* rowsA;
  int32_t* rowsB;
  int32_t* candRows;
  int32_t* cands;
  unsigned int* counts;
  unsigned int cap;
  unsigned int* set(int s) const { return counts + (size_t)s * kShards * kShardStride; }
};
inline unsigned int shard_cap(int64_t n) {
  return (unsigned int)((n + 32 * kShards - 1) / (32 * kShards) * 32 + 2048);
}
int compact(unsigned int* counts, unsigned int cap, const int32_t* src, int32_t* dst, int width,
            const int32_t* src2, int32_t* dst2, int width2, unsigned int* dstCount,
            hipStream_t st);

struct DriftParams {
  double d1, d2;
  double cmax2;
  int i1;
  int bad;
};
struct Bounds {
  float2* ub_lb;
  const int32_t* rowsIn;
  const unsigned int* rowsInCount;
  float* lnc = nullptr;
  int32_t* sets = nullptr;
  unsigned char* state = nullptr;
  const int32_t* rcRows = nullptr;
  const unsigned int* rcCount = nullptr;
  const DriftParams* dp = nullptr;
  const int32_t* nbr = nullptr;
  const float* nbrR = nullptr;
  int dump = 0;
  bool collected = false;
  int32_t* tmp = nullptr;
  unsigned int* bcount = nullptr;
  int32_t* list = nullptr;
  unsigned int* listCount = nullptr;
  unsigned long long* cum = nullptr;
  int64_t n = 0;
};
int centers_drift(const double* C, double* Cp, int k, int d, double* delta, double* ccs,
                  DriftParams* prm, hipStream_t st);
constexpr int kBndRows = 2048;
inline int64_t bounds_blocks(int64_t n) { return (n + kBndRows - 1) / kBndRows; }
int bounds_filter(const int32_t* assign, float2* ub_lb, float* lnc, unsigned char* state,
                  const double* xnorm, int64_t n, int k, const double* delta,
                  const DriftParams* prm, int32_t* tmp, unsigned int* bcount, int32_t* rcList,
                  unsigned int* rcCount, unsigned long long* rcCum, const double* stats,
                  int32_t* nbr, float* nbrR, hipStream_t st, int32_t* tmp2 = nullptr,
                  unsigned int* bcount2 = nullptr, int32_t* list1 = nullptr,
                  unsigned int* list1Count = nullptr, unsigned long long* cum1 = nullptr);
bool recheck_two_phase();

int bounds_collect(const Bounds& bd, hipStream_t st);

int screen(const void* img, const int2* meta, const double* xnorm, int64_t n, int d,
           const void* Cb, const float* cq, const double* g, const double* cnorm,
           const CenterParams* prm, int ktp, int32_t* assign, int32_t* list,
           unsigned int* listCount, int32_t* list2, unsigned int* list2Count, hipStream_t st,
           const CandArgs* ca = nullptr,
           const RefineArgs* ra = nullptr, const AppendStage* stg = nullptr,
           const Bounds* bd = nullptr);

}
}
```

Before: 13.36 billion.

## Fuse per-iteration center preparation kernels into a single batched prep launch

Moves the bodies of the stats, transpose, require-norms, centers-scan and related kernels into device helpers. A new prep_all path feeds them into one centers_prepare_all call that also zeroes the screen counters and computes drift and neighbours. The goal is to cut the many small kernel launches and memsets that run each training iteration before assignment. The cost is a more complex dispatch path, gated by prep_fused() and the i8 width check, which adds correctness risk around counter zeroing and the nbrsReady ordering.

```diff
diff --git a/cycloneml_amd/csrc/kmeans.hip b/cycloneml_amd/csrc/kmeans.hip
--- a/cycloneml_amd/csrc/kmeans.hip
+++ b/cycloneml_amd/csrc/kmeans.hip
@@ -72,9 +72,9 @@
   Ct[idx] = (i < k && j < d) ? C[(int64_t)i * d + j] : 0.0;
 }
 
-constexpr unsigned long long kInfBits = 0x7FF0000000000000ull;
-constexpr int kStT = 32;
-constexpr int kStC = 32;
+using cyc::kmc::kInfBits;
+using cyc::kmc::kStT;
+using cyc::kmc::kStC;
 
 __global__ void k_fill_u64(unsigned long long* __restrict__ p, int n, unsigned long long v) {
   const int i = blockIdx.x * blockDim.x + threadIdx.x;
@@ -83,88 +83,21 @@
 __global__ void k_center_transpose_fill(const double* __restrict__ C, int k, int d, int d4,
                                         int kpad, double* __restrict__ Ct,
                                         unsigned long long* __restrict__ p, unsigned long long v) {
-  const int64_t idx = (int64_t)blockIdx.x * blockDim.x + threadIdx.x;
-  if (idx < k) p[idx] = v;
-  const int64_t total = (int64_t)d4 * kpad;
-  if (idx >= total) return;
-  const int j = (int)(idx / kpad), i = (int)(idx % kpad);
-  Ct[idx] = (i < k && j < d) ? C[(int64_t)i * d + j] : 0.0;
+  cyc::kmc::center_transpose_fill(C, k, d, d4, kpad, Ct, p, v, blockIdx.x, threadIdx.x);
 }
 __global__ void k_zero2(unsigned int* __restrict__ a, unsigned int* __restrict__ b) {
-  if (threadIdx.x == 0) *a = 0u;
-  if (threadIdx.x == 1 && b) *b = 0u;
+  cyc::kmc::zero2(a, b, threadIdx.x);
 }
 
 __global__ __launch_bounds__(256) void k_stats_pairs(const double* __restrict__ C, int k, int d,
                                                      int tps, double* __restrict__ packed,
                                                      unsigned long long* __restrict__ dmin) {
-  __shared__ double Ci[kStT][kStC + 1], Cj[kStT][kStC + 1];
-  __shared__ unsigned long long rmin[kStT], cmin[kStT];
-  int t = blockIdx.x, bi = 0;
-  while (t >= tps - bi) {
-    t -= tps - bi;
-    ++bi;
-  }
-  const int bj = bi + t;
-  const int tx = threadIdx.x & 15, ty = threadIdx.x >> 4;
-  if (threadIdx.x < kStT) rmin[threadIdx.x] = cmin[threadIdx.x] = kInfBits;
-  double s00 = 0.0, s01 = 0.0, s10 = 0.0, s11 = 0.0;
-  for (int c0 = 0; c0 < d; c0 += kStC) {
-    __syncthreads();
-    for (int e = threadIdx.x; e < kStT * kStC; e += 256) {
-      const int r = e >> 5, cc = e & 31, col = c0 + cc;
-      const int gi = bi * kStT + r, gj = bj * kStT + r;
-      Ci[r][cc] = (gi < k && col < d) ? C[(int64_t)gi * d + col] : 0.0;
-      Cj[r][cc] = (gj < k && col < d) ? C[(int64_t)gj * d + col] : 0.0;
-    }
-    __syncthreads();
-    const int lim = min(kStC, d - c0);
-    for (int cc = 0; cc < lim; ++cc) {
-      const double a0 = Ci[ty][cc], a1 = Ci[ty + 16][cc];
-      const double b0 = Cj[tx][cc], b1 = Cj[tx + 16][cc];
-      double q = dsub(a0, b0);
-      s00 = dadd(s00, dmul(q, q));
-      q = dsub(a0, b1);
-      s01 = dadd(s01, dmul(q, q));
-      q = dsub(a1, b0);
-      s10 = dadd(s10, dmul(q, q));
-      q = dsub(a1, b1);
-      s11 = dadd(s11, dmul(q, q));
-    }
-  }
-  const double sv[2][2] = {{s00, s01}, {s10, s11}};
-#pragma unroll
-  for (int a = 0; a < 2; ++a) {
-#pragma unroll
-    for (int b = 0; b < 2; ++b) {
-      const int i = bi * kStT + ty + 16 * a, j = bj * kStT + tx + 16 * b;
-      if (i < k && j < k && j > i) {
-        const double dist = __builtin_sqrt(sv[a][b]);
-        const double v = dmul(dmul(0.25, dist), dist);
-        packed[iut(i, j)] = v;
-        const unsigned long long bits = (unsigned long long)__double_as_longlong(v);
-        atomicMin(&rmin[ty + 16 * a], bits);
-        atomicMin(&cmin[tx + 16 * b], bits);
-      }
-    }
-  }
-  __syncthreads();
-  if (threadIdx.x < kStT) {
-    const int i = bi * kStT + threadIdx.x, j = bj * kStT + threadIdx.x;
-    if (i < k && rmin[threadIdx.x] != kInfBits) atomicMin(&dmin[i], rmin[threadIdx.x]);
-    if (j < k && cmin[threadIdx.x] != kInfBits) atomicMin(&dmin[j], cmin[threadIdx.x]);
-  }
+  cyc::kmc::stats_pairs(C, k, d, tps, packed, dmin, blockIdx.x, threadIdx.x);
 }
 
 __global__ void k_stats_diag(int k, double* __restrict__ packed,
                              const unsigned long long* __restrict__ dmin) {
-  const int i = blockIdx.x * blockDim.x + threadIdx.x;
-  if (i >= k) return;
-  if (k == 1) {
-    packed[0] = __builtin_nan("");
-    return;
-  }
-  packed[iut(i, i)] = __longlong_as_double((long long)dmin[i]);
+  cyc::kmc::stats_diag(k, packed, dmin, kInfBits, blockIdx.x, threadIdx.x);
 }
 
 struct Slot {
@@ -1075,16 +1008,7 @@
 __global__ void k_require_norms(const double* __restrict__ C, int k, int d,
                                 const double* __restrict__ xnorm, int64_t n,
                                 unsigned long long* __restrict__ req) {
-  const int64_t stride = (int64_t)gridDim.x * blockDim.x;
-  const int64_t t0 = (int64_t)blockIdx.x * blockDim.x + threadIdx.x;
-  const int64_t kd = (int64_t)k * d;
-  for (int64_t i = t0; i < kd; i += stride)
-    if (__builtin_isnan(C[i])) atomicMin(&req[0], (unsigned long long)(i / d));
-  for (int64_t r = t0; r < n; r += stride)
-    if (__builtin_isnan(xnorm[r])) atomicMin(&req[1], (unsigned long long)r);
-  double* out = reinterpret_cast<double*>(req + 2);
-  if (t0 < 2 && t0 < k) out[t0] = seq_norm2(C + t0 * d, d);
-  if (t0 == 2) out[2] = n > 0 ? xnorm[0] : 0.0;
+  cyc::kmc::require_norms(C, k, d, xnorm, n, req, gridDim.x, blockIdx.x, threadIdx.x);
 }
 
 __global__ void k_hist(const int32_t* __restrict__ assign, int64_t n, int k,
@@ -2305,8 +2229,8 @@
   return off || cyc::strict_parity();
 }
 
-int bounds_prepare(cyc_kmeans_plan p, cyc_kmeans_rows rows, const double* C,
-                   const double* xnorm, int64_t n, hipStream_t st, cyc::km8::Bounds& bd) {
+int bounds_reserve(cyc_kmeans_plan p, cyc_kmeans_rows rows, int64_t n, hipStream_t st,
+                   bool& carry) {
   namespace k8 = cyc::km8;
   const int k = p->k, d = p->d;
   int rc;
@@ -2335,11 +2259,16 @@
     CYC_HIP(hipMemsetAsync(rows->bCum.ptr, 0, 8, st));
     CYC_HIP(hipMemsetAsync(rows->bRcCum.ptr, 0, 8, st));
   }
-  const bool carry = rows->bValid && rows->bk == k;
+  carry = rows->bValid && rows->bk == k;
   rows->bValid = false;
-  if ((rc = k8::centers_drift(C, (double*)rows->bCp.ptr, k, d, (double*)rows->bDelta.ptr,
-                              (double*)rows->bCcs.ptr, (k8::DriftParams*)rows->bPrm.ptr, st)))
-    return rc;
+  return CYC_OK;
+}
+
+int bounds_lists(cyc_kmeans_plan p, cyc_kmeans_rows rows, const double* xnorm, int64_t n,
+                 hipStream_t st, cyc::km8::Bounds& bd, bool carry, bool nbrsReady) {
+  namespace k8 = cyc::km8;
+  const int k = p->k;
+  int rc;
   bd = k8::Bounds{(float2*)rows->bnd.ptr, nullptr, nullptr};
   bd.lnc = (float*)rows->bLnc.ptr;
   bd.sets = (int32_t*)rows->bSets.ptr;
@@ -2363,7 +2292,7 @@
                                 two ? (int32_t*)rows->bTmp2.ptr : nullptr,
                                 two ? (unsigned int*)rows->bCount2.ptr : nullptr,
                                 two ? bd.list : nullptr, two ? bd.listCount : nullptr,
-                                two ? bd.cum : nullptr)))
+                                two ? bd.cum : nullptr, nbrsReady)))
       return rc;
     bd.collected = two;
     if (!nbrOff()) {
@@ -2394,6 +2323,18 @@
     rows->bFullRows += n;
   }
   return CYC_OK;
+}
+
+int bounds_prepare(cyc_kmeans_plan p, cyc_kmeans_rows rows, const double* C,
+                   const double* xnorm, int64_t n, hipStream_t st, cyc::km8::Bounds& bd) {
+  namespace k8 = cyc::km8;
+  bool carry = false;
+  int rc;
+  if ((rc = bounds_reserve(p, rows, n, st, carry)) ||
+      (rc = k8::centers_drift(C, (double*)rows->bCp.ptr, p->k, p->d, (double*)rows->bDelta.ptr,
+                              (double*)rows->bCcs.ptr, (k8::DriftParams*)rows->bPrm.ptr, st)))
+    return rc;
+  return bounds_lists(p, rows, xnorm, n, st, bd, carry, false);
 }
 
 int stage_args(cyc_kmeans_plan p, int64_t n, bool useCa, cyc::km8::AppendStage& sg, bool& use) {
@@ -2454,17 +2395,21 @@
 int do_assign(cyc_kmeans_plan p, const double* X, const double* xnorm, cyc_kmeans_rows rows,
               int64_t n, const double* C, const double* cnorm, int32_t* assign, double* cost,
               int64_t* n_exact_out, hipStream_t st, bool nostats = false,
-              const cyc::km8::Bounds* bd = nullptr, bool approxNorm = false) {
+              const cyc::km8::Bounds* bd = nullptr, bool approxNorm = false,
+              bool prepared = false) {
   const double* statsArg = nostats ? nullptr : (const double*)p->stats.ptr;
   const bool i8 = rows && rows->usable;
-  hipLaunchKernelGGL(k_zero2, dim3(1), dim3(64), 0, st, (unsigned int*)p->slowCount.ptr,
-                     i8 ? (unsigned int*)p->list3Count.ptr : nullptr);
-  CYC_LAUNCH_CHECK("k_zero2");
+  if (!prepared) {
+    hipLaunchKernelGGL(k_zero2, dim3(1), dim3(64), 0, st, (unsigned int*)p->slowCount.ptr,
+                       i8 ? (unsigned int*)p->list3Count.ptr : nullptr);
+    CYC_LAUNCH_CHECK("k_zero2");
+  }
   int rc = CYC_OK;
   const int32_t* rowList = nullptr;
   const unsigned int* rowCount = nullptr;
   if (i8) {
-    if ((rc = cyc::km8::centers_prepare(C, cnorm, p->k, p->d, p->ktp8, p->cb8.ptr,
+    if (!prepared &&
+        (rc = cyc::km8::centers_prepare(C, cnorm, p->k, p->d, p->ktp8, p->cb8.ptr,
                                         (float*)p->cq8.ptr, (double*)p->g8.ptr,
                                         (cyc::km8::CenterParams*)p->prm8.ptr,
                                         (double*)p->scr8.ptr, st)))
@@ -2484,7 +2429,7 @@
                                assign, (int32_t*)p->list3.ptr, (unsigned int*)p->list3Count.ptr,
                                (int32_t*)p->slowList.ptr, (unsigned int*)p->list8Count.ptr, st,
                                useCa ? &ca : nullptr, useRa ? &ra : nullptr,
-                               useSg ? &sg : nullptr, bd)))
+                               useSg ? &sg : nullptr, bd, prepared)))
       return rc;
     rowList = (const int32_t*)p->list3.ptr;
     rowCount = (const unsigned int*)p->list3Count.ptr;
@@ -2556,6 +2501,67 @@
                          hipMemcpyDeviceToHost, st));
   CYC_HIP(hipEventRecord(p->reqEv, st));
   return CYC_OK;
+}
+
+int prep_all(cyc_kmeans_plan p, cyc_kmeans_rows rows, const double* X, const double* xnorm,
+             int64_t n, const double* C, const double* cnorm, bool useBnd, bool carry,
+             hipStream_t st, bool statsOnly = false) {
+  namespace k8 = cyc::km8;
+  const int k = p->k, d = p->d;
+  int rc;
+  const size_t reqBytes = sizeof(unsigned long long) * (8 + (size_t)k);
+  if ((rc = p->req.reserve(reqBytes))) return rc;
+  if (!p->reqHost) CYC_HIP(hipHostMalloc((void**)&p->reqHost, 5 * sizeof(unsigned long long)));
+  if (!p->reqEv) CYC_HIP(hipEventCreateWithFlags(&p->reqEv, hipEventDisableTiming));
+  CYC_HIP(hipMemsetAsync(p->req.ptr, 0xff, reqBytes, st));
+  k8::PrepJobs J;
+  J.C = C;
+  J.cnorm = cnorm;
+  J.k = k;
+  J.d = d;
+  J.stats = (double*)p->stats.ptr;
+  J.dmin = (unsigned long long*)p->req.ptr + 8;
+  J.ct = p->dense_ok ? (double*)p->ct.ptr : nullptr;
+  J.d4 = p->d4;
+  J.kpad = p->kpad;
+  J.xnorm = xnorm;
+  J.n = n;
+  J.req = (unsigned long long*)p->req.ptr;
+  const int64_t work = std::max<int64_t>(n, (int64_t)k * d);
+  J.reqBlocks = (unsigned)std::max<int64_t>(1, std::min<int64_t>((work + 255) / 256, 2048));
+  if (useBnd) {
+    J.Cp = (double*)rows->bCp.ptr;
+    J.delta = (double*)rows->bDelta.ptr;
+    J.ccs = (double*)rows->bCcs.ptr;
+    J.dprm = (k8::DriftParams*)rows->bPrm.ptr;
+    if (carry && !nbrOff()) {
+      J.nbr = (int32_t*)rows->bNbr.ptr;
+      J.nbrR = (float*)rows->bNbrR.ptr;
+    }
+  }
+  const bool i8 = rows && rows->usable;
+  if (!statsOnly) {
+    J.zeroA = (unsigned int*)p->slowCount.ptr;
+    J.zeroB = i8 ? (unsigned int*)p->list3Count.ptr : nullptr;
+  }
+  if (i8 && !statsOnly) {
+    J.ktp = p->ktp8;
+    J.Cb = p->cb8.ptr;
+    J.cq = (float*)p->cq8.ptr;
+    J.g = (double*)p->g8.ptr;
+    J.cprm = (k8::CenterParams*)p->prm8.ptr;
+    J.scratch = (double*)p->scr8.ptr;
+    k8::CandArgs ca;
+    k8::RefineArgs ra;
+    k8::AppendStage sg;
+    bool useCa = false, useRa = false, useSg = false;
+    if ((rc = cand_args(p, n, X, nullptr, C, cnorm, false, ca, useCa)) ||
+        (rc = refine_args(p, n, useCa, ra, useRa)) || (rc = stage_args(p, n, useCa, sg, useSg)))
+      return rc;
+    J.zero = k8::screen_zero_args((unsigned int*)p->list8Count.ptr, useCa ? &ca : nullptr,
+                                  useRa ? &ra : nullptr, useSg ? &sg : nullptr);
+  }
+  return k8::centers_prepare_all(J, st, p->reqHost, p->reqEv);
 }
 
 int require_check(cyc_kmeans_plan p, int64_t n, const double* Xrow0 = nullptr) {
@@ -3033,6 +3039,9 @@
     if ((rc = cos_enqueue(p, cn, p->k >= 2, nullptr, 0, st))) return rc;
     if (p->dense_ok && (rc = cos_transpose(p, C, st))) return rc;
     if ((rc = cos_stats(p, C, cn, st))) return rc;
+  } else if (cyc::km8::prep_fused()) {
+    if ((rc = prep_all(p, nullptr, nullptr, nullptr, 0, C, nullptr, false, false, st, true)))
+      return rc;
   } else {
     if ((rc = require_enqueue(p, C, nullptr, 0, st))) return rc;
     if ((rc = do_stats(p, C, st))) return rc;
@@ -3274,15 +3283,27 @@
         (rc = cos_assign(p, X, xnorm, rows, n, C, cnorm, assign, nullptr, nullptr, st, false)))
       return rc;
   } else {
-    if ((rc = require_enqueue(p, C, xnorm, n, st))) return rc;
-    if ((rc = do_stats(p, C, st))) return rc;
+    const bool fused = cyc::km8::prep_fused() &&
+                       (!(rows && rows->usable) || cyc::km8::uses32(d));
     cyc::km8::Bounds bd{};
-    if (useBnd) {
-      if ((rc = bounds_prepare(p, rows, C, xnorm, n, st, bd))) return rc;
-      assign = (int32_t*)rows->bAssign.ptr;
+    if (fused) {
+      bool carry = false;
+      if (useBnd && (rc = bounds_reserve(p, rows, n, st, carry))) return rc;
+      if ((rc = prep_all(p, rows, X, xnorm, n, C, cnorm, useBnd, carry, st))) return rc;
+      if (useBnd) {
+        if ((rc = bounds_lists(p, rows, xnorm, n, st, bd, carry, true))) return rc;
+        assign = (int32_t*)rows->bAssign.ptr;
+      }
+    } else {
+      if ((rc = require_enqueue(p, C, xnorm, n, st))) return rc;
+      if ((rc = do_stats(p, C, st))) return rc;
+      if (useBnd) {
+        if ((rc = bounds_prepare(p, rows, C, xnorm, n, st, bd))) return rc;
+        assign = (int32_t*)rows->bAssign.ptr;
+      }
     }
     if ((rc = do_assign(p, X, xnorm, rows, n, C, cnorm, assign, nullptr, nullptr, st, false,
-                        useBnd ? &bd : nullptr, approxNorm)))
+                        useBnd ? &bd : nullptr, approxNorm, fused)))
       return rc;
     if (useBnd) {
       rows->bValid = true;
diff --git a/cycloneml_amd/csrc/kmeans_i8.hip b/cycloneml_amd/csrc/kmeans_i8.hip
--- a/cycloneml_amd/csrc/kmeans_i8.hip
+++ b/cycloneml_amd/csrc/kmeans_i8.hip
@@ -321,11 +321,12 @@
   }
 }
 
-__global__ __launch_bounds__(256) void k_centers_scan(const double* __restrict__ C, int k, int d,
-                                                      double* __restrict__ cmax,
-                                                      double* __restrict__ cn1) {
-  const int lane = threadIdx.x & 63;
-  const int c = (blockIdx.x * blockDim.x + threadIdx.x) >> 6;
+__device__ __forceinline__ void d_centers_scan(const double* __restrict__ C, int k, int d,
+                                               double* __restrict__ cmax,
+                                               double* __restrict__ cn1, unsigned bid,
+                                               unsigned tid) {
+  const int lane = tid & 63;
+  const int c = (int)((bid * 256 + tid) >> 6);
   if (c >= k) return;
   double m = 0.0, s1 = 0.0;
   bool fin = true;
@@ -343,28 +344,33 @@
     cn1[c] = s1 * (1.0 + 0x1p-40);
   }
 }
-
-__global__ __launch_bounds__(256) void k_centers_params(int k, const double* __restrict__ cmax,
-                                                        const double* __restrict__ cn1,
-                                                        CenterParams* __restrict__ prm) {
+__global__ __launch_bounds__(256) void k_centers_scan(const double* __restrict__ C, int k, int d,
+                                                      double* __restrict__ cmax,
+                                                      double* __restrict__ cn1) {
+  d_centers_scan(C, k, d, cmax, cn1, blockIdx.x, threadIdx.x);
+}
+
+__device__ __forceinline__ void d_centers_params(int k, const double* __restrict__ cmax,
+                                                 const double* __restrict__ cn1,
+                                                 CenterParams* __restrict__ prm, unsigned tid) {
   __shared__ double sm[256], sn[256];
   double m = 0.0, nmax = 0.0;
-  for (int c = threadIdx.x; c < k; c += 256) {
+  for (int c = tid; c < k; c += 256) {
     m = __builtin_fmax(m, cmax[c]);
     nmax = __builtin_fmax(nmax, cn1[c]);
     if (!(cmax[c] <= 0x1p60)) m = __builtin_inf();
   }
-  sm[threadIdx.x] = m;
-  sn[threadIdx.x] = nmax;
+  sm[tid] = m;
+  sn[tid] = nmax;
   __syncthreads();
   for (int off = 128; off > 0; off >>= 1) {
-    if (threadIdx.x < off) {
-      sm[threadIdx.x] = __builtin_fmax(sm[threadIdx.x], sm[threadIdx.x + off]);
-      sn[threadIdx.x] = __builtin_fmax(sn[threadIdx.x], sn[threadIdx.x + off]);
+    if (tid < (unsigned)off) {
+      sm[tid] = __builtin_fmax(sm[tid], sm[tid + off]);
+      sn[tid] = __builtin_fmax(sn[tid], sn[tid + off]);
     }
     __syncthreads();
   }
-  if (threadIdx.x == 0) {
+  if (tid == 0) {
     const double gm = sm[0];
     const int ec = choose_exp(__builtin_isfinite(gm) ? gm : 0.0);
     CenterParams p;
@@ -376,6 +382,11 @@
     p.k = k;
     *prm = p;
   }
+}
+__global__ __launch_bounds__(256) void k_centers_params(int k, const double* __restrict__ cmax,
+                                                        const double* __restrict__ cn1,
+                                                        CenterParams* __restrict__ prm) {
+  d_centers_params(k, cmax, cn1, prm, threadIdx.x);
 }
 
 __global__ __launch_bounds__(256) void k_centers_pack(
@@ -632,13 +643,14 @@
 
 __device__ __forceinline__ double err_term2(int e, double n1, double mu, int d);
 __device__ __forceinline__ double err_term1(int e, double n1, double mu);
-__global__ __launch_bounds__(256) void k_centers_pack32(
+__device__ __forceinline__ void d_centers_pack32(
     const double* __restrict__ C, const double* __restrict__ cnorm, int k, int d, int S, int ktp,
     const double* __restrict__ cn1, const CenterParams* __restrict__ prm, uint4* __restrict__ Cb,
     float* __restrict__ cq, double* __restrict__ g, float* __restrict__ cq2,
-    double* __restrict__ g2, float* __restrict__ cq1, double* __restrict__ g1) {
+    double* __restrict__ g2, float* __restrict__ cq1, double* __restrict__ g1, unsigned bid,
+    unsigned tid) {
   const CenterParams p = *prm;
-  const int64_t idx = (int64_t)blockIdx.x * blockDim.x + threadIdx.x;
+  const int64_t idx = (int64_t)bid * 256 + tid;
   const int64_t total = (int64_t)ktp * S * 64;
   if (idx < total) {
     const int lane = (int)(idx & 63);
@@ -684,6 +696,14 @@
       cq2[c] = cq1[c] = 0x1.fffffep127f;
     }
   }
+}
+__global__ __launch_bounds__(256) void k_centers_pack32(
+    const double* __restrict__ C, const double* __restrict__ cnorm, int k, int d, int S, int ktp,
+    const double* __restrict__ cn1, const CenterParams* __restrict__ prm, uint4* __restrict__ Cb,
+    float* __restrict__ cq, double* __restrict__ g, float* __restrict__ cq2,
+    double* __restrict__ g2, float* __restrict__ cq1, double* __restrict__ g1) {
+  d_centers_pack32(C, cnorm, k, d, S, ktp, cn1, prm, Cb, cq, g, cq2, g2, cq1, g1, blockIdx.x,
+                   threadIdx.x);
 }
 
 typedef int v16i __attribute__((ext_vector_type(16)));
@@ -2208,14 +2228,12 @@
   return compact_jobs(&j, 1, cap, st);
 }
 
-struct ZeroArgs {
-  unsigned int* p[8];
-  int w[8];
-  int n;
-};
+__device__ __forceinline__ void d_zero_counters(const ZeroArgs& z, unsigned bid, unsigned tid) {
+  unsigned int* q = z.p[bid];
+  for (int i = (int)tid; i < z.w[bid]; i += 256) q[i] = 0u;
+}
 __global__ __launch_bounds__(256) void k_zero_counters(ZeroArgs z) {
-  unsigned int* q = z.p[blockIdx.x];
-  for (int i = threadIdx.x; i < z.w[blockIdx.x]; i += 256) q[i] = 0u;
+  d_zero_counters(z, blockIdx.x, threadIdx.x);
 }
 
 template <int S, int W>
@@ -2224,27 +2242,12 @@
              const CenterParams* prm, int ktp, int32_t* assign, int32_t* list,
              unsigned int* listCount, int32_t* list2, unsigned int* list2Count,
              const CandArgs* ca, hipStream_t st, const RefineArgs* ra = nullptr,
-             const AppendStage* stg = nullptr, const Bounds* bd = nullptr) {
+             const AppendStage* stg = nullptr, const Bounds* bd = nullptr,
+             bool countersZeroed = false) {
   const AppendStage* sg = ca ? stg : nullptr;
   const unsigned scap = sg ? sg->cap : 0u;
-  {
-    ZeroArgs z{};
-    auto add = [&](unsigned int* q, int words) {
-      if (q) {
-        z.p[z.n] = q;
-        z.w[z.n++] = words;
-      }
-    };
-    add(list2Count, 1);
-    if (ca) {
-      add(ca->candCount, 1);
-      add(ca->candCount2, 1);
-    }
-    if (ra && ca) {
-      add(ra->cand1Count, 1);
-      add(ra->fullCount, 2);
-    }
-    add(sg ? sg->counts : nullptr, kSets * kShards * kShardStride);
+  if (!countersZeroed) {
+    const ZeroArgs z = screen_zero_args(list2Count, ca, ra, stg);
     if (z.n) {
       hipLaunchKernelGGL(k_zero_counters, dim3(z.n), dim3(256), 0, st, z);
       CYC_LAUNCH_CHECK("k_zero_counters");
@@ -2422,12 +2425,13 @@
 }
 
 
-__global__ __launch_bounds__(256) void k_center_drift(const double* __restrict__ C,
-                                                      double* __restrict__ Cp, int k, int d,
-                                                      double* __restrict__ delta,
-                                                      double* __restrict__ ccs) {
-  const int lane = threadIdx.x & 63;
-  const int c = (blockIdx.x * blockDim.x + threadIdx.x) >> 6;
+__device__ __forceinline__ void d_center_drift(const double* __restrict__ C,
+                                               double* __restrict__ Cp, int k, int d,
+                                               double* __restrict__ delta,
+                                               double* __restrict__ ccs, unsigned bid,
+                                               unsigned tid) {
+  const int lane = tid & 63;
+  const int c = (int)((bid * 256 + tid) >> 6);
   if (c >= k) return;
   double s = 0.0, q = 0.0;
   for (int j = lane; j < d; j += 64) {
@@ -2444,13 +2448,19 @@
     ccs[c] = q * (1.0 + 0x1p-40);
   }
 }
-
-__global__ __launch_bounds__(1024) void k_drift_top(const double* __restrict__ delta,
-                                                    const double* __restrict__ ccs, int k,
-                                                    DriftParams* __restrict__ prm) {
+__global__ __launch_bounds__(256) void k_center_drift(const double* __restrict__ C,
+                                                      double* __restrict__ Cp, int k, int d,
+                                                      double* __restrict__ delta,
+                                                      double* __restrict__ ccs) {
+  d_center_drift(C, Cp, k, d, delta, ccs, blockIdx.x, threadIdx.x);
+}
+
+__device__ __forceinline__ void d_drift_top(const double* __restrict__ delta,
+                                            const double* __restrict__ ccs, int k,
+                                            DriftParams* __restrict__ prm, unsigned tid) {
   __shared__ double s1[1024], s2[1024], sc[1024];
   __shared__ int si[1024];
-  const int t = threadIdx.x;
+  const int t = (int)tid;
   double d1 = 0.0, d2 = 0.0, cm = 0.0;
   int i1 = -1;
   bool bad = false;
@@ -2496,6 +2506,11 @@
     *prm = p;
   }
 }
+__global__ __launch_bounds__(1024) void k_drift_top(const double* __restrict__ delta,
+                                                    const double* __restrict__ ccs, int k,
+                                                    DriftParams* __restrict__ prm) {
+  d_drift_top(delta, ccs, k, prm, threadIdx.x);
+}
 
 constexpr int kBndIT = kBndRows / 256;
 __device__ __forceinline__ void bnd_block_list(const unsigned long long (&masks)[kBndIT],
@@ -2521,10 +2536,9 @@
   }
 }
 
-__global__ __launch_bounds__(64) void k_center_nbrs(const double* __restrict__ stats, int k,
-                                                    int32_t* __restrict__ nbr,
-                                                    float* __restrict__ nbrR) {
-  const int a = blockIdx.x, lane = threadIdx.x;
+__device__ __forceinline__ void d_center_nbrs(const double* __restrict__ stats, int k,
+                                              int32_t* __restrict__ nbr,
+                                              float* __restrict__ nbrR, int a, int lane) {
   constexpr int T = kCandMax;
   double v[T];
   int ix[T];
@@ -2584,6 +2598,11 @@
       }
     }
   }
+}
+__global__ __launch_bounds__(64) void k_center_nbrs(const double* __restrict__ stats, int k,
+                                                    int32_t* __restrict__ nbr,
+                                                    float* __restrict__ nbrR) {
+  d_center_nbrs(stats, k, nbr, nbrR, blockIdx.x, threadIdx.x);
 }
 
 __global__ __launch_bounds__(256) void k_bounds_filter(const int32_t* __restrict__ assign,
@@ -2740,6 +2759,72 @@
                      cq, g, cnorm, prm, ktp, assign, list, listCount);
   CYC_LAUNCH_CHECK("k_kmeans_screen_i8");
   return CYC_OK;
+}
+
+struct PrepLevel {
+  unsigned ext[8];
+  int tps;
+  int S, ktp32;
+};
+enum { kP0Pairs, kP0Require, kP0Drift, kP0Scan, kP0Transpose, kP0Zero2, kP0Zero, kP0Jobs };
+enum { kP1DriftTop, kP1Params, kP1Diag, kP1Jobs };
+enum { kP2Pack, kP2Nbrs, kP2Jobs };
+
+__global__ __launch_bounds__(256) void k_prep_level0(PrepJobs J, PrepLevel L) {
+  const unsigned job = blockIdx.y, bid = blockIdx.x, tid = threadIdx.x;
+  if (bid >= L.ext[job]) return;
+  switch (job) {
+    case kP0Pairs:
+      kmc::stats_pairs(J.C, J.k, J.d, L.tps, J.stats, J.dmin, bid, tid);
+      break;
+    case kP0Require:
+      kmc::require_norms(J.C, J.k, J.d, J.xnorm, J.n, J.req, L.ext[kP0Require], bid, tid);
+      break;
+    case kP0Drift:
+      d_center_drift(J.C, J.Cp, J.k, J.d, J.delta, J.ccs, bid, tid);
+      break;
+    case kP0Scan:
+      d_centers_scan(J.C, J.k, J.d, J.scratch, J.scratch + J.k, bid, tid);
+      break;
+    case kP0Transpose:
+      kmc::center_transpose_fill(J.C, J.k, J.d, J.d4, J.kpad, J.ct, nullptr, 0ull, bid, tid);
+      break;
+    case kP0Zero2:
+      kmc::zero2(J.zeroA, J.zeroB, tid);
+      break;
+    default:
+      d_zero_counters(J.zero, bid, tid);
+      break;
+  }
+}
+
+__global__ __launch_bounds__(1024) void k_prep_level1(PrepJobs J, PrepLevel L) {
+  const unsigned job = blockIdx.y, bid = blockIdx.x, tid = threadIdx.x;
+  if (bid >= L.ext[job]) return;
+  switch (job) {
+    case kP1DriftTop:
+      d_drift_top(J.delta, J.ccs, J.k, J.dprm, tid);
+      break;
+    case kP1Params:
+      if (tid < 256) d_centers_params(J.k, J.scratch, J.scratch + J.k, J.cprm, tid);
+      break;
+    default:
+      if (tid < 256) kmc::stats_diag(J.k, J.stats, J.dmin, ~0ull, bid, tid);
+      break;
+  }
+}
+
+__global__ __launch_bounds__(256) void k_prep_level2(PrepJobs J, PrepLevel L) {
+  const unsigned job = blockIdx.y, bid = blockIdx.x, tid = threadIdx.x;
+  if (bid >= L.ext[job]) return;
+  if (job == kP2Pack) {
+    const size_t t16 = (size_t)J.ktp * 16;
+    d_centers_pack32(J.C, J.cnorm, J.k, J.d, L.S, L.ktp32, J.scratch + J.k, J.cprm, (uint4*)J.Cb,
+                     J.cq, J.g, J.cq + t16, J.g + t16, J.cq + 2 * t16, J.g + 2 * t16, bid, tid);
+  } else {
+    const int a = (int)(bid * 4 + (tid >> 6));
+    if (a < J.k) d_center_nbrs(J.stats, J.k, J.nbr, J.nbrR, a, (int)(tid & 63));
+  }
 }
 
 }
@@ -2800,6 +2885,88 @@
   return CYC_OK;
 }
 
+ZeroArgs screen_zero_args(unsigned int* list2Count, const CandArgs* ca, const RefineArgs* ra,
+                          const AppendStage* stg) {
+  const AppendStage* sg = ca ? stg : nullptr;
+  ZeroArgs z{};
+  auto add = [&](unsigned int* q, int words) {
+    if (q) {
+      z.p[z.n] = q;
+      z.w[z.n++] = words;
+    }
+  };
+  add(list2Count, 1);
+  if (ca) {
+    add(ca->candCount, 1);
+    add(ca->candCount2, 1);
+  }
+  if (ra && ca) {
+    add(ra->cand1Count, 1);
+    add(ra->fullCount, 2);
+  }
+  add(sg ? sg->counts : nullptr, kSets * kShards * kShardStride);
+  return z;
+}
+
+bool prep_fused() {
+  static const bool on = [] {
+    const char* e = std::getenv("CYC_KMEANS_PREP");
+    return !(e && e[0] == '0');
+  }();
+  return on;
+}
+
+int centers_prepare_all(const PrepJobs& J, hipStream_t st, void* reqHost, hipEvent_t reqEv) {
+  const int k = J.k, d = J.d;
+  if (J.Cb && !uses32(d)) {
+    set_error("centers_prepare_all packs the 32x32 screen's image only (d <= 256)");
+    return CYC_ERR_INVALID_ARG;
+  }
+  if (J.nbr && !J.stats) {
+    set_error("centers_prepare_all: neighbourhoods need the statistics");
+    return CYC_ERR_INVALID_ARG;
+  }
+  auto launch = [&](auto kern, const PrepLevel& L, int jobs, unsigned threads) {
+    unsigned gx = 0;
+    for (int i = 0; i < jobs; ++i) gx = std::max(gx, L.ext[i]);
+    if (gx) hipLaunchKernelGGL(kern, dim3(gx, (unsigned)jobs), dim3(threads), 0, st, J, L);
+  };
+  PrepLevel L0{};
+  L0.tps = (k + kmc::kStT - 1) / kmc::kStT;
+  L0.ext[kP0Pairs] = J.stats && k >= 2 ? (unsigned)(L0.tps * (L0.tps + 1) / 2) : 0u;
+  L0.ext[kP0Require] = J.req ? J.reqBlocks : 0u;
+  L0.ext[kP0Drift] = J.Cp ? (unsigned)((k + 3) / 4) : 0u;
+  L0.ext[kP0Scan] = J.Cb ? (unsigned)((k + 3) / 4) : 0u;
+  L0.ext[kP0Transpose] = J.ct ? (unsigned)(((int64_t)J.d4 * J.kpad + 255) / 256) : 0u;
+  L0.ext[kP0Zero2] = J.zeroA ? 1u : 0u;
+  L0.ext[kP0Zero] = (unsigned)J.zero.n;
+  launch(k_prep_level0, L0, kP0Jobs, 256);
+  CYC_LAUNCH_CHECK("k_prep_level0");
+  if (J.req) {
+    CYC_HIP(hipMemcpyAsync(reqHost, J.req, 5 * sizeof(unsigned long long), hipMemcpyDeviceToHost,
+                           st));
+    CYC_HIP(hipEventRecord(reqEv, st));
+  }
+  PrepLevel L1{};
+  L1.ext[kP1DriftTop] = J.Cp ? 1u : 0u;
+  L1.ext[kP1Params] = J.Cb ? 1u : 0u;
+  L1.ext[kP1Diag] = J.stats ? (unsigned)((k + 255) / 256) : 0u;
+  launch(k_prep_level1, L1, kP1Jobs, 1024);
+  CYC_LAUNCH_CHECK("k_prep_level1");
+  PrepLevel L2{};
+  if (J.Cb) {
+    L2.S = 2 * ksteps(d);
+    L2.ktp32 = tiles32(k);
+    const int64_t total =
+        std::max<int64_t>((int64_t)L2.ktp32 * L2.S * 64, (int64_t)L2.ktp32 * 32);
+    L2.ext[kP2Pack] = (unsigned)((total + 255) / 256);
+  }
+  L2.ext[kP2Nbrs] = J.nbr ? (unsigned)((k + 3) / 4) : 0u;
+  launch(k_prep_level2, L2, kP2Jobs, 256);
+  CYC_LAUNCH_CHECK("k_prep_level2");
+  return CYC_OK;
+}
+
 int centers_drift(const double* C, double* Cp, int k, int d, double* delta, double* ccs,
                   DriftParams* prm, hipStream_t st) {
   hipLaunchKernelGGL(k_center_drift, dim3((unsigned)((k + 3) / 4)), dim3(256), 0, st, C, Cp, k, d,
@@ -2817,12 +2984,12 @@
                   unsigned int* rcCount, unsigned long long* rcCum, const double* stats,
                   int32_t* nbr, float* nbrR, hipStream_t st, int32_t* tmp2,
                   unsigned int* bcount2, int32_t* list1, unsigned int* list1Count,
-                  unsigned long long* cum1) {
+                  unsigned long long* cum1, bool nbrsReady) {
   const int64_t nb = bounds_blocks(n);
   const bool two = tmp2 && bcount2 && list1 && list1Count;
   if (nb <= 0) return CYC_OK;
   KernelTimer timer("k_kmeans_bounds", st);
-  if (stats) {
+  if (stats && !nbrsReady) {
     hipLaunchKernelGGL(k_center_nbrs, dim3((unsigned)k), dim3(64), 0, st, stats, k, nbr, nbrR);
     CYC_LAUNCH_CHECK("k_center_nbrs");
   }
@@ -2871,7 +3038,7 @@
            const CenterParams* prm, int ktp, int32_t* assign, int32_t* list,
            unsigned int* listCount, int32_t* list2, unsigned int* list2Count, hipStream_t st,
            const CandArgs* ca, const RefineArgs* ra, const AppendStage* stg,
-           const Bounds* bd) {
+           const Bounds* bd, bool countersZeroed) {
   if (n <= 0) return CYC_OK;
   if (stg && stg->cap < shard_cap(n)) {
     set_error("append stage smaller than shard_cap(n)");
@@ -2884,8 +3051,8 @@
   if (uses32(d)) {
     const int k32 = ktp * 16 / 32;
     switch (ksteps(d)) {
-      case 2: return screen32<4, 4>(img, meta, xnorm, n, d, Cb, cq, g, cnorm, prm, k32, assign, list, listCount, list2, list2Count, ca, st, ra, stg, bd);
-      default: return screen32<8, 4>(img, meta, xnorm, n, d, Cb, cq, g, cnorm, prm, k32, assign, list, listCount, list2, list2Count, ca, st, ra, stg, bd);
+      case 2: return screen32<4, 4>(img, meta, xnorm, n, d, Cb, cq, g, cnorm, prm, k32, assign, list, listCount, list2, list2Count, ca, st, ra, stg, bd, countersZeroed);
+      default: return screen32<8, 4>(img, meta, xnorm, n, d, Cb, cq, g, cnorm, prm, k32, assign, list, listCount, list2, list2Count, ca, st, ra, stg, bd, countersZeroed);
     }
   }
   switch (ksteps(d)) {
diff --git a/cycloneml_amd/csrc/kmeans_i8.hpp b/cycloneml_amd/csrc/kmeans_i8.hpp
--- a/cycloneml_amd/csrc/kmeans_i8.hpp
+++ b/cycloneml_amd/csrc/kmeans_i8.hpp
@@ -114,7 +114,8 @@
                   unsigned int* rcCount, unsigned long long* rcCum, const double* stats,
                   int32_t* nbr, float* nbrR, hipStream_t st, int32_t* tmp2 = nullptr,
                   unsigned int* bcount2 = nullptr, int32_t* list1 = nullptr,
-                  unsigned int* list1Count = nullptr, unsigned long long* cum1 = nullptr);
+                  unsigned int* list1Count = nullptr, unsigned long long* cum1 = nullptr,
+                  bool nbrsReady = false);
 bool recheck_two_phase();
 
 int bounds_collect(const Bounds& bd, hipStream_t st);
@@ -125,7 +126,169 @@
            unsigned int* listCount, int32_t* list2, unsigned int* list2Count, hipStream_t st,
            const CandArgs* ca = nullptr,
            const RefineArgs* ra = nullptr, const AppendStage* stg = nullptr,
-           const Bounds* bd = nullptr);
-
-}
-}
+           const Bounds* bd = nullptr, bool countersZeroed = false);
+
+struct ZeroArgs {
+  unsigned int* p[8];
+  int w[8];
+  int n;
+};
+ZeroArgs screen_zero_args(unsigned int* list2Count, const CandArgs* ca, const RefineArgs* ra,
+                          const AppendStage* stg);
+
+struct PrepJobs {
+  const double* C = nullptr;
+  const double* cnorm = nullptr;
+  int k = 0, d = 0;
+  double* stats = nullptr;
+  unsigned long long* dmin = nullptr;
+  double* ct = nullptr;
+  int d4 = 0, kpad = 0;
+  const double* xnorm = nullptr;
+  int64_t n = 0;
+  unsigned long long* req = nullptr;
+  unsigned int reqBlocks = 0;
+  double* Cp = nullptr;
+  double* delta = nullptr;
+  double* ccs = nullptr;
+  DriftParams* dprm = nullptr;
+  int32_t* nbr = nullptr;
+  float* nbrR = nullptr;
+  int ktp = 0;
+  void* Cb = nullptr;
+  float* cq = nullptr;
+  double* g = nullptr;
+  CenterParams* cprm = nullptr;
+  double* scratch = nullptr;
+  unsigned int* zeroA = nullptr;
+  unsigned int* zeroB = nullptr;
+  ZeroArgs zero = {};
+};
+int centers_prepare_all(const PrepJobs& jobs, hipStream_t st, void* reqHost, hipEvent_t reqEv);
+bool prep_fused();
+
+}
+}
+
+#ifdef __HIPCC__
+#include "common.hpp"
+namespace cyc {
+namespace kmc {
+
+constexpr unsigned long long kInfBits = 0x7FF0000000000000ull;
+constexpr int kStT = 32;
+constexpr int kStC = 32;
+
+__device__ __forceinline__ void center_transpose_fill(const double* __restrict__ C, int k, int d,
+                                                      int d4, int kpad, double* __restrict__ Ct,
+                                                      unsigned long long* __restrict__ p,
+                                                      unsigned long long v, unsigned bid,
+                                                      unsigned tid) {
+  const int64_t idx = (int64_t)bid * 256 + tid;
+  if (p && idx < k) p[idx] = v;
+  const int64_t total = (int64_t)d4 * kpad;
+  if (idx >= total) return;
+  const int j = (int)(idx / kpad), i = (int)(idx % kpad);
+  Ct[idx] = (i < k && j < d) ? C[(int64_t)i * d + j] : 0.0;
+}
+
+__device__ __forceinline__ void zero2(unsigned int* __restrict__ a, unsigned int* __restrict__ b,
+                                      unsigned tid) {
+  if (tid == 0) *a = 0u;
+  if (tid == 1 && b) *b = 0u;
+}
+
+__device__ __forceinline__ void stats_pairs(const double* __restrict__ C, int k, int d, int tps,
+                                            double* __restrict__ packed,
+                                            unsigned long long* __restrict__ dmin, unsigned bid,
+                                            unsigned tid) {
+  __shared__ double Ci[kStT][kStC + 1], Cj[kStT][kStC + 1];
+  __shared__ unsigned long long rmin[kStT], cmin[kStT];
+  int t = (int)bid, bi = 0;
+  while (t >= tps - bi) {
+    t -= tps - bi;
+    ++bi;
+  }
+  const int bj = bi + t;
+  const int tx = tid & 15, ty = tid >> 4;
+  if (tid < kStT) rmin[tid] = cmin[tid] = kInfBits;
+  double s00 = 0.0, s01 = 0.0, s10 = 0.0, s11 = 0.0;
+  for (int c0 = 0; c0 < d; c0 += kStC) {
+    __syncthreads();
+    for (int e = tid; e < kStT * kStC; e += 256) {
+      const int r = e >> 5, cc = e & 31, col = c0 + cc;
+      const int gi = bi * kStT + r, gj = bj * kStT + r;
+      Ci[r][cc] = (gi < k && col < d) ? C[(int64_t)gi * d + col] : 0.0;
+      Cj[r][cc] = (gj < k && col < d) ? C[(int64_t)gj * d + col] : 0.0;
+    }
+    __syncthreads();
+    const int lim = min(kStC, d - c0);
+    for (int cc = 0; cc < lim; ++cc) {
+      const double a0 = Ci[ty][cc], a1 = Ci[ty + 16][cc];
+      const double b0 = Cj[tx][cc], b1 = Cj[tx + 16][cc];
+      double q = dsub(a0, b0);
+      s00 = dadd(s00, dmul(q, q));
+      q = dsub(a0, b1);
+      s01 = dadd(s01, dmul(q, q));
+      q = dsub(a1, b0);
+      s10 = dadd(s10, dmul(q, q));
+      q = dsub(a1, b1);
+      s11 = dadd(s11, dmul(q, q));
+    }
+  }
+  const double sv[2][2] = {{s00, s01}, {s10, s11}};
+#pragma unroll
+  for (int a = 0; a < 2; ++a) {
+#pragma unroll
+    for (int b = 0; b < 2; ++b) {
+      const int i = bi * kStT + ty + 16 * a, j = bj * kStT + tx + 16 * b;
+      if (i < k && j < k && j > i) {
+        const double dist = __builtin_sqrt(sv[a][b]);
+        const double v = dmul(dmul(0.25, dist), dist);
+        packed[iut(i, j)] = v;
+        const unsigned long long bits = (unsigned long long)__double_as_longlong(v);
+        atomicMin(&rmin[ty + 16 * a], bits);
+        atomicMin(&cmin[tx + 16 * b], bits);
+      }
+    }
+  }
+  __syncthreads();
+  if (tid < kStT) {
+    const int i = bi * kStT + tid, j = bj * kStT + tid;
+    if (i < k && rmin[tid] != kInfBits) atomicMin(&dmin[i], rmin[tid]);
+    if (j < k && cmin[tid] != kInfBits) atomicMin(&dmin[j], cmin[tid]);
+  }
+}
+
+__device__ __forceinline__ void stats_diag(int k, double* __restrict__ packed,
+                                           const unsigned long long* __restrict__ dmin,
+                                           unsigned long long empty, unsigned bid, unsigned tid) {
+  const int i = (int)(bid * 256 + tid);
+  if (i >= k) return;
+  if (k == 1) {
+    packed[0] = __builtin_nan("");
+    return;
+  }
+  const unsigned long long b = dmin[i];
+  packed[iut(i, i)] = __longlong_as_double((long long)(b == empty ? kInfBits : b));
+}
+
+__device__ __forceinline__ void require_norms(const double* __restrict__ C, int k, int d,
+                                              const double* __restrict__ xnorm, int64_t n,
+                                              unsigned long long* __restrict__ req,
+                                              unsigned nblocks, unsigned bid, unsigned tid) {
+  const int64_t stride = (int64_t)nblocks * 256;
+  const int64_t t0 = (int64_t)bid * 256 + tid;
+  const int64_t kd = (int64_t)k * d;
+  for (int64_t i = t0; i < kd; i += stride)
+    if (__builtin_isnan(C[i])) atomicMin(&req[0], (unsigned long long)(i / d));
+  for (int64_t r = t0; r < n; r += stride)
+    if (__builtin_isnan(xnorm[r])) atomicMin(&req[1], (unsigned long long)r);
+  double* out = reinterpret_cast<double*>(req + 2);
+  if (t0 < 2 && t0 < k) out[t0] = seq_norm2(C + t0 * d, d);
+  if (t0 == 2) out[2] = n > 0 ? xnorm[0] : 0.0;
+}
+
+}
+}
+#endif
```

Result: faster. 14.27 billion (median of 6 runs) (+6.8%).
